# petabi/petal-neighbors

Measured on AMD Instinct MI355X. Metric: exact k-NN queries/sec (1M x 128 fp32, k=10), higher is better.
Workload: dtype f32; 1 GPU; c2: 1000000 points x 128 dims f32, 10000 queries, k=10, uniform[0,1); n_points=1000000, dim=128, n_queries=10000, k=10, engine=bf16, exchange=none (one shard), rccl_world_size=1

## Files before the change

bindings/rust/src/ffi.rs:

```rust
#![allow(non_camel_case_types)]
use std::os::raw::{c_char, c_int, c_uint, c_void};

pub const PN_RADIUS_SORTED: c_uint = 1;
pub const PN_SELF_INCLUDE: c_uint = 2;
pub const PN_MS_SEED_ROWS: c_uint = 4;
pub const PN_MS_ORPHANS: c_uint = 8;
pub const PN_KDE_GAUSSIAN: c_int = 0;
pub const PN_KDE_TOPHAT: c_int = 1;
pub const PN_KDE_EPANECHNIKOV: c_int = 2;
pub const PN_KDE_EXPONENTIAL: c_int = 3;
pub const PN_KDE_LINEAR: c_int = 4;

#[repr(C)]
pub struct pn_index {
    _private: [u8; 0],
}
#[repr(C)]
pub struct pn_sharded {
    _private: [u8; 0],
}

pub const PN_OK: c_int = 0;
pub const PN_ERR_EMPTY: c_int = 1;
pub const PN_ERR_NOT_CONTIGUOUS: c_int = 2;
pub const PN_ERR_COMM: c_int = 8;

extern "C" {
    pub fn pn_last_error() -> *const c_char;
    pub fn pn_index_destroy(index: *mut pn_index);
    pub fn pn_free(p: *mut c_void);

    pub fn pn_index_create_f32(points: *const f32, n_rows: usize, n_cols: usize, row_stride: isize, col_stride: isize,
                               device: c_int, out: *mut *mut pn_index) -> c_int;
    pub fn pn_index_create_f64(points: *const f64, n_rows: usize, n_cols: usize, row_stride: isize, col_stride: isize,
                               device: c_int, out: *mut *mut pn_index) -> c_int;
    pub fn pn_index_create_cosine_f32(points: *const f32, n_rows: usize, n_cols: usize, row_stride: isize,
                                      col_stride: isize, device: c_int, out: *mut *mut pn_index) -> c_int;
    pub fn pn_index_create_cosine_f64(points: *const f64, n_rows: usize, n_cols: usize, row_stride: isize,
                                      col_stride: isize, device: c_int, out: *mut *mut pn_index) -> c_int;

    pub fn pn_query_f32(index: *const pn_index, queries: *const f32, nq: usize, q_cols: usize, q_row_stride: isize,
                        k: usize, idx_out: *mut u64, dist_out: *mut f32) -> c_int;
    pub fn pn_query_f64(index: *const pn_index, queries: *const f64, nq: usize, q_cols: usize, q_row_stride: isize,
                        k: usize, idx_out: *mut u64, dist_out: *mut f64) -> c_int;
    pub fn pn_query_radius_f32(index: *const pn_index, queries: *const f32, nq: usize, q_cols: usize,
                               q_row_stride: isize, radius: f32, offsets: *mut u64, idx_out: *mut *mut u64) -> c_int;
    pub fn pn_query_radius_f64(index: *const pn_index, queries: *const f64, nq: usize, q_cols: usize,
                               q_row_stride: isize, radius: f64, offsets: *mut u64, idx_out: *mut *mut u64) -> c_int;
    pub fn pn_query_radius_with_distance_f32(index: *const pn_index, queries: *const f32, nq: usize, q_cols: usize,
                                             q_row_stride: isize, radius: f32, flags: c_uint, offsets: *mut u64,
                                             idx_out: *mut *mut u64, dist_out: *mut *mut f32) -> c_int;
    pub fn pn_query_radius_with_distance_f64(index: *const pn_index, queries: *const f64, nq: usize, q_cols: usize,
                                             q_row_stride: isize, radius: f64, flags: c_uint, offsets: *mut u64,
                                             idx_out: *mut *mut u64, dist_out: *mut *mut f64) -> c_int;
    pub fn pn_query_radius_with_distance_device_f32(index: *const pn_index, d_queries: *const f32, nq: usize,
                                                    q_cols: usize, q_row_stride: usize, radius: f32, flags: c_uint,
                                                    d_offsets: *mut u64, d_idx: *mut u64, d_dist: *mut f32,
                                                    capacity: usize, d_total: *mut u64, stream: *mut c_void) -> c_int;
    pub fn pn_query_radius_with_distance_device_f64(index: *const pn_index, d_queries: *const f64, nq: usize,
                                                    q_cols: usize, q_row_stride: usize, radius: f64, flags: c_uint,
                                                    d_offsets: *mut u64, d_idx: *mut u64, d_dist: *mut f64,
                                                    capacity: usize, d_total: *mut u64, stream: *mut c_void) -> c_int;
    pub fn pn_sharded_query_radius_with_distance_f32(sharded: *const pn_sharded, queries: *const f32, nq: usize,
                                                     q_cols: usize, q_row_stride: isize, radius: f32, flags: c_uint,
// ... 284 lines not shown
```

include/petal_mi355x.h:

```cpp
#ifndef PETAL_MI355X_H
#define PETAL_MI355X_H

#include <stddef.h>
#include <stdint.h>

#ifdef __cplusplus
extern "C" {
#endif

#define PN_ABI_VERSION 3

enum {
    PN_OK = 0,
    PN_ERR_EMPTY = 1,
    PN_ERR_NOT_CONTIGUOUS = 2,
    PN_ERR_INVALID = 3,
    PN_ERR_DEVICE = 4,
    PN_ERR_NOMEM = 5,
    PN_ERR_UNSUPPORTED = 6,
    PN_ERR_EMPTY_MATRIX = 7,
    PN_ERR_COMM = 8
};

enum {
    PN_ENGINE_AUTO = 0,
    PN_ENGINE_EXACT = 1,
    PN_ENGINE_MFMA = 2,
    PN_ENGINE_BF16 = 3
};

enum {
    PN_OPT_ENGINE = 1,
    PN_OPT_SEGMENTS = 2,
    PN_OPT_INDEX_BASE = 3,
    PN_OPT_PROFILE = 4,
    PN_OPT_FILTER_SLOTS = 5,
    PN_OPT_MFMA_STRUCTURE = 6,
    PN_OPT_EXCHANGE_ALWAYS = 7,
    PN_OPT_SHARED_THRESHOLDS = 8,
    PN_OPT_BF16_WAVES = 9,
    PN_OPT_SEED_MODEL = 10,
    PN_OPT_DBSCAN_PIECE = 11,
    PN_OPT_MST_BATCH = 12,
    PN_OPT_OPTICS_PIECE = 13,
    PN_OPT_KDE_PIECE = 14,
    PN_OPT_MS_PIECE = 15,
    PN_OPT_KMEANS_FILTER = 16
};

enum {
    PN_KDE_GAUSSIAN = 0,
    PN_KDE_TOPHAT = 1,
    PN_KDE_EPANECHNIKOV = 2,
    PN_KDE_EXPONENTIAL = 3,
    PN_KDE_LINEAR = 4
};

typedef struct pn_index pn_index;

typedef struct pn_info {
    uint64_t n_points;
    uint64_t dim;
    uint64_t row_stride_device;
    int32_t elem_bytes;
    int32_t device;
    int32_t mfma_eligible;
    int32_t bf16_eligible;
    int32_t bf16_layout;
    int32_t seed_model;
} pn_info;

typedef struct pn_stats {
    uint64_t queries;
    uint64_t fallback_queries;
    uint64_t candidates;
    uint64_t hot_launches;
    double hot_ms;
    double last_call_ms;
    uint64_t radius_results;
    uint64_t evaluations;
    double shard_ms;
    double exchange_ms;
    uint64_t reserved[1];
} pn_stats;

const char *pn_last_error(void);
const char *pn_strerror(int code);
int pn_abi_version(void);
int pn_device_count(int *count);

int pn_index_create_f32(const float *points, size_t n_rows, size_t n_cols, ptrdiff_t row_stride,
                        ptrdiff_t col_stride, int device, pn_index **out);
int pn_index_create_f64(const double *points, size_t n_rows, size_t n_cols, ptrdiff_t row_stride,
                        ptrdiff_t col_stride, int device, pn_index **out);
int pn_index_create_cosine_f32(const float *points, size_t n_rows, size_t n_cols, ptrdiff_t row_stride,
                               ptrdiff_t col_stride, int device, pn_index **out);
int pn_index_create_cosine_f64(const double *points, size_t n_rows, size_t n_cols, ptrdiff_t row_stride,
                               ptrdiff_t col_stride, int device, pn_index **out);
int pn_index_create_device_f32(const float *d_points, size_t n_rows, size_t n_cols, size_t row_stride,
                               int device, void *stream, pn_index **out);
// ... 378 lines not shown
```

petal-neighbors_amd/_lib.py:

```python
from __future__ import annotations

import ctypes as C
import os

_HERE = os.path.dirname(os.path.abspath(__file__))
LIB_PATH = os.environ.get("PN_LIBRARY_PATH") or os.path.join(_HERE, "libpetal_mi355x.so")

PN_OK, PN_ERR_EMPTY, PN_ERR_NOT_CONTIGUOUS, PN_ERR_INVALID, PN_ERR_DEVICE, PN_ERR_NOMEM, \
    PN_ERR_UNSUPPORTED, PN_ERR_EMPTY_MATRIX, PN_ERR_COMM = range(9)
PN_COMM_ID_BYTES = 128
PN_ENGINE_AUTO, PN_ENGINE_EXACT, PN_ENGINE_MFMA, PN_ENGINE_BF16 = 0, 1, 2, 3
PN_OPT_ENGINE, PN_OPT_SEGMENTS, PN_OPT_INDEX_BASE, PN_OPT_PROFILE, PN_OPT_FILTER_SLOTS = 1, 2, 3, 4, 5
PN_OPT_MFMA_STRUCTURE = 6
PN_OPT_EXCHANGE_ALWAYS = 7
PN_OPT_SHARED_THRESHOLDS = 8
PN_OPT_BF16_WAVES = 9
PN_OPT_SEED_MODEL = 10
PN_OPT_DBSCAN_PIECE = 11
PN_OPT_MST_BATCH = 12
PN_OPT_OPTICS_PIECE = 13
PN_OPT_KDE_PIECE = 14
PN_OPT_MS_PIECE = 15
PN_OPT_KMEANS_FILTER = 16
PN_KDE_GAUSSIAN, PN_KDE_TOPHAT, PN_KDE_EPANECHNIKOV, PN_KDE_EXPONENTIAL, PN_KDE_LINEAR = 0, 1, 2, 3, 4
PN_RADIUS_SORTED = 1
PN_SELF_INCLUDE = 2
PN_MS_SEED_ROWS = 4
PN_MS_ORPHANS = 8


class PnInfo(C.Structure):
    _fields_ = [("n_points", C.c_uint64), ("dim", C.c_uint64), ("row_stride_device", C.c_uint64),
                ("elem_bytes", C.c_int32), ("device", C.c_int32), ("mfma_eligible", C.c_int32),
                ("bf16_eligible", C.c_int32), ("bf16_layout", C.c_int32), ("seed_model", C.c_int32)]


class PnStats(C.Structure):
    _fields_ = [("queries", C.c_uint64), ("fallback_queries", C.c_uint64), ("candidates", C.c_uint64),
                ("hot_launches", C.c_uint64), ("hot_ms", C.c_double), ("last_call_ms", C.c_double),
                ("radius_results", C.c_uint64), ("evaluations", C.c_uint64),
                ("shard_ms", C.c_double), ("exchange_ms", C.c_double), ("reserved", C.c_uint64 * 1)]


class PnShardedInfo(C.Structure):
    _fields_ = [("n_points", C.c_uint64), ("dim", C.c_uint64), ("local_first_row", C.c_uint64),
                ("local_rows", C.c_uint64), ("n_shards", C.c_int32), ("world", C.c_int32),
                ("local_shards", C.c_int32), ("rank", C.c_int32), ("mfma_eligible", C.c_int32),
                ("bf16_eligible", C.c_int32)]


_sz, _ssz, _i, _vp, _u64, _cu, _d = C.c_size_t, C.c_ssize_t, C.c_int, C.c_void_p, C.c_uint64, C.c_uint, C.c_double
_u64p, _ip, _vpp = C.POINTER(C.c_uint64), C.POINTER(C.c_int), C.POINTER(C.c_void_p)
_R, _RP = "real", "real*"

_QH, _QD = [_vp, _vp, _sz, _sz, _ssz], [_vp, _vp, _sz, _sz, _sz]
_CSR_H, _CSR_D = [_vp, _vpp, _vpp], [_vp, _vp, _vp, _sz, _vp, _vp]
_CREATE = [_vp, _sz, _sz, _ssz, _ssz, _i, _vpp]
_SH_CREATE = [_vp, _sz, _sz, _ssz, _ssz, _ip, _i, _vpp]
_PAIRWISE = [_vp, _sz, _sz, _ssz, _i, _vp]

PAIRED = {
    "pn_index_create": (_i, _CREATE),
    "pn_index_create_cosine": (_i, _CREATE),
    "pn_pairwise_device": (_i, [_vp, _sz, _sz, _sz, _i, _vp, _vp]),
    "pn_index_create_device": (_i, [_vp, _sz, _sz, _sz, _i, _vp, _vpp]),
    "pn_query": (_i, _QH + [_sz, _vp, _vp]),
    "pn_query_device": (_i, _QD + [_sz, _vp, _vp, _vp]),
    "pn_query_nearest": (_i, _QH + [_vp, _vp]),
    "pn_query_radius": (_i, _QH + [_R, _vp, _vpp]),
    "pn_query_radius_device": (_i, _QD + [_R, _vp, _vp, _sz, _vp, _vp]),
    "pn_query_radius_with_distance": (_i, _QH + [_R, _cu] + _CSR_H),
    "pn_query_radius_with_distance_device": (_i, _QD + [_R, _cu] + _CSR_D),
    "pn_query_self": (_i, [_vp, _sz, _cu, _vp, _vp]),
    "pn_query_self_device": (_i, [_vp, _sz, _cu, _vp, _vp, _vp]),
    "pn_query_radius_self": (_i, [_vp, _R, _cu] + _CSR_H),
    "pn_query_radius_self_device": (_i, [_vp, _R, _cu] + _CSR_D),
# ... 128 lines not shown
```

petal-neighbors_amd/csrc/bf16_filter.hip:

```cpp
#include "pn_internal.h"
#include "topk_buffer.h"

#include <cstdio>
#include <cstdlib>

namespace pn {

typedef __bf16 bf16x8 __attribute__((ext_vector_type(8)));
typedef float f32x16 __attribute__((ext_vector_type(16)));
typedef uint32_t u32x4 __attribute__((ext_vector_type(4)));
typedef __attribute__((address_space(3))) void lds_void_b;
typedef const __attribute__((address_space(1))) void glb_void_b;

#ifdef PN_DIAG_BF_COUNT
__device__ unsigned long long g_bfdbg[16];
#define BF_COUNT(i, v) (dbg_[i] += (unsigned long long)(v))
#define BF_DBG_DECL unsigned long long dbg_[12] = {0, 0, 0, 0, 0, 0, 0, 0, 0, 0, 0, 0}
#define BF_DBG_ARG , unsigned long long (&dbg_)[12]
#define BF_DBG_PASS , dbg_
#define BF_DBG_FLUSH(lane)                                                        \
    do {                                                                          \
        if ((lane) == 0)                                                          \
            for (int i_ = 0; i_ < 12; ++i_) {                                     \
                atomicAdd(&g_bfdbg[i_], dbg_[i_]);                                \
                dbg_[i_] = 0;                                                     \
            }                                                                     \
    } while (0)
__device__ __forceinline__ unsigned long long bf_stamp() {
    unsigned long long t;
    asm volatile("s_memtime %0\n\ts_waitcnt lgkmcnt(0)" : "=s"(t)::"memory");
    return t;
}
__device__ __forceinline__ unsigned long long bf_stamp_nw() {
    unsigned long long t;
    asm volatile("s_memtime %0" : "=s"(t));
    return t;
}
__device__ __forceinline__ void bf_settle(unsigned long long &t) { asm volatile("s_waitcnt lgkmcnt(0)" : "+s"(t)::"memory"); }
#else
#define BF_COUNT(i, v) ((void)0)
#define BF_DBG_DECL ((void)0)
#define BF_DBG_ARG
#define BF_DBG_PASS
#define BF_DBG_FLUSH(lane) ((void)0)
#endif

constexpr int kBQ = 256;
constexpr int kBP = 64;
constexpr double kG = 1.0 / 8192.0;
constexpr double kUp = 1.0 + 1.0 / 1099511627776.0;
__host__ __device__ inline int bf16_extra_col(int dim) {
    const int room = (dim + 15) / 16 * 16 - dim;
    return room >= 5 && dim > 16 ? dim : (dim + 15) / 16 * 16;
}
__host__ __device__ inline int bf16_steps(int dim) { return (bf16_extra_col(dim) + 5 + 15) / 16; }
__host__ __device__ inline bool bf16_ci_dim(int dim) { return dim >= 17 && dim <= 128 && bf16_steps(dim) > (dim + 15) / 16; }
__host__ __device__ inline int bf16_steps_for(int dim, bool ci) { return ci ? (dim + 15) / 16 : bf16_steps(dim); }

__device__ __forceinline__ uint16_t bf_rne(float x) {
    const uint32_t u = __float_as_uint(x);
    return (uint16_t)((u + 0x7FFFu + ((u >> 16) & 1u)) >> 16);
}
__device__ __forceinline__ float bf_f(uint16_t b) { return __uint_as_float((uint32_t)b << 16); }
__device__ __forceinline__ float f_down(double x) {
    float f = (float)x;
    if ((double)f > x) f = __uint_as_float(__float_as_uint(f) - 1u);
    return f;
}
__device__ __forceinline__ float f_up(double x) {
    float f = (float)x;
    if ((double)f < x) f = __uint_as_float(__float_as_uint(f) + 1u);
    return f;
}
__device__ __forceinline__ float f_up_signed(double x) {
    float f = (float)x;
    if ((double)f < x) f = (f >= 0.0f) ? __uint_as_float(__float_as_uint(f) + 1u) : __uint_as_float(__float_as_uint(f) - 1u);
    return f;
}
__device__ __forceinline__ uint16_t bf_trunc(float x) { return (uint16_t)(__float_as_uint(x) >> 16); }
__device__ __forceinline__ uint16_t bf_up(float x) {
    const uint32_t u = __float_as_uint(x);
    return (uint16_t)((u >> 16) + ((u & 0xFFFFu) ? 1u : 0u));
}

constexpr int kWR = 256;
constexpr int kWPitch = 128;
constexpr int kWPiece = kWR * kWPitch;
constexpr int kWStage = 2 * kWPiece;
constexpr int kWDma = kWStage / 1024 / 8;
__host__ __device__ inline int bf16_wide_nkc(int dim) { return (dim + 63) / 64; }
__host__ __device__ inline bool bf16_wide_has_x(int dim) { return bf16_extra_col(dim) + 5 > 64 * bf16_wide_nkc(dim); }
constexpr int kWXPiece = kWR * 32;
__host__ __device__ inline size_t bf16_wide_tile_bytes(int dim) {
    return (size_t)bf16_wide_nkc(dim) * kWPiece + (bf16_wide_has_x(dim) ? kWXPiece : 0);
}
__host__ __device__ inline unsigned bf_wide_swz(size_t r) { return (unsigned)((r >> 1) & 7); }
__host__ __device__ inline unsigned bf_wide_xswz(size_t r) { return (unsigned)((r >> 3) & 1); }
__device__ __forceinline__ size_t bf_wide_at(size_t r, int k, int dim) {
    const int nkc = bf16_wide_nkc(dim);
    const size_t tile = (r / kWR) * (bf16_wide_tile_bytes(dim) / 2), rr = r % kWR;
    if ((k >> 6) >= nkc) {
        const unsigned slot = (unsigned)(((k - 64 * nkc) >> 3) & 1) ^ bf_wide_xswz(rr);
        return tile + (size_t)nkc * (kWPiece / 2) + rr * 16 + (size_t)slot * 8 + (size_t)(k & 7);
    }
    const unsigned slot = (unsigned)((k & 63) >> 3) ^ bf_wide_swz(rr);
    return tile + ((size_t)(k >> 6) * kWR + rr) * (size_t)(kWPitch / 2) + (size_t)slot * 8 + (size_t)(k & 7);
}

template <typename T>
__device__ __forceinline__ bool bf_row_part8(const T *__restrict__ src, const float *__restrict__ mu, int dim, size_t ld,
                                             int c0, int CH, bool in_rows, uint16_t (&hb)[18], double &pn, double &en,
                                             double &hn) {
    T xf[18];
#pragma unroll
    for (int i = 0; i < 18; ++i) xf[i] = (T)0;
    constexpr int VE = 16 / (int)sizeof(T);
    const bool vec = (CH % 4) == 0 && c0 + CH <= (int)ld;
    if (in_rows) {
        if (vec) {
#pragma unroll
            for (int i = 0; i < 18; i += VE)
                if (i + VE <= CH) {
                    typedef T tv_ __attribute__((ext_vector_type(VE)));
                    const tv_ t4 = *reinterpret_cast<const tv_ *>(src + c0 + i);
#pragma unroll
                    for (int j = 0; j < VE; ++j) xf[i + j] = t4[j];
                }
        } else {
#pragma unroll
// ... 97 lines not shown
template <typename T>
__global__ __launch_bounds__(256) void bf16_row_stats8_kernel(const T *__restrict__ P, const float *__restrict__ mu,
                                                              size_t n, int dim, size_t ld, int KS, size_t rows,
                                                              double *__restrict__ out) {
    const int sub = (int)(threadIdx.x & 7);
    const int CH = 2 * KS;
    double bm = 0.0, dm = 0.0, bs = 0.0, ds = 0.0;
    const size_t stride = (size_t)gridDim.x * blockDim.x;
    for (size_t t = (size_t)blockIdx.x * blockDim.x + threadIdx.x; t < rows * 8; t += stride) {
        const size_t r = t >> 3;
        uint16_t v[18];
        double pn, en, hn;
        const bool in_rows = r < n;
        const bool finite = bf_row_part8<T>(P + (in_rows ? r : 0) * ld, mu, dim, ld, sub * CH, CH, in_rows, v, pn, en, hn);
        if (in_rows && sub == 0 && finite && pn < 1.2676506002282294e30) {
            const double bp = (2.0 * sqrt(en) * kUp + 2.0 * kG * sqrt(hn) * kUp) * (1.0 + 2.0 * kG) * kUp;
            const double dp = 2.0 * sqrt(pn) * kUp * (1.0 + 2.0 * kG) * kUp;
            bm = fmax(bm, bp);
            dm = fmax(dm, dp);
            bs += bp;
            ds += dp;
        }
    }
    for (int d = 32; d > 0; d >>= 1) {
        bm = fmax(bm, __shfl_xor(bm, d));
        dm = fmax(dm, __shfl_xor(dm, d));
        bs += __shfl_xor(bs, d);
        ds += __shfl_xor(ds, d);
    }
    __shared__ double red[4][4];
    const int wave = (int)(threadIdx.x >> 6);
    if ((threadIdx.x & 63) == 0) {
        red[wave][0] = bm;
        red[wave][1] = dm;
        red[wave][2] = bs;
        red[wave][3] = ds;
    }
    __syncthreads();
    if (threadIdx.x == 0) {
        for (int w = 1; w < 4; ++w) {
            bm = fmax(bm, red[w][0]);
            dm = fmax(dm, red[w][1]);
            bs += red[w][2];
            ds += red[w][3];
        }
        atomicMax(reinterpret_cast<unsigned long long *>(out), (unsigned long long)__double_as_longlong(bm));
        atomicMax(reinterpret_cast<unsigned long long *>(out + 1), (unsigned long long)__double_as_longlong(dm));
        atomicAdd(out + 2, bs);
        atomicAdd(out + 3, ds);
    }
}

template <typename T>
__global__ void bf16_row_stats_kernel(const T *__restrict__ P, const float *__restrict__ mu, size_t n, int dim,
                                      size_t ld, double *__restrict__ out) {
    const size_t r = (size_t)blockIdx.x * blockDim.x + threadIdx.x;
    double bp = 0.0, dp = 0.0;
    if (r < n) {
        double pn = 0.0, en = 0.0, hn = 0.0;
        bool finite = true;
        const T *src = P + r * ld;
        for (int k = 0; k < dim; ++k) {
            const double x = (double)src[k];
            finite = finite && (fabs(x) < 1.0e30);
            const double c = x - (double)mu[k];
            const float cf = (float)c;
            const uint16_t hb = (fabsf(cf) < 8.67361737988403547e-19f) ? (uint16_t)0 : bf_rne(cf);
            const double xh = (double)bf_f(hb);
            pn += c * c;
            en += (c - xh) * (c - xh);
            hn += xh * xh;
        }
        if (finite && pn < 1.2676506002282294e30) {
            bp = (2.0 * sqrt(en) * kUp + 2.0 * kG * sqrt(hn) * kUp) * (1.0 + 2.0 * kG) * kUp;
            dp = 2.0 * sqrt(pn) * kUp * (1.0 + 2.0 * kG) * kUp;
        }
    }
    double bm = bp, dm = dp, bs = bp, ds = dp;
    for (int d = 32; d > 0; d >>= 1) {
        bm = fmax(bm, __shfl_xor(bm, d));
        dm = fmax(dm, __shfl_xor(dm, d));
        bs += __shfl_xor(bs, d);
        ds += __shfl_xor(ds, d);
    }
    if ((threadIdx.x & 63) == 0) {
        atomicMax(reinterpret_cast<unsigned long long *>(out), (unsigned long long)__double_as_longlong(bm));
        atomicMax(reinterpret_cast<unsigned long long *>(out + 1), (unsigned long long)__double_as_longlong(dm));
        atomicAdd(out + 2, bs);
        atomicAdd(out + 3, ds);
    }
}

template <typename T, bool QRY>
__global__ void bf16_pack_wide8_kernel(const T *__restrict__ X, const float *__restrict__ mu, size_t n_valid,
                                       size_t n_rows_img, int dim, size_t ld, uint16_t *__restrict__ img,
                                       double *__restrict__ qn, uint32_t *__restrict__ qbad, uint32_t *__restrict__ bad,
                                       Bf16SeedModel sm) {
    const size_t t = (size_t)blockIdx.x * blockDim.x + threadIdx.x;
    const size_t r = t >> 3;
    const int sub = (int)(t & 7);
    if (r >= n_rows_img) return;
    double sm_mean = 0.0, sm_var = 0.0;
    const int n_slots = 8 * bf16_wide_nkc(dim) + (bf16_wide_has_x(dim) ? 2 : 0);
    const int E = bf16_extra_col(dim);
    const int gx0 = E >> 3, gx1 = (E + 4) >> 3;
    const bool in_rows = r < n_valid;
// ... 79 lines not shown
        rem -= (double)bf_f(x[1]);
        x[2] = bf_trunc(f_down(rem));
        const double e_n = sqrt(en) * kUp, h_n = sqrt(hn) * kUp, p_n = sqrt(s) * kUp;
        x[3] = bf_up(f_up((2.0 * e_n + 2.0 * kG * h_n) * (1.0 + 2.0 * kG)));
        x[4] = bf_up(f_up(2.0 * p_n * (1.0 + 2.0 * kG)));
    }
    const bool zero_data = QRY && !ok;
    if (zero_data)
        for (int g = sub; g < n_slots; g += 8)
            if (g != gx0 && g != gx1) *reinterpret_cast<u4_ *>(img + bf_wide_at(r, 8 * g, dim)) = u4_{0u, 0u, 0u, 0u};
#pragma unroll
    for (int w = 0; w < 2; ++w) {
        const int g = w == 0 ? gx0 : gx1;
        if ((w == 1 && gx1 == gx0) || (g & 7) != sub || g >= n_slots) continue;
#pragma unroll
        for (int j = 0; j < 8; ++j) {
            const int k = 8 * g + j;
            if (zero_data) vx[w][j] = 0;
            if (k >= E && k < E + 5) vx[w][j] = x[k - E];
        }
        *reinterpret_cast<u4_ *>(img + bf_wide_at(r, 8 * g, dim)) = pack8(vx[w]);
    }
    if (QRY && sm.seed_out) {
#pragma unroll
        for (int d = 1; d < 8; d <<= 1) {
            sm_mean += __shfl_xor(sm_mean, d);
            sm_var += __shfl_xor(sm_var, d);
        }
    }
    if (sub == 0) {
        if (QRY) {
            qn[r] = ok ? s / kUp : 0.0;
            qbad[r] = ok ? 0u : 1u;
            if (sm.seed_out) {
                float sd = __uint_as_float(0xFF800000u);
                if (in_rows && ok) {
                    const double var = sm.v0 + sm_var;
                    sd = f_up_signed(sm.c0 - 2.0 * sm_mean - sm.z * sqrt(var > 0.0 ? var : 0.0));
                }
                const uint32_t key = f2s(sd);
                sm.seed_out[r] = (sd == sd && key != 0xFFFFFFFFu && in_rows && ok) ? key + 1u : f2s(__uint_as_float(0xFF800000u));
            }
        } else if (in_rows && !ok) {
            atomicOr(bad, 1u);
        }
    }
}

template <typename T>
__global__ void bf16_pack_queries8_kernel(const T *__restrict__ Q, const float *__restrict__ mu, size_t nq,
                                          size_t nq_pad, int dim, size_t ld, int KS, uint16_t *__restrict__ B,
                                          double *__restrict__ qn, uint32_t *__restrict__ qbad, int ci, double bmax,
                                          double dmax, T *__restrict__ Qp, size_t ldq,
                                          uint32_t *__restrict__ misc, Bf16SeedModel sm) {
    const size_t t = (size_t)blockIdx.x * blockDim.x + threadIdx.x;
    const size_t q = t >> 3;
    const int sub = (int)(t & 7);
    if (misc && t < 16) misc[t] = 0u;
    if (q >= nq_pad) return;
    const int K = 16 * KS, CH = 2 * KS, E = bf16_extra_col(dim);
    const int c0 = sub * CH;
    uint16_t v[18];
    double s = 0.0, en = 0.0, hn = 0.0, sm_mean = 0.0, sm_var = 0.0;
    bool finite = true;
    const T *src = Q + q * ld;
    if (Qp) {
        for (int k = K + sub; k < (int)ldq; k += 8) Qp[q * ldq + k] = (T)0;
    }
    T xf[18];
    const bool in_rows = q < nq;
    constexpr int VE = 16 / (int)sizeof(T);
    const bool vec = (CH % 4) == 0 && ((reinterpret_cast<uintptr_t>(Q) | (ld * sizeof(T))) & 15u) == 0 &&
                     c0 + CH <= dim;
#pragma unroll
    for (int i = 0; i < 18; ++i) xf[i] = (T)0;
    if (in_rows) {
        if (vec) {
#pragma unroll
            for (int i = 0; i < 18; i += VE)
                if (i + VE <= CH) {
                    typedef T tv_ __attribute__((ext_vector_type(VE)));
                    const tv_ t4 = *reinterpret_cast<const tv_ *>(src + c0 + i);
#pragma unroll
                    for (int j = 0; j < VE; ++j) xf[i + j] = t4[j];
                }
        } else {
#pragma unroll
            for (int i = 0; i < 18; ++i)
                if (i < CH && c0 + i < dim) xf[i] = src[c0 + i];
        }
    }
    if (Qp) {
        T *qd = Qp + q * ldq + c0;
#pragma unroll
        for (int i = 0; i < 18; i += 2)
            if (i + 2 <= CH && c0 + i + 2 <= (int)ldq) {
                typedef T tp_ __attribute__((ext_vector_type(2)));
                tp_ pr;
                pr[0] = xf[i];
                pr[1] = xf[i + 1];
                *reinterpret_cast<tp_ *>(qd + i) = pr;
            }
    }
    float muv[18], m1v[18], av[18], bv[18];
    const bool vecm = (CH % 4) == 0 && c0 + CH <= dim;
#pragma unroll
    for (int i = 0; i < 18; i += 4) {
// ... 35 lines not shown
            const double x = (double)xf[i];
            finite = finite && (fabs(x) < 1.0e30);
            const double c = x - (double)muv[i];
            const float cf = (float)c;
            const uint16_t hb = (fabsf(cf) < 8.67361737988403547e-19f) ? (uint16_t)0 : bf_rne(cf);
            const float xh = bf_f(hb);
            v[i] = bf_rne(-2.0f * xh);
            s += c * c;
            const double e = c - (double)xh;
            en += e * e;
            hn += (double)xh * (double)xh;
            if (sm.seed_out) {
                sm_mean += c * (double)m1v[i];
                sm_var += c * (c * (double)av[i] - (double)bv[i]);
            }
        }
    }
    uint32_t fin = finite ? 1u : 0u;
#pragma unroll
    for (int d = 1; d < 8; d <<= 1) {
        s += __shfl_xor(s, d);
        en += __shfl_xor(en, d);
        hn += __shfl_xor(hn, d);
        fin &= (uint32_t)__shfl_xor((int)fin, d);
    }
    if (sm.seed_out) {
#pragma unroll
        for (int d = 1; d < 8; d <<= 1) {
            sm_mean += __shfl_xor(sm_mean, d);
            sm_var += __shfl_xor(sm_var, d);
        }
    }
    const bool ok = fin != 0u && (s < 1.2676506002282294e30);
    if (!ok) {
#pragma unroll
        for (int i = 0; i < 18; ++i)
            if (c0 + i < dim) v[i] = 0;
    }
    if (!ci) {
#pragma unroll
        for (int i = 0; i < 18; ++i) {
            const int k = c0 + i;
            if (i < CH) {
                if (k == E + 0 || k == E + 1 || k == E + 2) v[i] = 0x3F80u;
                if (ok && k == E + 3) v[i] = (uint16_t)(bf_up(f_up(sqrt(hn) * kUp)) | 0x8000u);
                if (ok && k == E + 4) v[i] = (uint16_t)(bf_up(f_up(sqrt(en) * kUp)) | 0x8000u);
            }
        }
    }
    uint16_t *dst = B + q * (size_t)K + c0;
#pragma unroll
    for (int i = 0; i < 18; ++i)
        if (i < CH) dst[i] = v[i];
    if (sub == 0) {
        if (ci) {
            const double eq = (sqrt(hn) * kUp * bmax + sqrt(en) * kUp * dmax) * kUp;
            qn[q] = ok ? s / kUp - eq : 0.0;
        } else {
            qn[q] = ok ? s / kUp : 0.0;
        }
        qbad[q] = ok ? 0u : 1u;
        if (sm.seed_out) {
            float sd = __uint_as_float(0xFF800000u);
            if (q < nq && ok) {
                const double var = sm.v0 + sm_var;
                const double S = sm.c0 - 2.0 * sm_mean - sm.z * sqrt(var > 0.0 ? var : 0.0);
                sd = f_up_signed(S);
            }
            const uint32_t key = f2s(sd);
            sm.seed_out[q] = (sd == sd && key != 0xFFFFFFFFu && q < nq && ok) ? key + 1u : f2s(__uint_as_float(0xFF800000u));
        }
    }
}

template <typename T>
__global__ __launch_bounds__(256) void cos_normalize_rows_kernel(const T *__restrict__ X, size_t n_valid, size_t n_out,
                                                                 int dim, size_t ld_in, double *__restrict__ out,
                                                                 size_t ld_out, uint32_t *__restrict__ bad, int nan_rows) {
    const size_t t = (size_t)blockIdx.x * blockDim.x + threadIdx.x;
    const size_t r = t >> 3;
    const int sub = (int)(t & 7);
    if (r >= n_out) return;
    const int CH = (int)(ld_out / 8), c0 = sub * CH;
    double *o = out + r * ld_out + c0;
    if (r >= n_valid) {
        for (int i = 0; i < CH; ++i) o[i] = 0.0;
        return;
    }
    const T *x = X + r * ld_in;
    double ss = 0.0;
    for (int i = 0; i < CH; ++i)
        if (c0 + i < dim) {
            const double v = (double)x[c0 + i];
            ss += v * v;
        }
#pragma unroll
    for (int d = 1; d < 8; d <<= 1) ss += __shfl_xor(ss, d);
    const bool ok = ss >= 7.888609052210118e-31 && ss <= 1.2676506002282294e30;
    if (!ok) {
        if (nan_rows) {
            for (int i = 0; i < CH; ++i) o[i] = (c0 + i < dim) ? __longlong_as_double(0x7FF8000000000000ll) : 0.0;
        } else {
            if (sub == 0) atomicOr(bad, 1u);
            for (int i = 0; i < CH; ++i) o[i] = 0.0;
        }
        return;
    }
    const double inv = 1.0 / sqrt(ss);
    for (int i = 0; i < CH; ++i) o[i] = (c0 + i < dim) ? (double)x[c0 + i] * inv : 0.0;
}
template <typename T>
hipError_t launch_cos_normalize_rows(const T *X, size_t n_valid, size_t n_out, int dim, size_t ld_in, double *out,
                                     size_t ld_out, uint32_t *bad, bool nan_rows, hipStream_t s) {
    if (ld_out % 8 != 0 || (size_t)dim > ld_out || (size_t)dim > ld_in) return hipErrorInvalidValue;
// ... 83 lines not shown
}

constexpr int kLA = 3;
constexpr int kBfFinalKeep = 32;
constexpr int kScoutList = 12;
__device__ __forceinline__ void bf_min2(const f32x16 &v, float &mn, float &sec) {
    const float big = 3.4e38f;
    auto lo3 = [](float a, float b, float c) { return fminf(fminf(a, b), c); };
    auto md3 = [](float a, float b, float c) { return __builtin_amdgcn_fmed3f(a, b, c); };
    const float l0 = lo3(v[0], v[1], v[2]), d0 = md3(v[0], v[1], v[2]);
    const float l1 = lo3(v[3], v[4], v[5]), d1 = md3(v[3], v[4], v[5]);
    const float l2 = lo3(v[6], v[7], v[8]), d2 = md3(v[6], v[7], v[8]);
    const float l3 = lo3(v[9], v[10], v[11]), d3 = md3(v[9], v[10], v[11]);
    const float l4 = lo3(v[12], v[13], v[14]), d4 = md3(v[12], v[13], v[14]);
    const float l5 = v[15];
    const float a = lo3(l0, l1, l2), am = md3(l0, l1, l2);
    const float b = lo3(l3, l4, l5), bm = md3(l3, l4, l5);
    mn = fminf(a, b);
    const float sec_lo = lo3(fmaxf(a, b), am, bm);
    const float dmin = fminf(lo3(d0, d1, d2), fminf(d3, d4));
    sec = fminf(sec_lo, dmin);
    (void)big;
}

template <int KS, bool CI>
__device__ __forceinline__ void bf_chain(const char *arow, const bf16x8 (&pre)[kLA], const bf16x8 (&b0)[KS],
                                         const bf16x8 (&b1)[KS], const f32x16 &c0, f32x16 &w0, f32x16 &w1, f32x16 &r0,
                                         f32x16 &r1, float &m0, float &m1) {
    bf16x8 f[KS];
#pragma unroll
    for (int i = 0; i < kLA && i < KS; ++i) f[i] = pre[i];
    f32x16 z;
#pragma unroll
    for (int i = 0; i < 16; ++i) z[i] = 0.0f;
#pragma unroll
    for (int ks = 0; ks < KS; ++ks) {
        if (ks + kLA < KS) f[ks + kLA] = *reinterpret_cast<const bf16x8 *>(arow + 32 * (ks + kLA));
        if (CI) {
            w0 = __builtin_amdgcn_mfma_f32_32x32x16_bf16(f[ks], b0[ks], ks ? w0 : c0, 0, 0, 0);
            w1 = __builtin_amdgcn_mfma_f32_32x32x16_bf16(f[ks], b1[ks], ks ? w1 : c0, 0, 0, 0);
        } else {
            w0 = __builtin_amdgcn_mfma_f32_32x32x16_bf16(f[ks], b0[ks], ks ? w0 : z, 0, 0, 0);
            w1 = __builtin_amdgcn_mfma_f32_32x32x16_bf16(f[ks], b1[ks], ks ? w1 : z, 0, 0, 0);
        }
#pragma unroll
        for (int i = 16 * ks / KS; i < 16 * (ks + 1) / KS; ++i) {
            m0 = i ? fminf(m0, r0[i]) : r0[0];
            m1 = i ? fminf(m1, r1[i]) : r1[0];
        }
        __builtin_amdgcn_sched_barrier(0);
    }
}

template <int CP>
__device__ __forceinline__ f32x16 bf_cinit(const char *tb, int blk, int h) {
    typedef float f32x4_ __attribute__((ext_vector_type(4)));
    f32x16 c;
#pragma unroll
    for (int g = 0; g < 4; ++g) {
        const f32x4_ v = *reinterpret_cast<const f32x4_ *>(tb + ((blk * 8 + 2 * g + h) * CP + (CP - 1)) * 16);
        c[4 * g + 0] = v[0];
        c[4 * g + 1] = v[1];
        c[4 * g + 2] = v[2];
        c[4 * g + 3] = v[3];
    }
    return c;
}

struct BfNoMid {
    static constexpr int at(int) { return -1; }
    __device__ __forceinline__ void operator()() const {}
};
template <int KS, bool CI, int CP, typename MID = BfNoMid>
__device__ __forceinline__ void bf_chain_p(const char *arow, bf16x8 (&pre)[kLA], const bf16x8 (&b0)[KS],
                                           const bf16x8 (&b1)[KS], f32x16 &c, f32x16 &w0, f32x16 &w1, f32x16 &r0,
                                           f32x16 &r1, float &m0, float &m1, const char *narow, const char *ntb,
                                           int nblk, int h, MID mid = MID()) {
    typedef float f32x4_ __attribute__((ext_vector_type(4)));
    bf16x8 f[KS];
#pragma unroll
    for (int i = 0; i < kLA && i < KS; ++i) f[i] = pre[i];
    f32x16 z, nc = c;
#pragma unroll
    for (int i = 0; i < 16; ++i) z[i] = 0.0f;
#pragma unroll
    for (int ks = 0; ks < KS; ++ks) {
        if (ks == MID::at(KS)) mid();
        if (ks + kLA < KS) f[ks + kLA] = *reinterpret_cast<const bf16x8 *>(arow + 32 * (ks + kLA));
#pragma unroll
        for (int i = 0; i < kLA; ++i)
            if (ks == (KS - kLA + i > 0 ? KS - kLA + i : 0))
                pre[i] = *reinterpret_cast<const bf16x8 *>(narow + 32 * (i < KS ? i : 0));
        if (CI) {
#pragma unroll
            for (int g = 0; g < 4; ++g)
                if (ks == (KS - 4 + g > 0 ? KS - 4 + g : 0)) {
                    const f32x4_ v =
                        *reinterpret_cast<const f32x4_ *>(ntb + ((nblk * 8 + 2 * g + h) * CP + (CP - 1)) * 16);
                    nc[4 * g + 0] = v[0];
                    nc[4 * g + 1] = v[1];
                    nc[4 * g + 2] = v[2];
                    nc[4 * g + 3] = v[3];
                }
            w0 = __builtin_amdgcn_mfma_f32_32x32x16_bf16(f[ks], b0[ks], ks ? w0 : c, 0, 0, 0);
            w1 = __builtin_amdgcn_mfma_f32_32x32x16_bf16(f[ks], b1[ks], ks ? w1 : c, 0, 0, 0);
            if (ks == 0) asm volatile("" ::"v"(c));
        } else {
            w0 = __builtin_amdgcn_mfma_f32_32x32x16_bf16(f[ks], b0[ks], ks ? w0 : z, 0, 0, 0);
            w1 = __builtin_amdgcn_mfma_f32_32x32x16_bf16(f[ks], b1[ks], ks ? w1 : z, 0, 0, 0);
        }
#pragma unroll
        for (int i = 16 * ks / KS; i < 16 * (ks + 1) / KS; ++i) {
            m0 = i ? fminf(m0, r0[i]) : r0[0];
            m1 = i ? fminf(m1, r1[i]) : r1[0];
        }
        __builtin_amdgcn_sched_barrier(0);
    }
    c = nc;
}

constexpr uint32_t kShPeriod = 32;
constexpr uint32_t kShMaxPass = 1u << 14;
__device__ __forceinline__ uint32_t sh_load(const uint32_t *p) {
    return __hip_atomic_load(p, __ATOMIC_RELAXED, __HIP_MEMORY_SCOPE_AGENT);
}
__device__ __forceinline__ void sh_store(uint32_t *p, uint32_t v) {
    __hip_atomic_store(p, v, __ATOMIC_RELAXED, __HIP_MEMORY_SCOPE_AGENT);
}
__device__ __forceinline__ void sh_store_entry(uint2 *p, uint32_t key, uint32_t row) {
    __hip_atomic_store(reinterpret_cast<unsigned long long *>(p), ((unsigned long long)row << 32) | key, __ATOMIC_RELAXED,
                       __HIP_MEMORY_SCOPE_AGENT);
}
__device__ __forceinline__ uint32_t sh_tag(uint32_t epoch, uint32_t ncomp) { return (epoch << 20) | ((ncomp & 0xFFu) << 12); }

template <int M>
__device__ __forceinline__ void bf_refresher(const uint2 *__restrict__ cand, const uint32_t *pcnt, uint32_t *gtau,
                                          const uint32_t *done, uint32_t n_main, size_t nq_pad, uint32_t nseg,
                                          uint32_t epoch, uint32_t rank, uint32_t wv, uint32_t n_wv, int lane) {
    constexpr uint32_t CAP = 64u * M;
    constexpr int NK = 8;
    auto words_of = [&](size_t q) -> uint32_t {
        uint32_t x = 0;
        if (lane < (int)nseg) x = sh_load(pcnt + (size_t)lane * nq_pad + q);
        else if (lane == 63) x = sh_load(done);
        return x;
    };
    for (uint32_t pass = 0; pass < kShMaxPass; ++pass) {
        uint32_t x_next = words_of(wv < nq_pad ? wv : 0);
        for (size_t q = wv; q < nq_pad; q += n_wv) {
            const uint32_t x = x_next;
            x_next = words_of(q + n_wv < nq_pad ? q + n_wv : q);
            if ((uint32_t)__builtin_amdgcn_readlane((int)x, 63) >= n_main) return;
#ifdef PN_DIAG_BF_COUNT
            if (lane == 0) atomicAdd(&g_bfdbg[12], 1ull);
#endif
            uint32_t c = (lane < (int)nseg && (x >> 20) == epoch) ? (x & 0xFFFu) : 0u;
            if (c > CAP) c = 0;
            uint32_t inc = c;
#pragma unroll
            for (int d = 1; d < 64; d <<= 1) {
                const uint32_t t = (uint32_t)__shfl_up((int)inc, d);
                if (lane >= d) inc += t;
            }
            uint32_t U = (uint32_t)__builtin_amdgcn_readlane((int)inc, 63);
            if (U < rank) continue;
            if (U > 64u * NK) U = 64u * NK;
            const uint32_t excl = inc - c;
            uint32_t key[NK];
#pragma unroll
            for (int i = 0; i < NK; ++i) key[i] = 0xFFFFFFFFu;
            const int nk = (int)((U + 63u) / 64u);
// ... 861 lines not shown
        }
        asm volatile("s_waitcnt vmcnt(0)" ::: "memory");
        const uint32_t kfin = keep_arg > kp ? keep_arg : kp;
        unsigned long long need = __ballot(h == 0 && cnt > kfin);
        constexpr int NB = M == 1 ? 4 : 1;
        while (need) {
            int jj[NB];
            uint32_t cj[NB], key[NB][M], ixs[NB][M];
#pragma unroll
            for (int bb = 0; bb < NB; ++bb) {
                jj[bb] = need ? __builtin_ctzll(need) : -1;
                if (need) need &= need - 1;
                cj[bb] = jj[bb] >= 0 ? (uint32_t)__builtin_amdgcn_readlane((int)cnt, jj[bb] >= 0 ? jj[bb] : 0) : 0u;
                if (jj[bb] >= 0) bf_compact_load<M>(ce_blk + (size_t)jj[bb] * CAP, cj[bb], lane, key[bb], ixs[bb]);
            }
#pragma unroll
            for (int bb = 0; bb < NB; ++bb) {
                if (jj[bb] >= 0) {
                    uint32_t T, nn;
                    bf_compact_finish<M>(ce_blk + (size_t)jj[bb] * CAP, key[bb], ixs[bb], cj[bb], kp, lane, T, nn);
                    if (jq == jj[bb]) { tau = fminf(tau, s2f(T)); cnt = nn; }
                }
            }
        }
        if (h == 0) {
            ccnt[cell0 + jq] = cnt;
            ctau[cell0 + jq] = f2s(tau);
        }
        BF_DBG_FLUSH(lane);
    }
    if (SH) {
        __syncthreads();
        if (tid == 0) (void)__hip_atomic_fetch_add(sh.done, 1u, __ATOMIC_RELAXED, __HIP_MEMORY_SCOPE_AGENT);
    }
}

#ifndef PN_DIAG_PAIR_STAGGER
#define PN_DIAG_PAIR_STAGGER 1
#endif
constexpr int kPairStagger = PN_DIAG_PAIR_STAGGER;
#ifndef PN_DIAG_PAIR_MID4
#define PN_DIAG_PAIR_MID4 2
#endif
struct BfPairMeet {
    uint32_t ns;
    static constexpr int at(int ks) { return ks * PN_DIAG_PAIR_MID4 / 4 > 1 ? ks * PN_DIAG_PAIR_MID4 / 4 : 1; }
    __device__ __forceinline__ void operator()() const {
        bf_wait_dma(ns);
        __builtin_amdgcn_s_barrier();
        asm volatile("" ::: "memory");
    }
};

template <int KS, bool CI, int STAG>
__device__ __forceinline__ void bf_pair_run(const char *__restrict__ img, char *tiles, uint32_t kp, uint32_t kfin, uint2 *__restrict__ cand,
                                            uint32_t *__restrict__ ccnt, uint32_t *__restrict__ ctau,
                                            const bf16x8 (&b0)[KS], const bf16x8 (&b1)[KS], float tau0, float tau1,
                                            uint32_t rt0, uint32_t rt1, size_t cell0, bool active, int wave, int lane) {
    constexpr int C = 2 * KS, CP = C + 1;
    constexpr uint32_t CAP = 64u;
    constexpr int TB = kBP * CP * 16;
    constexpr int NBUF = 3, NW = 8;
    const int jq = lane & 31, h = lane >> 5;
    BF_DBG_DECL;
    constexpr int P = (CP + NW - 1) / NW;
    static_assert(P <= 3, "piece schedule written out for up to three pieces per wave");
    const int n_mine = CP - wave * P < P ? (CP - wave * P > 0 ? CP - wave * P : 0) : P;
    const uint32_t lane_off = (uint32_t)lane * 16u;
    auto dma_tile = [&](uint32_t rt, int buf) {
        const char *wbase = img + ((size_t)rt * (size_t)TB + (size_t)(wave * (P * 1024)));
        const char *ws = wbase + lane_off;
        char *wd = tiles + buf * TB + wave * (P * 1024);
        if (0 < n_mine) __builtin_amdgcn_global_load_lds((glb_void_b *)ws, (lds_void_b *)wd, 16, 0, 0);
        if (P > 1 && 1 < n_mine) __builtin_amdgcn_global_load_lds((glb_void_b *)ws, (lds_void_b *)wd, 16, 1024, 0);
        if (P > 2 && 2 < n_mine) __builtin_amdgcn_global_load_lds((glb_void_b *)ws, (lds_void_b *)wd, 16, 2048, 0);
    };

    uint32_t cnt0 = 0, cnt1 = 0;
    uint2 *ce_blk0 = cand + cell0 * CAP;
    uint2 *ce_blk1 = ce_blk0 + (size_t)32 * CAP;
    uint2 *ceq0 = ce_blk0 + (size_t)jq * CAP, *ceq1 = ce_blk1 + (size_t)jq * CAP;
    uint32_t ns = 0;

    f32x16 a00, a01, a10, a11;
#pragma unroll
    for (int r = 0; r < 16; ++r) {
        a00[r] = 3.0e38f;
        a01[r] = 3.0e38f;
        a10[r] = 3.0e38f;
        a11[r] = 3.0e38f;
    }
    bf16x8 pre[kLA];
    f32x16 cc = a00;
    {
        const char *ar = tiles + (jq * CP + h) * 16;
#pragma unroll
        for (int i = 0; i < kLA; ++i) pre[i] = *reinterpret_cast<const bf16x8 *>(ar + 32 * (i < KS ? i : 0));
        if (CI) cc = bf_cinit<CP>(tiles, 0, h);
    }
    int cur = 0;
    for (uint32_t rt = rt0; rt < rt1; ++rt) {
        const int nxt = cur == NBUF - 1 ? 0 : cur + 1, prv = cur == 0 ? NBUF - 1 : cur - 1;
        const char *tb = tiles + cur * TB;
        const char *arow0 = tb + (jq * CP + h) * 16;
        const char *arow1 = arow0 + 32 * CP * 16;
        float m0, m1, p0, p1;
        if (STAG == 2) BfPairMeet{ns}();
        if (STAG == 1)
            bf_chain_p<KS, CI, CP>(arow0, pre, b0, b1, cc, a00, a01, a10, a11, m0, m1, arow1, tb, 1, h, BfPairMeet{ns});
        else
            bf_chain_p<KS, CI, CP>(arow0, pre, b0, b1, cc, a00, a01, a10, a11, m0, m1, arow1, tb, 1, h);
        if (rt == rt0) { m0 = __uint_as_float(0x7F800000u); m1 = m0; }
        if (__any(m0 < tau0 || m1 < tau1)) {
            const uint32_t row0 = (rt - 1) * kBP + 32;
            if (__any(m0 < tau0)) bf_slow<1, false>(a10, m0, tau0, cnt0, row0, h, jq, lane, kp, ceq0, ce_blk0, ns BF_DBG_PASS);
            if (__any(m1 < tau1)) bf_slow<1, false>(a11, m1, tau1, cnt1, row0, h, jq, lane, kp, ceq1, ce_blk1, ns BF_DBG_PASS);
        }
        if (STAG == 0) {
            bf_wait_dma(ns);
#ifndef PN_DIAG_PAIR_NOLGKM
            asm volatile("s_waitcnt lgkmcnt(0)" ::: "memory");
#endif
            __builtin_amdgcn_s_barrier();
            asm volatile("" ::: "memory");
        }
        if (rt + 2 < rt1) {
            dma_tile(rt + 2, prv);
            ns = 0;
        }
        const bool last = rt + 1 >= rt1;
        const char *ntb = last ? tb : tiles + nxt * TB;
        bf_chain_p<KS, CI, CP>(arow1, pre, b0, b1, cc, a10, a11, a00, a01, p0, p1, ntb + (jq * CP + h) * 16, ntb, 0, h);
        if (__any(p0 < tau0 || p1 < tau1)) {
            const uint32_t row0 = rt * kBP;
            if (__any(p0 < tau0)) bf_slow<1, false>(a00, p0, tau0, cnt0, row0, h, jq, lane, kp, ceq0, ce_blk0, ns BF_DBG_PASS);
            if (__any(p1 < tau1)) bf_slow<1, false>(a01, p1, tau1, cnt1, row0, h, jq, lane, kp, ceq1, ce_blk1, ns BF_DBG_PASS);
        }
        cur = nxt;
    }
    {
        float m0 = a10[0], m1 = a11[0];
#pragma unroll
        for (int i = 1; i < 16; ++i) {
            m0 = fminf(m0, a10[i]);
            m1 = fminf(m1, a11[i]);
        }
        const uint32_t row0 = (rt1 - 1) * kBP + 32;
        if (__any(m0 < tau0)) bf_slow<1, false>(a10, m0, tau0, cnt0, row0, h, jq, lane, kp, ceq0, ce_blk0, ns BF_DBG_PASS);
        if (__any(m1 < tau1)) bf_slow<1, false>(a11, m1, tau1, cnt1, row0, h, jq, lane, kp, ceq1, ce_blk1, ns BF_DBG_PASS);
    }
    asm volatile("s_waitcnt vmcnt(0)" ::: "memory");
    auto final_compact = [&](uint2 *ce_blk, float &tau, uint32_t &cnt) {
        constexpr int NB = 4;
        unsigned long long need = __ballot(h == 0 && cnt > kfin);
        while (need) {
            int jj[NB];
            uint32_t cj[NB], key[NB][1], ixs[NB][1];
#pragma unroll
            for (int b = 0; b < NB; ++b) {
                jj[b] = need ? __builtin_ctzll(need) : -1;
                if (need) need &= need - 1;
                cj[b] = jj[b] >= 0 ? (uint32_t)__builtin_amdgcn_readlane((int)cnt, jj[b] >= 0 ? jj[b] : 0) : 0u;
                if (jj[b] >= 0) bf_compact_load<1>(ce_blk + (size_t)jj[b] * CAP, cj[b], lane, key[b], ixs[b]);
            }
#pragma unroll
            for (int b = 0; b < NB; ++b) {
                if (jj[b] >= 0) {
                    uint32_t T, nn;
                    bf_compact_finish<1>(ce_blk + (size_t)jj[b] * CAP, key[b], ixs[b], cj[b], kp, lane, T, nn);
                    if (jq == jj[b]) { tau = fminf(tau, s2f(T)); cnt = nn; }
                }
            }
        }
    };
    final_compact(ce_blk0, tau0, cnt0);
    final_compact(ce_blk1, tau1, cnt1);
    if (active && h == 0) {
        ccnt[cell0 + jq] = cnt0;
        ctau[cell0 + jq] = f2s(tau0);
        ccnt[cell0 + 32 + jq] = cnt1;
        ctau[cell0 + 32 + jq] = f2s(tau1);
    }
    BF_DBG_FLUSH(lane);
}

template <int KS, bool CI>
__global__ __launch_bounds__(512, 2) void bf16_filter_kernel_pair(const char *__restrict__ img, uint32_t n_tiles,
                                                                  const u32x4 *__restrict__ Bq, uint32_t q_tiles,
                                                                  uint32_t kp_keep, uint2 *__restrict__ cand,
                                                                  uint32_t *__restrict__ ccnt,
                                                                  uint32_t *__restrict__ ctau, size_t nq_pad,
                                                                  const uint32_t *tau_init, BfShared sh) {
    const uint32_t kp = kp_keep & 0xFFFFu, keep_arg = kp_keep >> 16;
    const uint32_t kfin = keep_arg > kp ? keep_arg : kp;
    constexpr int CP = 2 * KS + 1;
    constexpr int TB = kBP * CP * 16;
    extern __shared__ __attribute__((aligned(16))) unsigned char smem_raw[];
    char *tiles = reinterpret_cast<char *>(smem_raw);
    const int tid = threadIdx.x, lane = tid & 63;
    const int wave = __builtin_amdgcn_readfirstlane(tid >> 6);
    const int jq = lane & 31, h = lane >> 5;
    constexpr int C = 2 * KS;
    const uint32_t W = gridDim.x, n_pairs = (q_tiles + 1u) >> 1, c_per = W / n_pairs;
    uint32_t w;
    {
        const uint32_t b = blockIdx.x, x = b & 7u, base = W >> 3, rem = W & 7u;
        const uint32_t L = x * base + (x < rem ? x : rem) + (b >> 3);
        w = (L % n_pairs) * c_per + L / n_pairs;
    }
    const uint32_t pt = w / c_per, seg = w % c_per;
    const uint32_t rt0 = (uint32_t)((unsigned long long)seg * n_tiles / c_per);
    const uint32_t rt1 = (uint32_t)((unsigned long long)(seg + 1) * n_tiles / c_per);
    if (rt0 >= rt1) return;
    const uint32_t qt = 2u * pt + (uint32_t)(wave >> 2);
    const bool active = qt < q_tiles;
    const size_t q0 = active ? (size_t)qt * kBQ + (size_t)(wave & 3) * 64 : 0;
    const size_t cell0 = (size_t)seg * nq_pad + q0;

    bf16x8 b0[KS], b1[KS];
    float tau0 = __uint_as_float(0xFF800000u), tau1 = tau0;
    if (active) {
        const u32x4 *br0 = Bq + (q0 + jq) * (size_t)C + h;
        const u32x4 *br1 = br0 + (size_t)32 * C;
#pragma unroll
        for (int ks = 0; ks < KS; ++ks) {
            const u32x4 v0 = br0[2 * ks], v1 = br1[2 * ks];
            b0[ks] = __builtin_bit_cast(bf16x8, v0);
            b1[ks] = __builtin_bit_cast(bf16x8, v1);
        }
        if (sh.seed_lists) {
            const size_t ql = q0 + (size_t)lane;
            float sd = __uint_as_float(0xFF800000u);
            if (ql < (size_t)sh.seed_nq) {
                const uint32_t key = f2s(bf_seed_lane(sh.seed_lists, nq_pad, sh.nseg, sh.seed_rank, ql));
                sd = s2f(key == 0xFFFFFFFFu ? key : key + 1u);
            }
            tau0 = __shfl(sd, jq);
            tau1 = __shfl(sd, 32 + jq);
        } else {
            tau0 = s2f(tau_init[q0 + jq]);
            tau1 = s2f(tau_init[q0 + 32 + jq]);
        }
    } else {
        const u32x4 zero = {0u, 0u, 0u, 0u};
#pragma unroll
        for (int ks = 0; ks < KS; ++ks) {
            b0[ks] = __builtin_bit_cast(bf16x8, zero);
            b1[ks] = b0[ks];
        }
    }
    {
        constexpr int P = (CP + 7) / 8;
        const int n_mine = CP - wave * P < P ? (CP - wave * P > 0 ? CP - wave * P : 0) : P;
        for (uint32_t t = 0; t < 2u && rt0 + t < rt1; ++t) {
            const char *ws = img + ((size_t)(rt0 + t) * (size_t)TB + (size_t)(wave * (P * 1024))) + (uint32_t)lane * 16u;
            char *wd = tiles + t * TB + wave * (P * 1024);
            if (0 < n_mine) __builtin_amdgcn_global_load_lds((glb_void_b *)ws, (lds_void_b *)wd, 16, 0, 0);
            if (P > 1 && 1 < n_mine) __builtin_amdgcn_global_load_lds((glb_void_b *)ws, (lds_void_b *)wd, 16, 1024, 0);
            if (P > 2 && 2 < n_mine) __builtin_amdgcn_global_load_lds((glb_void_b *)ws, (lds_void_b *)wd, 16, 2048, 0);
        }
    }
    __syncthreads();
    if (wave >= 4)
        bf_pair_run<KS, CI, kPairStagger>(img, tiles, kp, kfin, cand, ccnt, ctau, b0, b1, tau0, tau1, rt0, rt1, cell0,
                                          active, wave, lane);
    else
        bf_pair_run<KS, CI, 0>(img, tiles, kp, kfin, cand, ccnt, ctau, b0, b1, tau0, tau1, rt0, rt1, cell0, active, wave,
                               lane);
}

template <int M, bool RAD>
__global__ __launch_bounds__(512, 1) void bf16_wide_kernel(const char *__restrict__ img, uint32_t n_tiles,
                                                           const char *__restrict__ Bimg, uint32_t nkc,
                                                           uint32_t tile_bytes, uint32_t has_x, uint32_t kp,
                                                           uint2 *__restrict__ cand, uint32_t *__restrict__ ccnt,
                                                           uint32_t *__restrict__ ctau, size_t nq_pad,
                                                           uint32_t scout_max,
                                                           const uint32_t *__restrict__ tau_init,
                                                           float *__restrict__ scout_out) {
    constexpr uint32_t CAP = 64u * M;
    extern __shared__ __attribute__((aligned(16))) unsigned char smem_raw[];
    char *lds = reinterpret_cast<char *>(smem_raw);

    const int tid = threadIdx.x, lane = tid & 63;
    const int wave = __builtin_amdgcn_readfirstlane(tid >> 6);
    const int jq = lane & 31, h = lane >> 5;
    const int qg = wave & 3, rh = wave >> 2;
    BF_DBG_DECL;

    uint32_t w = blockIdx.x;
    const uint32_t W = gridDim.x;
    {
        const uint32_t x = blockIdx.x & 7u, base = W >> 3, rem = W & 7u;
        w = x * base + (x < rem ? x : rem) + (blockIdx.x >> 3);
    }
    const unsigned long long U = (unsigned long long)(nq_pad / kWR) * n_tiles, Wn = W;
    unsigned long long u0 = (unsigned long long)w * U / Wn;
    const unsigned long long u1 = (unsigned long long)(w + 1) * U / Wn;
    const float inf = __uint_as_float(0x7F800000u);

    int slot_off[4];
#pragma unroll
    for (int s = 0; s < 4; ++s) slot_off[s] = (int)(((unsigned)(2 * s + h) ^ bf_wide_swz((size_t)jq)) * 16u);
    int st = 0;
    uint32_t ns = 0;
    f32x16 acc[4][2];

    while (u0 < u1) {
    const uint32_t qt = (uint32_t)(u0 / n_tiles);
    const unsigned long long v_begin = (unsigned long long)qt * n_tiles, v_end = v_begin + n_tiles;
    const unsigned long long run_end = u1 < v_end ? u1 : v_end;
    const uint32_t rt0 = (uint32_t)(u0 - v_begin), rt1 = (uint32_t)(run_end - v_begin);
    unsigned long long wf = v_begin * Wn / U;
    while ((wf + 1) * U / Wn <= v_begin) ++wf;
    while (wf > 0 && wf * U / Wn > v_begin) --wf;
    const uint32_t sg = (uint32_t)(w - wf);
    const size_t q0 = (size_t)qt * kWR + (size_t)qg * 64;
    const size_t cell0 = (size_t)(sg * 2 + rh) * nq_pad + q0;
    float tau0 = inf, tau1 = inf;
    uint32_t cnt0 = 0, cnt1 = 0;

// ... 356 lines not shown
    double mu2 = 0.0;
    for (int k = 0; k < dim; ++k) {
        const double m = sums[k] / (double)n;
        const float f = (m == m && fabs(m) < 1e30) ? (float)m : 0.0f;
        mu[k] = f;
        mu2 += (double)f * (double)f;
    }
    const double s2 = sums[dim], s2c = s2 - (double)n * mu2;
    const bool centered = !never && s2 > 0.0 && s2c < s2 / factor;
    if (!centered)
        for (int k = 0; k < dim; ++k) mu[k] = 0.0f;
    words[0] = centered ? 1u : 0u;
}
hipError_t launch_bf16_decide_mu(const double *sums, size_t n, int dim, bool never, float *mu, uint32_t *words, hipStream_t s) {
    hipLaunchKernelGGL(bf16_decide_mu_kernel, dim3(1), dim3(64), 0, s, sums, n, dim, bf16_is_wide(dim) ? 2.0 : 16.0,
                       never ? 1 : 0, mu, words);
    return hipGetLastError();
}

template <typename T>
hipError_t launch_bf16_row_stats(const T *P, const float *mu, size_t n, int dim, size_t ld, double *out4,
                                 hipStream_t s) {
    if (!bf16_is_wide(dim)) {
        const size_t rows = (n + 31) / 32 * 32;
        const size_t blocks = rows * 8 / 256;
        hipLaunchKernelGGL(bf16_row_stats8_kernel<T>, dim3((unsigned)(blocks < 2048 ? blocks : 2048)), dim3(256), 0, s, P, mu,
                           n, dim, ld, bf16_ks_for(dim, false), rows, out4);
        return hipGetLastError();
    }
    hipLaunchKernelGGL(bf16_row_stats_kernel<T>, dim3((unsigned)((n + 127) / 128)), dim3(128), 0, s, P, mu, n, dim, ld, out4);
    return hipGetLastError();
}
template hipError_t launch_bf16_row_stats<float>(const float *, const float *, size_t, int, size_t, double *, hipStream_t);
template hipError_t launch_bf16_row_stats<double>(const double *, const float *, size_t, int, size_t, double *, hipStream_t);

template <typename T>
hipError_t launch_bf16_pack_corpus(const T *P, const float *mu, size_t n, int dim, size_t ld, void *img,
                                   uint32_t *bad, bool ci, hipStream_t s) {
    const bool wide = bf16_is_wide(dim);
    if (wide && ci) return hipErrorInvalidValue;
    const size_t rows = wide ? (n + kWR - 1) / kWR * kWR : (n + kBP - 1) / kBP * kBP;
    if (wide) {
        hipLaunchKernelGGL((bf16_pack_wide8_kernel<T, false>), dim3((unsigned)(rows * 8 / 256)), dim3(256), 0, s, P, mu, n, rows,
                           dim, ld, static_cast<uint16_t *>(img), (double *)nullptr, (uint32_t *)nullptr, bad, Bf16SeedModel{});
        return hipGetLastError();
    }
    hipLaunchKernelGGL(bf16_pack_corpus8_kernel<T>, dim3((unsigned)(rows * 8 / 256)), dim3(256), 0, s, P, mu, n, dim, ld,
                       bf16_ks_for(dim, ci), static_cast<uint16_t *>(img), rows, bad, ci ? 1 : 0);
    return hipGetLastError();
}
template hipError_t launch_bf16_pack_corpus<float>(const float *, const float *, size_t, int, size_t, void *, uint32_t *, bool, hipStream_t);
template hipError_t launch_bf16_pack_corpus<double>(const double *, const float *, size_t, int, size_t, void *, uint32_t *, bool, hipStream_t);

bool bf16_pack_fused_supported(int dim) { return !bf16_is_wide(dim); }
template <typename T>
hipError_t launch_bf16_pack_queries(const T *Q, const float *mu, size_t nq, size_t nq_pad, int dim, size_t ld,
                                    void *B, double *qn, uint32_t *qbad, bool ci, double bmax, double dmax,
                                    hipStream_t s, T *Qp, size_t ldq, uint32_t *misc, const Bf16SeedModel *smp) {
    if ((Qp || misc) && !bf16_pack_fused_supported(dim)) return hipErrorInvalidValue;
    Bf16SeedModel sm{};
    if (smp) sm = *smp;
    if (sm.seed_out && (!sm.m1 || !sm.a || !sm.b)) return hipErrorInvalidValue;
    if (!bf16_is_wide(dim)) {
        hipLaunchKernelGGL(bf16_pack_queries8_kernel<T>, dim3((unsigned)(nq_pad * 8 / 256)), dim3(256), 0, s, Q, mu, nq,
                           nq_pad, dim, ld, bf16_ks_for(dim, ci), static_cast<uint16_t *>(B), qn, qbad, ci ? 1 : 0,
                           bmax, dmax, Qp, ldq, misc, sm);
        return hipGetLastError();
    }
    if (ci || nq_pad % 32 != 0) return hipErrorInvalidValue;
    hipLaunchKernelGGL((bf16_pack_wide8_kernel<T, true>), dim3((unsigned)(nq_pad * 8 / 256)), dim3(256), 0, s, Q, mu, nq, nq_pad,
                       dim, ld, static_cast<uint16_t *>(B), qn, qbad, (uint32_t *)nullptr, sm);
    return hipGetLastError();
}
template <typename T>
__global__ void bf16_column_moments_kernel(const T *__restrict__ P, const float *__restrict__ mu, size_t n, int dim, size_t ld,
                                           double *__restrict__ out) {
    const size_t r0 = (size_t)blockIdx.x * 1024;
    const size_t r1 = r0 + 1024 < n ? r0 + 1024 : n;
    for (int k = threadIdx.x; k < dim; k += blockDim.x) {
        const double m = (double)mu[k];
        double s1 = 0.0, s2 = 0.0, s3 = 0.0, s4 = 0.0;
        for (size_t r = r0; r < r1; ++r) {
            const double x = (double)P[r * ld + k];
            const double u = (fabs(x) < 1.0e30) ? x - m : 0.0;
            const double u2 = u * u;
            s1 += u;
            s2 += u2;
            s3 += u2 * u;
            s4 += u2 * u2;
        }
        atomicAdd(&out[k], s1);
        atomicAdd(&out[dim + k], s2);
        atomicAdd(&out[2 * dim + k], s3);
        atomicAdd(&out[3 * dim + k], s4);
    }
}
template <typename T>
hipError_t launch_bf16_column_moments(const T *P, const float *mu, size_t n, int dim, size_t ld, double *out, hipStream_t s) {
    hipLaunchKernelGGL(bf16_column_moments_kernel<T>, dim3((unsigned)((n + 1023) / 1024)), dim3(128), 0, s, P, mu, n, dim, ld, out);
    return hipGetLastError();
}
template hipError_t launch_bf16_column_moments<float>(const float *, const float *, size_t, int, size_t, double *, hipStream_t);
template hipError_t launch_bf16_column_moments<double>(const double *, const float *, size_t, int, size_t, double *, hipStream_t);

template hipError_t launch_bf16_pack_queries<float>(const float *, const float *, size_t, size_t, int, size_t, void *, double *,
                                                    uint32_t *, bool, double, double, hipStream_t, float *, size_t, uint32_t *,
                                                    const Bf16SeedModel *);
template hipError_t launch_bf16_pack_queries<double>(const double *, const float *, size_t, size_t, int, size_t, void *, double *,
                                                     uint32_t *, bool, double, double, hipStream_t, double *, size_t, uint32_t *,
                                                     const Bf16SeedModel *);

static_assert(kBQ == (int)kBf16QueryTile && kBP == (int)kBf16RowTile && kWR == (int)kBf16WideTile, "bf16_launch.h");
static void bf_debug_kernel(const char *which, unsigned grid, unsigned block) {
    if (debug_plan()) std::fprintf(stderr, "bf16 main pass: kernel %s grid %u x %u\n", which, grid, block);
}
template <auto Kern, typename... A>
static hipError_t bf_go(unsigned grid, unsigned block, size_t sh, hipStream_t s, A... args) {
    static LdsAttrOnce lds_attr;
    const hipError_t e = lds_attr.ensure(reinterpret_cast<const void *>(Kern), sh);
    if (e != hipSuccess) return e;
    hipLaunchKernelGGL(Kern, dim3(grid), dim3(block), sh, s, args...);
    return hipGetLastError();
}
static bool bf_launch_valid(const Bf16Launch &l, bool wide) {
    const CandBuf &cb = l.cb;
    const Bf16Grid &g = l.grid, w = bf16_grid(l.n, cb.nq_pad, g.n_wg, g.split, wide);
    if (!bf16_supported(l.dim) || bf16_is_wide(l.dim) != wide || cb.nq_pad % kBQ || l.kp < 1 || l.kp + 32 > cb.cap ||
        (cb.cap != 64 && cb.cap != 128 && cb.cap != 256) || cb.idx_stride != 2 ||
        cb.idx != static_cast<uint32_t *>(cb.keys) + 1 || g.n_wg < 1 || g.split < 1 || l.scout_tiles < 0)
        return false;
    if (g.q_tiles < 1 || g.q_tiles != w.q_tiles || g.n_tiles != w.n_tiles || g.aligned != w.aligned || g.nseg != w.nseg ||
        g.run_tiles != w.run_tiles || cb.nseg < g.nseg || (wide ? g.split != 1 : (uint32_t)g.split > g.n_tiles))
        return false;
    const bool thresholds = l.pass == Bf16Pass::Seeded || l.pass == Bf16Pass::Radius;
    if (thresholds != (l.tau != nullptr) || (l.pass == Bf16Pass::ScoutOnly) != (l.scout_out != nullptr)) return false;
    return l.pass != Bf16Pass::Radius || (cb.cap == 256 && !l.refresh);
}
template <int KS, int M, bool RAD, bool CI>
static hipError_t launch_bf16_t(const Bf16Launch &l, hipStream_t s) {
    const CandBuf &cb = l.cb;
    const Bf16Grid &g = l.grid;
    const size_t sh = (size_t)3 * kBP * (2 * KS + 1) * 16 + 16;
    const uint32_t kp = (uint32_t)l.kp, split = (uint32_t)g.split, scout = (uint32_t)l.scout_tiles;
    const uint32_t kp_keep = kp | ((uint32_t)(M <= 2 && !RAD && cb.final_keep > (int)kp ? cb.final_keep : 0) << 16);
    const uint32_t spp = (uint32_t)bf16_touching((size_t)g.q_tiles * split, g.n_wg);
    const unsigned n_wg = (unsigned)g.n_wg, n_all = n_wg + (unsigned)(l.refresh ? l.refresh->n_refresh : 0);
    BfShared a{};
    a.nseg = (uint32_t)cb.nseg;
    if (l.seed) {
        a.seed_lists = l.seed->lists;
        a.seed_rank = l.seed->rank;
        a.seed_nq = l.seed->nq;
        a.seed_words = l.seed->words;
    }
    if (l.refresh) {
        a.pcnt = l.refresh->pcnt;
        a.done = l.refresh->done;
        a.n_main = n_wg;
        a.epoch = l.refresh->epoch;
        a.rank = l.refresh->rank;
    }
    const char *img = static_cast<const char *>(l.img);
    const u32x4 *B = static_cast<const u32x4 *>(l.B);
    uint2 *keys = static_cast<uint2 *>(cb.keys);
    uint32_t *tau = static_cast<uint32_t *>(cb.tau);
    if constexpr (!RAD) {
        if constexpr (M == 1)
            if (l.kernel == Bf16Kernel::Pair) {
                const unsigned grid = (unsigned)(((g.q_tiles + 1u) / 2u) * (n_wg / g.q_tiles));
                bf_debug_kernel("pair", grid, 512);
                return bf_go<bf16_filter_kernel_pair<KS, CI>>(grid, 512, sh, s, img, g.n_tiles, B, g.q_tiles, kp_keep, keys,
                                                              cb.cnt, tau, cb.nq_pad, l.tau, a);
            }
        if (l.kernel == Bf16Kernel::Eight) {
            bf_debug_kernel("8", n_all, 512);
            return l.refresh ? bf_go<bf16_filter8_kernel<KS, CI, true, M>>(n_all, 512, sh, s, img, g.n_tiles, B, g.q_tiles, kp_keep,
                                                                          keys, cb.cnt, tau, cb.nq_pad, l.tau, a)
                             : bf_go<bf16_filter8_kernel<KS, CI, false, M>>(n_all, 512, sh, s, img, g.n_tiles, B, g.q_tiles, kp_keep,
                                                                           keys, cb.cnt, tau, cb.nq_pad, l.tau, a);
        }
        if constexpr (M <= 2)
            if (l.refresh) {
                bf_debug_kernel("4", n_all, 256);
                return bf_go<bf16_filter_kernel<KS, M, false, CI, 2, true>>(n_all, 256, sh, s, img, g.n_tiles, B, g.q_tiles, kp_keep,
                                                                           keys, cb.cnt, tau, cb.nq_pad, split, spp, scout, l.tau,
                                                                           l.scout_out, a);
            }
    }
#define PN_BF_LAUNCH_MODE(MD)                                                                                            \
    bf_go<bf16_filter_kernel<KS, M, RAD, CI, MD>>(n_wg, 256, sh, s, img, g.n_tiles, B, g.q_tiles, kp_keep, keys, cb.cnt, tau, \
                                                  cb.nq_pad, split, spp, scout, l.tau, l.scout_out, a)
    if (l.pass == Bf16Pass::ScoutOnly) return PN_BF_LAUNCH_MODE(1);
    if (l.pass != Bf16Pass::SelfScout) {
        if (!RAD) bf_debug_kernel("4", n_wg, 256);
        return PN_BF_LAUNCH_MODE(2);
    }
    return PN_BF_LAUNCH_MODE(0);
#undef PN_BF_LAUNCH_MODE
}

template <int KS, bool CI>
static hipError_t launch_bf16_m(const Bf16Launch &l, hipStream_t s) {
    if (l.pass == Bf16Pass::Radius) return launch_bf16_t<KS, 4, true, CI>(l, s);
    switch (l.cb.cap) {
        case 64: return launch_bf16_t<KS, 1, false, CI>(l, s);
        case 128: return launch_bf16_t<KS, 2, false, CI>(l, s);
        default: return launch_bf16_t<KS, 4, false, CI>(l, s);
    }
}

bool bf16_shared_supported(int cap) {
    return cap == 64 || cap == 128;
}
hipError_t launch_bf16_filter(const Bf16Launch &l, hipStream_t s) {
    const CandBuf &cb = l.cb;
    if (!bf_launch_valid(l, false) || (l.ci && !bf16_ci_dim(l.dim)) ||
        !bf16_kernel_applies(l.kernel, l.grid, cb.cap, l.pass, l.refresh.has_value()))
        return hipErrorInvalidValue;
    if (l.refresh) {
        const Bf16Refresh &r = *l.refresh;
        if (l.pass != Bf16Pass::Seeded || !l.grid.aligned || !bf16_shared_supported(cb.cap) || r.n_refresh < 1 ||
            r.epoch < 1 || r.epoch > 4095 || r.rank < 1 || !r.pcnt || !r.done)
            return hipErrorInvalidValue;
    }
    if (l.seed && (!l.seed->lists || l.seed->rank < 1 || l.seed->rank > (uint32_t)kScoutList || !bf16_seed_in_kernel(cb.nseg)))
        return hipErrorInvalidValue;
#define PN_BF_CASE(K, C) \
    case K: return launch_bf16_m<K, C>(l, s);
#ifdef PN_DEV_KS8_ONLY
    if (l.ci) {
        switch (bf16_ks_for(l.dim, true)) {
            PN_BF_CASE(8, true)
            default: return hipErrorInvalidValue;
        }
    }
    return hipErrorInvalidValue;
#else
    if (l.ci) {
        switch (bf16_ks_for(l.dim, true)) {
            PN_BF_CASE(2, true) PN_BF_CASE(3, true) PN_BF_CASE(4, true) PN_BF_CASE(5, true) PN_BF_CASE(6, true)
            PN_BF_CASE(7, true) PN_BF_CASE(8, true)
            default: return hipErrorInvalidValue;
        }
    }
    switch (bf16_ks_for(l.dim, false)) {
        PN_BF_CASE(2, false) PN_BF_CASE(3, false) PN_BF_CASE(4, false) PN_BF_CASE(5, false) PN_BF_CASE(6, false)
        PN_BF_CASE(7, false) PN_BF_CASE(8, false) PN_BF_CASE(9, false)
        default: return hipErrorInvalidValue;
    }
#endif
#undef PN_BF_CASE
}

__global__ __launch_bounds__(64) void bf16_seed_kernel(const float *__restrict__ lists, size_t nq_pad, int nseg,
                                                       uint32_t rank, uint32_t *__restrict__ out, size_t nq) {
    extern __shared__ __attribute__((aligned(16))) unsigned char smem_raw[];
    uint32_t *sk = reinterpret_cast<uint32_t *>(smem_raw);
    const int lane = threadIdx.x;
    const size_t q = blockIdx.x;
    if (q >= nq) {
        if (lane == 0) out[q] = f2s(__uint_as_float(0xFF800000u));
        return;
    }
    const uint32_t per = 2 * kScoutList, n = (uint32_t)nseg * per;
    uint32_t T = 0;
    if (n <= 512u) {
        uint32_t v[8];
#pragma unroll
        for (int i = 0; i < 8; ++i) {
            const uint32_t e = (uint32_t)lane + 64u * (uint32_t)i;
            v[i] = e < n ? f2s(lists[((size_t)(e / per) * nq_pad + q) * per + e % per]) : 0xFFFFFFFFu;
        }
        for (int bit = 31; bit >= 0; --bit) {
            const uint32_t cnd = T | (1u << bit);
            uint32_t c = 0;
#pragma unroll
            for (int i = 0; i < 8; ++i) c += (uint32_t)__popcll(__ballot(v[i] < cnd));
            if (c < rank) T = cnd;
        }
// ... 195 lines not shown
```

petal-neighbors_amd/csrc/bf16_launch.h:

```cpp
#pragma once

#include <cstddef>
#include <cstdint>

namespace pn {

enum class Bf16Pass { ScoutOnly, SelfScout, Seeded, Radius };
enum class Bf16Kernel { Four, Eight, Pair, Wide };

constexpr uint32_t kBf16QueryTile = 256;
constexpr uint32_t kBf16RowTile = 64;
constexpr uint32_t kBf16WideTile = 256;

inline int bf16_touching(size_t q_tiles, int n_wg) { return (int)(((size_t)n_wg + q_tiles - 1) / q_tiles) + 1; }
inline int bf16_segments(size_t q_tiles, int n_wg, int split) {
    return split * bf16_touching(q_tiles * (size_t)split, n_wg);
}

struct Bf16Grid {
    uint32_t q_tiles, n_tiles;
    int n_wg, split;
    bool aligned;
    int nseg;
    uint32_t run_tiles;
};
inline Bf16Grid bf16_grid(size_t n, size_t nq_pad, int n_wg, int split, bool wide = false) {
    Bf16Grid g{};
    const uint32_t rows = wide ? kBf16WideTile : kBf16RowTile;
    g.q_tiles = (uint32_t)(nq_pad / kBf16QueryTile);
    g.n_tiles = (uint32_t)((n + rows - 1) / rows);
    g.n_wg = n_wg;
    g.split = split;
    g.aligned = split == 1 && g.q_tiles > 0 && n_wg >= (int)g.q_tiles && (uint32_t)n_wg % g.q_tiles == 0;
    const int per_query = g.aligned ? n_wg / (int)g.q_tiles : g.q_tiles ? bf16_segments(g.q_tiles, n_wg, split) : 0;
    g.nseg = wide ? 2 * per_query : per_query;
    g.run_tiles = g.aligned && !wide ? g.n_tiles / (uint32_t)per_query : 0u;
    return g;
}

constexpr uint32_t kBf8MaxRun = 200;
constexpr size_t kBf8MaxImage = (size_t)768 << 20;
#ifndef PN_DIAG_PAIR_MIN_RUN
#define PN_DIAG_PAIR_MIN_RUN 200
#endif
constexpr uint32_t kPairMinRun = PN_DIAG_PAIR_MIN_RUN;

inline bool bf16_kernel_applies(Bf16Kernel k, const Bf16Grid &g, int cap, Bf16Pass pass, bool refreshers) {
    if (k == Bf16Kernel::Four) return true;
    if (k == Bf16Kernel::Wide || pass != Bf16Pass::Seeded || !g.aligned) return false;
    return k == Bf16Kernel::Eight || (cap == 64 && !refreshers && g.q_tiles >= 2);
}
inline Bf16Kernel bf16_main_kernel(const Bf16Grid &g, int cap, Bf16Pass pass, bool refreshers, size_t image_bytes,
                                   int wg_slots, int forced) {
    if (!bf16_kernel_applies(Bf16Kernel::Eight, g, cap, pass, refreshers)) return Bf16Kernel::Four;
    if (bf16_kernel_applies(Bf16Kernel::Pair, g, cap, pass, refreshers)) {
        const bool fills = wg_slots > 0 && g.n_wg >= wg_slots;
        if (forced == 16 || (forced == 0 && fills && g.run_tiles >= kPairMinRun && image_bytes <= kBf8MaxImage))
            return Bf16Kernel::Pair;
    }
    const bool want8 = forced == 8 || (forced == 0 && image_bytes <= kBf8MaxImage && (cap >= 128 || g.run_tiles < kBf8MaxRun));
    return want8 ? Bf16Kernel::Eight : Bf16Kernel::Four;
}

}
```

petal-neighbors_amd/csrc/index.hip:

```cpp
#include <algorithm>
#include <cmath>
#include <cstdarg>
#include <cstddef>
#include <cstdio>
#include <cstdlib>
#include <cstring>
#include <atomic>
#include <chrono>
#include <mutex>
#include <new>
#include <string>
#include <thread>
#include <vector>

#include "../../include/petal_mi355x.h"
#include "pn_internal.h"
#include "csr_pieces.h"

using namespace pn;

static thread_local std::string g_err;

static int fail(int code, const char *fmt, ...) {
    char buf[512];
// ... 43 lines not shown
        case PN_ERR_UNSUPPORTED: return "unsupported";
        case PN_ERR_EMPTY_MATRIX: return "empty matrix";
        case PN_ERR_COMM: return "collective communication (RCCL) error";
        default: return "unknown error";
    }
}
extern "C" int pn_device_count(int *count) {
    if (!count) return fail(PN_ERR_INVALID, "count is NULL");
    int c = 0;
    hipError_t e = hipGetDeviceCount(&c);
    if (e != hipSuccess) {
        *count = 0;
        return fail(PN_ERR_DEVICE, "hipGetDeviceCount: %s", hipGetErrorString(e));
    }
    *count = c;
    return PN_OK;
}

struct DevBuf {
    void *p = nullptr;
    size_t bytes = 0;
    std::vector<void *> *retired = nullptr;
    int ensure(size_t need) {
        if (need <= bytes && p) return PN_OK;
        if (p) {
            bool kept = false;
            if (retired) {
                try {
                    retired->push_back(p);
                    kept = true;
                } catch (const std::bad_alloc &) {
                }
            }
            if (!kept) (void)hipFree(p);
        }
        p = nullptr;
        bytes = 0;
        size_t want = need + need / 8 + 256;
        hipError_t e = hipMalloc(&p, want);
        if (e != hipSuccess) return fail(PN_ERR_NOMEM, "hipMalloc(%zu): %s", want, hipGetErrorString(e));
        bytes = want;
        return PN_OK;
    }
    void release() {
        if (p) (void)hipFree(p);
        p = nullptr;
        bytes = 0;
    }
};

struct WorkspaceBufs {
    DevBuf w_q, w_qnorm, w_qnrm, w_keys, w_idx, w_cnt, w_tau, w_flags, w_sel, w_misc, w2_keys, w2_idx, w2_cnt, w2_tau, w_lo;
    DevBuf w_bq, w_qn, w_qbad, w_gq, w_gqn, w_gsel, w_seed, w_lists;
    DevBuf w_hq, w_hidx, w_hdist;
    DevBuf w_hrad;
    DevBuf w_fparts;
    DevBuf w_rpos, w_rfin, w_rcx, w_rox, w_rscan;
    DevBuf w_rkd;
    DevBuf w_cs_nch, w_cs_off, w_cs_scan, w_cs_idx, w_cs_dist, w_cs_hoff;
    DevBuf w_sf_idx, w_sf_dist, w_sf_off, w_sf_coff, w_sf_flag, w_sf_cnt, w_sf_scan, w_sf_hoff;
    DevBuf w_db, w_db_side, w_db_out;
    DevBuf w_mst, w_mst_io;
    DevBuf w_hdb, w_hdb_io;
    DevBuf w_lof, w_lof_io;
    DevBuf w_opt, w_opt_graph, w_opt_io;
    DevBuf w_kde, w_kde_io;
    DevBuf w_ms, w_ms_io;
    DevBuf w_km_rows, w_km_cent, w_km, w_km_upd, w_km_io;
    DevBuf w_pcnt;
};
static_assert(std::is_standard_layout<WorkspaceBufs>::value && sizeof(WorkspaceBufs) % sizeof(DevBuf) == 0,
              "WorkspaceBufs holds DevBuf members only");
struct Workspace : WorkspaceBufs {
    void *pin_in = nullptr, *pin_out = nullptr;
    size_t pin_in_bytes = 0, pin_out_bytes = 0;
    int pin_ensure(void **p, size_t *have, size_t need) {
        if (need <= *have && *p) return PN_OK;
        if (*p) {
            (void)hipStreamSynchronize(stream);
            (void)hipHostFree(*p);
        }
        *p = nullptr;
        *have = 0;
        const size_t want = need + need / 2 + 4096;
        if (hipHostMalloc(p, want, hipHostMallocMapped) != hipSuccess) return fail(PN_ERR_NOMEM, "hipHostMalloc(%zu) failed", want);
        *have = want;
        return PN_OK;
    }
    uint32_t sh_epoch = 0;
    size_t sh_nseg = 0, sh_nq_pad = 0;
    hipStream_t stream = nullptr;
    hipEvent_t ev_r[2] = {nullptr, nullptr};
    hipEvent_t done = nullptr;
    hipStream_t last_stream = nullptr;
    bool in_flight = false;
    std::vector<void *> retired;
    DevBuf *begin() { return reinterpret_cast<DevBuf *>(static_cast<WorkspaceBufs *>(this)); }
    DevBuf *end() { return begin() + sizeof(WorkspaceBufs) / sizeof(DevBuf); }
    Workspace() {
        for (DevBuf &b : *this) b.retired = &retired;
    }
    Workspace(const Workspace &) = delete;
    Workspace &operator=(const Workspace &) = delete;
    void free_retired() {
        for (void *q : retired) (void)hipFree(q);
        retired.clear();
    }
};

struct CallRec {
    hipEvent_t ev[6] = {nullptr, nullptr, nullptr, nullptr, nullptr, nullptr};
    hipEvent_t done = nullptr;
    uint32_t *h_nflag = nullptr;
    size_t nq = 0;
    uint64_t call_id = 0;
    bool pending = false, busy = false, two_launches = false, has_flag = false, bf16_tier = false, hot = false;
    bool model_seed = false;
    int prof = 0;
};
constexpr int kCallRecs = 16;

constexpr int kSeedModelRetry = 64, kSeedModelMaxRetries = 3;
constexpr int kSeedModelGrid = 7;
enum PieceFamily { kPieceDbscan, kPieceOptics, kPieceKde, kPieceMs, kPieceFamilies };
struct pn_index {
    int device = 0;
    int elem_bytes = 4;
    size_t n = 0, dim = 0, ld = 0, n_pad = 0;
    void *d_pts = nullptr;
    float *d_norm = nullptr;
    bool mfma_ok = false;
    void *d_img = nullptr;
    float *d_mu = nullptr;
    bool centered = false;
    bool bf16_ok = false;
    int metric = 0;
    void *d_cnorm = nullptr;
    bool bf16_ci = false;
    double bf16_bmax = 0.0, bf16_dmax = 0.0;
    int n_cu = 256;
    hipStream_t stream = nullptr;
    unsigned long long *d_stats = nullptr;
    int engine = PN_ENGINE_AUTO;
    int opt_segments = 0;
    uint64_t index_base = 0;
    int profile = 0;
    int filter_slots = 0;
    int mfma_structure = 0;
    int shared_tau = 1;
    int bf16_waves = 0;
    float *d_smodel = nullptr;
    double sm_c0 = 0.0, sm_v0 = 0.0;
    double sm_zgrid[kSeedModelGrid] = {};
    double sm_sigma = 0.0;
    bool sm_ok = false;
    int seed_model = 1;
    uint64_t piece[kPieceFamilies] = {};
    uint64_t mst_batch = 0;
    int kmeans_filter = 0;
    struct Shared {
        std::mutex mu;
        std::vector<Workspace *> free_ws, all_ws;
        CallRec recs[kCallRecs];
        unsigned next_rec = 0;
        uint64_t next_call = 1, stats_call = 0;
        int bf16_level = 0;
        std::atomic<int> seed_model_widen{0};
        std::atomic<bool> seed_model_off{false};
        int seed_model_off_calls = 0;
        int seed_model_retries = 0;
        pn_stats stats{};
        std::atomic<HostTree *> tree{nullptr};
        std::mutex tree_mu;
    };
    mutable Shared sh;
};

struct DeviceGuard {
    int prev = -1;
    bool ok = true;
    explicit DeviceGuard(int dev) {
        if (hipGetDevice(&prev) != hipSuccess) prev = -1;
        if (prev != dev) ok = hipSetDevice(dev) == hipSuccess;
    }
    ~DeviceGuard() {
        if (prev >= 0) (void)hipSetDevice(prev);
    }
};

static int check_device(int device) {
    int c = 0;
    hipError_t e = hipGetDeviceCount(&c);
    if (e != hipSuccess || c <= 0)
        return fail(PN_ERR_DEVICE, "no usable GPU (hipGetDeviceCount: %s); this library has no CPU path",
                    hipGetErrorString(e));
    if (device < 0 || device >= c) return fail(PN_ERR_INVALID, "device %d out of range [0,%d)", device, c);
    return PN_OK;
}

namespace {
struct StreamPool {
    std::mutex mu;
    std::vector<std::pair<int, hipStream_t>> idle;
};
StreamPool &stream_pool() {
    static StreamPool *p = new StreamPool();
    return *p;
}
constexpr size_t kStreamPoolMax = 32;
// ... 53 lines not shown
PinnedPool &pinned_pool() {
    static PinnedPool *p = new PinnedPool();
    return *p;
}
constexpr size_t kPinnedBlock = 256;
struct PinnedBlock {
    void *h = nullptr;
    ~PinnedBlock() {
        if (!h) return;
        PinnedPool &pp = pinned_pool();
        std::lock_guard<std::mutex> lk(pp.mu);
        if (pp.idle.size() < 16) pp.idle.push_back(h);
        else (void)hipHostFree(h);
    }
    hipError_t acquire() {
        {
            PinnedPool &pp = pinned_pool();
            std::lock_guard<std::mutex> lk(pp.mu);
            if (!pp.idle.empty()) {
                h = pp.idle.back();
                pp.idle.pop_back();
                return hipSuccess;
            }
        }
        return hipHostMalloc(&h, kPinnedBlock, hipHostMallocDefault);
    }
};
}

struct BuildWords {
    double st[4];
    uint32_t w[4];
    float selftest;
    uint32_t pad;
};
constexpr int kMaxDevices = 64;
static std::atomic<int> g_bf16_hw[kMaxDevices];
static std::atomic<bool> g_bf16_hw_init{false};
static std::mutex g_bf16_hw_mu;
static std::atomic<int> &bf16_hw_state(int device) {
    if (!g_bf16_hw_init.load(std::memory_order_acquire)) {
        std::lock_guard<std::mutex> lk(g_bf16_hw_mu);
        if (!g_bf16_hw_init.load(std::memory_order_relaxed)) {
            for (auto &a : g_bf16_hw) a.store(-1, std::memory_order_relaxed);
            g_bf16_hw_init.store(true, std::memory_order_release);
        }
    }
    return g_bf16_hw[device >= 0 && device < kMaxDevices ? device : 0];
}
constexpr float kBf16SelftestLimit = 0.02f;

template <typename RT>
static int seed_model_build(pn_index *ix, const RT *rows, hipStream_t s);
template <typename T>
static int finish_index(pn_index *ix, const T *d_src, size_t row_stride, hipStream_t s) {
    {
        hipDeviceProp_t prop;
        if (hipGetDeviceProperties(&prop, ix->device) == hipSuccess && prop.multiProcessorCount > 0)
            ix->n_cu = prop.multiProcessorCount;
    }
    HIPCHK(hipMalloc((void **)&ix->d_stats, kPnStatWords * sizeof(unsigned long long)));
    HIPCHK(hipMemsetAsync(ix->d_stats, 0, kPnStatWords * sizeof(unsigned long long), s));
    const size_t bytes = ix->n_pad * ix->ld * sizeof(T);
    HIPCHK(hipMalloc(&ix->d_pts, bytes ? bytes : 256));
    HIPCHK(launch_pack_rows<T>(d_src, ix->n, ix->dim, row_stride, (T *)ix->d_pts, ix->n_pad, ix->ld, s));
    ix->mfma_ok = false;
    ix->bf16_ok = false;
    ix->bf16_ci = false;
    const bool cosine = ix->metric == 1;
    if (cosine) {
        HIPCHK(hipMalloc(&ix->d_cnorm, ix->n_pad * sizeof(T)));
        HIPCHK(hipMemsetAsync(ix->d_cnorm, 0, ix->n_pad * sizeof(T), s));
        HIPCHK(launch_cosine_norms<T>((const T *)ix->d_pts, ix->n, (int)ix->dim, ix->ld, (T *)ix->d_cnorm, s));
    }
    DevTmp scr, nrm;
    PinnedBlock hw;
    const size_t sums_bytes = (ix->dim + 1) * sizeof(double);
    HIPCHK(scr.alloc(sums_bytes + sizeof(BuildWords)));
    HIPCHK(hipMemsetAsync(scr.p, 0, sums_bytes + sizeof(BuildWords), s));
    HIPCHK(hw.acquire());
    static_assert(sizeof(BuildWords) <= kPinnedBlock, "host words fit one pinned block");
    double *d_sums = (double *)scr.p;
    BuildWords *d_bw = (BuildWords *)((char *)scr.p + sums_bytes);
    BuildWords *h_bw = (BuildWords *)hw.h;
    uint32_t *d_w = (uint32_t *)((char *)d_bw + offsetof(BuildWords, w));
    double *d_st = (double *)((char *)d_bw + offsetof(BuildWords, st));
    auto read_words = [&]() -> int {
        HIPCHK(hipMemcpyAsync(h_bw, d_bw, sizeof(BuildWords), hipMemcpyDeviceToHost, s));
        HIPCHK(hipStreamSynchronize(s));
        return PN_OK;
    };
    if constexpr (sizeof(T) == 4) {
        if (!cosine) {
            HIPCHK(hipMalloc((void **)&ix->d_norm, ix->n_pad * sizeof(float)));
            HIPCHK(launch_row_norms_f32((const float *)ix->d_pts, ix->n_pad, ix->n, (int)ix->dim, ix->ld,
                                        mfma_alpha(ix->dim), ix->d_norm, d_w + 0, s));
        }
    }
    const bool try_bf16 = bf16_supported((int)ix->dim) && ix->n < 0xFFFFFFF0ull && ix->n >= 64;
    if (try_bf16) {
        const void *rows = ix->d_pts;
        if (cosine) {
            HIPCHK(nrm.alloc(ix->n_pad * ix->ld * sizeof(double)));
            HIPCHK(launch_cos_normalize_rows<T>((const T *)ix->d_pts, ix->n, ix->n_pad, (int)ix->dim, ix->ld, (double *)nrm.p,
                                                ix->ld, d_w + 1, false, s));
            rows = nrm.p;
        }
        auto col_sums = [&]() {
            return cosine ? launch_bf16_column_sums<double>((const double *)rows, ix->n, (int)ix->dim, ix->ld, d_sums, s)
                          : launch_bf16_column_sums<T>((const T *)rows, ix->n, (int)ix->dim, ix->ld, d_sums, s);
        };
        auto row_stats = [&]() {
            return cosine ? launch_bf16_row_stats<double>((const double *)rows, ix->d_mu, ix->n, (int)ix->dim, ix->ld, d_st, s)
                          : launch_bf16_row_stats<T>((const T *)rows, ix->d_mu, ix->n, (int)ix->dim, ix->ld, d_st, s);
        };
        auto pack = [&]() {
            return cosine ? launch_bf16_pack_corpus<double>((const double *)rows, ix->d_mu, ix->n, (int)ix->dim, ix->ld,
                                                            ix->d_img, d_w + 1, ix->bf16_ci, s)
                          : launch_bf16_pack_corpus<T>((const T *)rows, ix->d_mu, ix->n, (int)ix->dim, ix->ld, ix->d_img,
                                                       d_w + 1, ix->bf16_ci, s);
        };
        HIPCHK(hipMalloc((void **)&ix->d_mu, ix->dim * sizeof(float)));
        HIPCHK(col_sums());
        HIPCHK(launch_bf16_decide_mu(d_sums, ix->n, (int)ix->dim, false, ix->d_mu, d_w + 2, s));
        if (bf16_ci_candidate((int)ix->dim)) {
            HIPCHK(row_stats());
            PNCHK(read_words());
            const double *h_st = h_bw->st;
            const double bmean = h_st[2] / (double)ix->n, dmean = h_st[3] / (double)ix->n;
            ix->bf16_ci = h_st[0] > 0.0 && h_st[1] > 0.0 && h_st[0] <= 1.3 * bmean && h_st[1] <= 1.3 * dmean &&
                          h_st[0] < 1e30 && h_st[1] < 1e30;
            ix->bf16_bmax = h_st[0];
            ix->bf16_dmax = h_st[1];
        }
        HIPCHK(hipMalloc(&ix->d_img, bf16_image_bytes(ix->n, (int)ix->dim, ix->bf16_ci)));
        HIPCHK(pack());
        if (bf16_hw_state(ix->device).load() < 0)
            HIPCHK(launch_bf16_selftest((float *)((char *)d_bw + offsetof(BuildWords, selftest)), s));
    }
    PNCHK(read_words());
    if constexpr (sizeof(T) == 4)
        ix->mfma_ok = !cosine && (h_bw->w[0] == 0) && mfma_supported((int)ix->dim, ix->ld) && ix->n < 0xFFFFFFF0ull;
    if (try_bf16) {
        std::atomic<int> &hw = bf16_hw_state(ix->device);
        if (hw.load() < 0) hw.store(h_bw->selftest < kBf16SelftestLimit ? 1 : 0);
        ix->centered = h_bw->w[2] != 0;
        ix->bf16_ok = h_bw->w[1] == 0;
        if (hw.load() == 0) {
            ix->bf16_ok = false;
            (void)fail(PN_OK, "bf16 tier refused on device %d: the matrix core's accumulation error is %.4f of the 2^-13 "
                              "allowance the bound makes (limit %.2f)", ix->device, (double)h_bw->selftest,
                       (double)kBf16SelftestLimit);
        }
        if (!ix->bf16_ok) {
            (void)hipFree(ix->d_img);
            ix->d_img = nullptr;
            ix->bf16_ci = false;
        }
    }
    if (cosine) {
        if (nrm.p) PNCHK(seed_model_build<double>(ix, (const double *)nrm.p, s));
    } else {
        PNCHK(seed_model_build<T>(ix, (const T *)ix->d_pts, s));
    }
    return PN_OK;
}

static int validate_create(const void *points, size_t n_rows, size_t n_cols, ptrdiff_t row_stride,
                           ptrdiff_t col_stride, pn_index **out) {
    if (!out) return fail(PN_ERR_INVALID, "out is NULL");
    *out = nullptr;
    if (n_rows == 0) return fail(PN_ERR_EMPTY, "array is empty");
    if (n_cols > 1 && col_stride != 1) return fail(PN_ERR_NOT_CONTIGUOUS, "array is not contiguous in memory");
    if (n_cols == 0 && n_rows >= 2) return fail(PN_ERR_EMPTY_MATRIX, "empty matrix");
    if (!points && n_cols) return fail(PN_ERR_INVALID, "points is NULL");
    if (row_stride < 0) return fail(PN_ERR_UNSUPPORTED, "negative row stride");
    if (n_rows > 1 && (size_t)row_stride < n_cols && n_cols > 0 && row_stride != 0)
        return fail(PN_ERR_UNSUPPORTED, "overlapping rows (row_stride < n_cols)");
    if (n_rows >= 0xFFFFFFF0ull) return fail(PN_ERR_UNSUPPORTED, "more than 2^32-16 rows per index: shard the corpus");
    return PN_OK;
}

template <typename T>
static int create_from_host(const T *points, size_t n_rows, size_t n_cols, ptrdiff_t row_stride,
                            ptrdiff_t col_stride, int device, pn_index **out, int metric = 0) {
    PNCHK(validate_create(points, n_rows, n_cols, row_stride, col_stride, out));
    PNCHK(check_device(device));
    DeviceGuard g(device);
    if (!g.ok) return fail(PN_ERR_DEVICE, "hipSetDevice(%d) failed", device);
    pn_index *ix = new (std::nothrow) pn_index();
    if (!ix) return fail(PN_ERR_NOMEM, "host allocation failed");
    ix->device = device;
    ix->elem_bytes = (int)sizeof(T);
    ix->metric = metric;
    ix->n = n_rows;
    ix->dim = n_cols;
    ix->ld = pick_ld(n_cols);
    ix->n_pad = round_up(n_rows, kRowPad);
    int rc = PN_OK;
    T *d_tmp = nullptr;
    do {
        if (!(ix->stream = pooled_stream_acquire(device))) {
            rc = fail(PN_ERR_DEVICE, "hipStreamCreate failed");
            break;
        }
        const size_t tmp_elems = n_rows * (n_cols ? n_cols : 1);
        hipError_t e = hipMalloc((void **)&d_tmp, tmp_elems * sizeof(T));
        if (e != hipSuccess) { rc = fail(PN_ERR_NOMEM, "hipMalloc staging: %s", hipGetErrorString(e)); break; }
        if (n_cols) {
            if (n_rows == 1 || (size_t)row_stride == n_cols)
                e = hipMemcpy(d_tmp, points, tmp_elems * sizeof(T), hipMemcpyHostToDevice);
            else if (row_stride == 0) {
                for (size_t r = 0; r < n_rows && e == hipSuccess; ++r)
                    e = hipMemcpy(d_tmp + r * n_cols, points, n_cols * sizeof(T), hipMemcpyHostToDevice);
            } else
                e = hipMemcpy2D(d_tmp, n_cols * sizeof(T), points, (size_t)row_stride * sizeof(T),
// ... 61 lines not shown
    }
    if (rc != PN_OK) {
        pn_index_destroy(ix);
        return rc;
    }
    *out = ix;
    return PN_OK;
}
extern "C" int pn_index_create_device_f32(const float *d_points, size_t n_rows, size_t n_cols, size_t row_stride,
                                          int device, void *stream, pn_index **out) {
    return create_from_device<float>(d_points, n_rows, n_cols, row_stride, device, stream, out);
}
extern "C" int pn_index_create_device_f64(const double *d_points, size_t n_rows, size_t n_cols, size_t row_stride,
                                          int device, void *stream, pn_index **out) {
    return create_from_device<double>(d_points, n_rows, n_cols, row_stride, device, stream, out);
}

static void handle_wait(const pn_index *ix, bool all) {
    std::vector<hipEvent_t> evs;
    {
        std::lock_guard<std::mutex> lk(ix->sh.mu);
        for (Workspace *ws : (all ? ix->sh.all_ws : ix->sh.free_ws))
            if (ws->in_flight && ws->done) evs.push_back(ws->done);
    }
    for (hipEvent_t e : evs) (void)hipEventSynchronize(e);
}

extern "C" void pn_index_destroy(pn_index *ix) {
    if (!ix) return;
    DeviceGuard g(ix->device);
    handle_wait(ix, true);
    if (ix->stream) (void)hipStreamSynchronize(ix->stream);
    for (Workspace *ws : ix->sh.all_ws) {
        for (DevBuf &b : *ws) b.release();
        ws->free_retired();
        for (hipEvent_t e : ws->ev_r)
            if (e) (void)hipEventDestroy(e);
        if (ws->pin_in) (void)hipHostFree(ws->pin_in);
        if (ws->pin_out) (void)hipHostFree(ws->pin_out);
        if (ws->done) (void)hipEventDestroy(ws->done);
        pooled_stream_release(ix->device, ws->stream);
        delete ws;
    }
    for (CallRec &r : ix->sh.recs) {
        for (hipEvent_t e : r.ev)
            if (e) (void)hipEventDestroy(e);
        if (r.done) (void)hipEventDestroy(r.done);
        if (r.h_nflag) (void)hipHostFree(r.h_nflag);
    }
    if (ix->d_pts) (void)hipFree(ix->d_pts);
    if (ix->d_img) (void)hipFree(ix->d_img);
    if (ix->d_mu) (void)hipFree(ix->d_mu);
    if (ix->d_smodel) (void)hipFree(ix->d_smodel);
    if (ix->d_norm) (void)hipFree(ix->d_norm);
    if (ix->d_cnorm) (void)hipFree(ix->d_cnorm);
    if (ix->d_stats) (void)hipFree(ix->d_stats);
    pooled_stream_release(ix->device, ix->stream);
    if (HostTree *t = ix->sh.tree.load()) host_tree_free(t);
    delete ix;
}

static int ws_acquire(const pn_index *ix, hipStream_t *s, bool own_stream, Workspace **out) {
    Workspace *ws = nullptr;
    {
        std::lock_guard<std::mutex> lk(ix->sh.mu);
        if (!ix->sh.free_ws.empty()) {
            ws = ix->sh.free_ws.back();
            ix->sh.free_ws.pop_back();
        }
    }
    if (!ws) {
        ws = new (std::nothrow) Workspace();
        if (!ws) return fail(PN_ERR_NOMEM, "host allocation failed");
        if (hipEventCreateWithFlags(&ws->done, hipEventDisableTiming) != hipSuccess) {
            delete ws;
            return fail(PN_ERR_DEVICE, "workspace creation failed: %s", hipGetErrorString(hipGetLastError()));
        }
        std::lock_guard<std::mutex> lk(ix->sh.mu);
        ix->sh.all_ws.push_back(ws);
    }
    if (own_stream) {
        if (!ws->stream && !(ws->stream = pooled_stream_acquire(ix->device))) {
            std::lock_guard<std::mutex> lk(ix->sh.mu);
            ix->sh.free_ws.push_back(ws);
            return fail(PN_ERR_DEVICE, "workspace stream creation failed: %s", hipGetErrorString(hipGetLastError()));
        }
        *s = ws->stream;
    }
    if (!ws->retired.empty() && (!ws->in_flight || hipEventQuery(ws->done) == hipSuccess)) ws->free_retired();
    if (ws->in_flight && ws->last_stream != *s) {
        if (hipStreamWaitEvent(*s, ws->done, 0) != hipSuccess) {
            std::lock_guard<std::mutex> lk(ix->sh.mu);
            ix->sh.free_ws.push_back(ws);
            return fail(PN_ERR_DEVICE, "hipStreamWaitEvent failed");
        }
    }
    *out = ws;
    return PN_OK;
}
static void ws_release(const pn_index *ix, Workspace *ws, hipStream_t s) {
    ws->in_flight = hipEventRecord(ws->done, s) == hipSuccess;
    if (!ws->in_flight) (void)hipStreamSynchronize(s);
    ws->last_stream = s;
    std::lock_guard<std::mutex> lk(ix->sh.mu);
    ix->sh.free_ws.push_back(ws);
}
// ... 146 lines not shown
    out->bf16_eligible = ix->bf16_ok ? 1 : 0;
    out->bf16_layout = !ix->bf16_ok ? 0 : ix->bf16_ci ? 2 : 1;
    out->seed_model = ix->sm_ok ? 1 : 0;
    return PN_OK;
}

static int set_piece(pn_index *ix, PieceFamily family, int64_t value, const char *bad) {
    if (value < 0) return fail(PN_ERR_INVALID, "%s", bad);
    ix->piece[family] = (uint64_t)value;
    return PN_OK;
}
extern "C" int pn_index_set_option(pn_index *ix, int option, int64_t value) {
    if (!ix) return fail(PN_ERR_INVALID, "index is NULL");
    std::lock_guard<std::mutex> lk(ix->sh.mu);
    switch (option) {
        case PN_OPT_ENGINE:
            if (value < PN_ENGINE_AUTO || value > PN_ENGINE_BF16) return fail(PN_ERR_INVALID, "bad engine %lld", (long long)value);
            if (ix->metric == 1 && value == PN_ENGINE_MFMA)
                return fail(PN_ERR_UNSUPPORTED, "a Cosine index is served by the bf16 filter or the exact scan");
            if (value == PN_ENGINE_BF16 && !ix->bf16_ok)
                return fail(PN_ERR_UNSUPPORTED, "the bf16 filter cannot serve this index (D > 4096, fewer than 64 rows or out-of-range values)");
            if (value == PN_ENGINE_MFMA && !ix->mfma_ok)
                return fail(PN_ERR_UNSUPPORTED, "the MFMA filter cannot serve this index (f64, non-finite norms or unsupported shape)");
            ix->engine = (int)value;
            ix->sh.bf16_level = 0;
            return PN_OK;
        case PN_OPT_SEGMENTS:
            if (value < 0 || value > 4096) return fail(PN_ERR_INVALID, "bad segment count");
            ix->opt_segments = (int)value;
            return PN_OK;
        case PN_OPT_INDEX_BASE: ix->index_base = (uint64_t)value; return PN_OK;
        case PN_OPT_PROFILE: ix->profile = value < 0 ? 0 : value > 2 ? 2 : (int)value; return PN_OK;
        case PN_OPT_FILTER_SLOTS:
            if (value < 0 || value > 960) return fail(PN_ERR_INVALID, "bad filter slot count");
            ix->filter_slots = (int)value;
            return PN_OK;
        case PN_OPT_MFMA_STRUCTURE:
            if (value == 1) return fail(PN_ERR_INVALID, "structure 1 (the (query tile x segment) grid) was retired in round 4");
            if (value < 0 || value > 3) return fail(PN_ERR_INVALID, "bad structure");
            ix->mfma_structure = (int)value;
            return PN_OK;
        case PN_OPT_SHARED_THRESHOLDS:
            if (value < 0 || value > 4096) return fail(PN_ERR_INVALID, "bad shared-threshold rank");
            ix->shared_tau = (int)value;
            return PN_OK;
        case PN_OPT_BF16_WAVES:
            if (value != 0 && value != 4 && value != 8 && value != 16) return fail(PN_ERR_INVALID, "bad wave count (0, 4, 8 or 16)");
            ix->bf16_waves = (int)value;
            return PN_OK;
        case PN_OPT_SEED_MODEL:
            if (value != 0 && value != 1) return fail(PN_ERR_INVALID, "bad seed-model switch (0 or 1)");
            ix->seed_model = (int)value;
            return PN_OK;
        case PN_OPT_DBSCAN_PIECE: return set_piece(ix, kPieceDbscan, value, "bad DBSCAN piece size");
        case PN_OPT_MST_BATCH:
            if (value < 0) return fail(PN_ERR_INVALID, "bad MST batch size");
            ix->mst_batch = (uint64_t)value;
            return PN_OK;
        case PN_OPT_OPTICS_PIECE: return set_piece(ix, kPieceOptics, value, "bad OPTICS piece size");
        case PN_OPT_KDE_PIECE: return set_piece(ix, kPieceKde, value, "bad KDE piece size");
        case PN_OPT_MS_PIECE: return set_piece(ix, kPieceMs, value, "bad mean shift piece size");
        case PN_OPT_KMEANS_FILTER:
            if (value < 0 || value > 2) return fail(PN_ERR_INVALID, "bad k-means filter choice %lld", (long long)value);
            ix->kmeans_filter = (int)value;
            return PN_OK;
        default: return fail(PN_ERR_INVALID, "unknown option %d", option);
    }
}

extern "C" int pn_index_get_stats(const pn_index *ix, pn_stats *out, int reset) {
    if (!ix || !out) return fail(PN_ERR_INVALID, "NULL argument");
    DeviceGuard g(ix->device);
    if (!g.ok) return fail(PN_ERR_DEVICE, "hipSetDevice(%d) failed", ix->device);
    handle_wait(ix, false);
    std::lock_guard<std::mutex> lk(ix->sh.mu);
    recs_collect(ix, true);
    unsigned long long h[kPnStatWords] = {0};
    if (ix->d_stats) HIPCHK(hipMemcpy(h, ix->d_stats, sizeof h, hipMemcpyDeviceToHost));
    *out = ix->sh.stats;
    out->fallback_queries += h[0];
    for (int i = 0; i < kPnStatSlots; ++i) {
        out->candidates += h[4 + 2 * i];
        out->evaluations += h[5 + 2 * i];
    }
    if (reset) {
        ix->sh.stats = pn_stats{};
        if (ix->d_stats) HIPCHK(hipMemset(ix->d_stats, 0, sizeof h));
    }
    return PN_OK;
}

static int pick_cap(size_t kp) {
    const int caps[] = {128, 256, 512, 1024};
    for (int c : caps)
        if ((size_t)c >= kp + 64) return c;
    return 0;
}

struct ScanPlan {
    int nseg;
    size_t seg_len;
};

static ScanPlan plan_segments(size_t n, size_t q_tiles, int cap, int forced, size_t min_seg_rows, size_t max_entries,
                              size_t target_wgs = 2048, bool round_down = false) {
    size_t max_seg = max_entries / (size_t)cap;
// ... 259 lines not shown
        for (int j = kSeedModelGrid - 1; j >= 0; --j) {
            const size_t rho = (size_t)16 << j;
            std::nth_element(a, a + (ptrdiff_t)rho, a + (ptrdiff_t)hi);
            gridv[q * kSeedModelGrid + (size_t)j] = a[rho];
            ok = ok && std::isfinite(a[rho]);
            hi = rho;
        }
        if (!ok) return;
        qmean[q] = c0 - 2.0 * mean;
        qsd[q] = std::sqrt(var);
    };
    {
        constexpr size_t NT = 8;
        std::vector<std::thread> pool;
        bool threaded = true;
        try {
            for (size_t t = 0; t < NT; ++t)
                pool.emplace_back([&, t] {
                    for (size_t q = t; q < NQ; q += NT) one_query(q);
                });
        } catch (...) {
            threaded = false;
        }
        const size_t started = pool.size();
        for (std::thread &th : pool) th.join();
        if (!threaded)
            for (size_t t = started; t < NT; ++t)
                for (size_t q = t; q < NQ; q += NT) one_query(q);
    }
    for (size_t q = 0; q < NQ; ++q) used += qsd[q] > 0.0 ? 1u : 0u;
    if (used < NQ * 3 / 4) return PN_OK;
    for (int j = 0; j < kSeedModelGrid; ++j) {
        double zs = 0.0;
        for (size_t q = 0; q < NQ; ++q)
            if (qsd[q] > 0.0) zs += (qmean[q] - (double)gridv[q * kSeedModelGrid + (size_t)j]) / qsd[q];
        ix->sm_zgrid[j] = zs / (double)used;
    }
    const double z64 = ix->sm_zgrid[2];
    double ls = 0.0, lss = 0.0;
    for (size_t q = 0; q < NQ; ++q) {
        if (!(qsd[q] > 0.0)) continue;
        const float S = (float)(qmean[q] - z64 * qsd[q]);
        const float *a = &all[q * (size_t)NSEG * per];
        size_t cnt_below = 0;
        for (size_t e = 0; e <= top_rank; ++e) cnt_below += a[e] < S ? 1u : 0u;
        if (cnt_below > 0) cnt_below -= 1;
        const double l = std::log(((double)cnt_below + 0.5) / 64.0);
        ls += l;
        lss += l * l;
    }
    const double lm = ls / (double)used, lv = lss / (double)used - lm * lm;
    ix->sm_c0 = c0;
    ix->sm_v0 = v0;
    ix->sm_sigma = std::sqrt(lv > 0.0 ? lv : 0.0);
    bool mono = true;
    for (int j = 1; j < kSeedModelGrid; ++j) mono = mono && ix->sm_zgrid[j] < ix->sm_zgrid[j - 1];
    if (plan_knobs().debug)
        std::fprintf(stderr, "[pn seed model] build: device part %.2f ms, host part %.2f ms\n", t_dev, ms_since(t_begin) - t_dev);
    if (plan_knobs().debug)
        std::fprintf(stderr, "[pn seed model] n %zu dim %d: z at ranks 16..1024 = %.3f %.3f %.3f %.3f %.3f %.3f %.3f, log-rank "
                             "error at rank 64: mean %.3f sigma %.3f; c0 %.6g v0 %.6g\n",
                     ix->n, dim, ix->sm_zgrid[0], ix->sm_zgrid[1], ix->sm_zgrid[2], ix->sm_zgrid[3], ix->sm_zgrid[4],
                     ix->sm_zgrid[5], ix->sm_zgrid[6], lm, ix->sm_sigma, c0, v0);
    if (!mono || !(ix->sm_zgrid[kSeedModelGrid - 1] > 0.5) || !(ix->sm_sigma <= kSeedModelSigma)) return PN_OK;
    HIPCHK(hipMalloc((void **)&ix->d_smodel, h_model.size() * sizeof(float)));
    HIPCHK(hipMemcpyAsync(ix->d_smodel, h_model.data(), h_model.size() * sizeof(float), hipMemcpyHostToDevice, s));
    HIPCHK(hipStreamSynchronize(s));
    ix->sm_ok = true;
    return PN_OK;
}

struct Bf16Plan {
    Bf16Grid grid;
    Bf16Pass main_pass;
    Bf16Kernel main_kernel;
    int kp, cap, scout_max;
    bool ok;
    bool shared_scout;
    int scout_tiles, seed_rank;
    bool wide;
    int per_tile;
    int n_refresh, sh_rank;
    int first_eval;
    bool model_seed;
    double model_z;
};
static void plan_seed_model(const pn_index *ix, Bf16Plan &p, double R, size_t kout, bool eligible) {
    p.model_seed = false;
    p.model_z = 0.0;
    if (!eligible || !ix->sm_ok || ix->seed_model == 0 || ix->sh.seed_model_off.load(std::memory_order_relaxed) ||
        kout > (plan_knobs().model_kmax ? plan_knobs().model_kmax : (size_t)128) || ix->n < 100000)
        return;
    const double sig = ix->sm_sigma > 0.05 ? ix->sm_sigma : 0.05;
    double rho_t = (R + 5.5 * std::sqrt(R)) * std::exp(4.0 * sig) * std::pow(1.5, (double)ix->sh.seed_model_widen.load(std::memory_order_relaxed));
    if (plan_knobs().model_rank > 0.0) rho_t = plan_knobs().model_rank;
    if (rho_t < 16.0) rho_t = 16.0;
    const double top_rank = (double)(16u << (kSeedModelGrid - 1));
    if (rho_t > top_rank || rho_t * 50.0 > (double)ix->n) return;
    const double x = std::log2(rho_t / 16.0);
    int j = (int)x;
    if (j > kSeedModelGrid - 2) j = kSeedModelGrid - 2;
    const double f = x - (double)j;
    p.model_z = ix->sm_zgrid[j] * (1.0 - f) + ix->sm_zgrid[j + 1] * f + plan_knobs().model_dz;
    p.model_seed = p.model_z > 0.5 && p.model_z < 12.0;
}
static Bf16Plan bf16_plan_wide(const pn_index *ix, size_t nq_pad, size_t kout, int level) {
    Bf16Plan p{};
    p.wide = true;
    p.main_kernel = Bf16Kernel::Wide;
    const size_t q_tiles = nq_pad / 256, r_tiles = (ix->n + 255) / 256;
    const size_t n_cu = (size_t)ix->n_cu;
    auto eff_of = [&](size_t c) {
        const double rounds = (double)(q_tiles * c) / (double)n_cu;
        return rounds <= 1.0 ? rounds : rounds / std::ceil(rounds);
    };
    size_t c_max = 1;
    double best_eff = eff_of(1);
    for (size_t c = 2; c <= 32; ++c) {
        if (r_tiles / c < 8) break;
        if (ix->opt_segments > 0 && 2 * c > (size_t)ix->opt_segments) break;
        c_max = c;
// ... 151 lines not shown
    if (level == 0 && ix->filter_slots == 0 && kp > 16.0 && kp < 32.0) {
        const double per2 = 2.0 * R / (double)(per_tile > (size_t)split ? per_tile : (size_t)split);
        const double v = per2 + n_sigma * std::sqrt(per2) + 3.0;
        kp = v < 32.0 ? (v > kp ? v : kp) : 32.0;
    }
    p.kp = (int)std::ceil(kp);
    p.ok = level < 2 && p.kp + 32 <= 256;
    p.cap = p.ok ? bf16_cap_for(p.kp) : 0;
    p.grid = bf16_grid(ix->n, nq_pad, (int)n_wg, split);
    const double sm = (double)r_tiles / (10.0 * R);
    p.scout_max = sm > 64.0 ? 64 : (int)sm;
    p.shared_scout = false;
    if (p.ok && level == 0 && ix->filter_slots == 0 && p.grid.aligned && per_tile >= 2) {
        const size_t run_len = r_tiles / per_tile;
        double lam_target = R / 27.0 > 1.2 ? R / 27.0 : 1.2;
        if (plan_knobs().scout_lambda > 0.0) lam_target = plan_knobs().scout_lambda;
        double t = lam_target * (double)r_tiles / (R * (double)per_tile);
        if (t > (double)run_len / 19.0) t = (double)run_len / 19.0;
        p.scout_tiles = (int)t;
        if (p.scout_tiles < 1 && run_len >= 8) p.scout_tiles = 1;
        while (p.scout_tiles >= 4 || (p.scout_tiles >= 1 && run_len < 64)) {
            const double lam = R * (double)p.scout_tiles * (double)per_tile / (double)r_tiles;
            double term = std::exp(-lam), cdf = term;
            int rank = 1;
            while (1.0 - cdf > 1e-7 && rank < 96) {
                term *= lam / (double)rank;
                cdf += term;
                ++rank;
            }
            p.seed_rank = rank < 5 ? 5 : rank;
            p.shared_scout = p.seed_rank < 96 && p.seed_rank <= 6 * p.grid.nseg;
            if (p.shared_scout || p.scout_tiles < 8) break;
            p.scout_tiles = p.scout_tiles * 3 / 4;
        }
    }
    p.first_eval = (int)std::ceil(R);
    plan_seed_model(ix, p, R, kout, p.shared_scout || (!plan_knobs().model_shared_only && p.ok && level == 0 && ix->filter_slots == 0));
    p.n_refresh = 0;
    p.sh_rank = 0;
    if (p.shared_scout && p.grid.aligned && ix->shared_tau != 0 && !(p.model_seed && ix->shared_tau == 1) &&
        bf16_shared_supported(p.cap)) {
        const int slots = 2 * ix->n_cu - p.grid.n_wg;
        const int rank = ix->shared_tau >= 2 ? ix->shared_tau : (int)std::ceil(R + 5.5 * std::sqrt(R));
        size_t sh_min_run = 320;
        if (plan_knobs().sh_min_run) sh_min_run = plan_knobs().sh_min_run;
        if (slots >= 4 && rank <= 256 && rank < p.grid.nseg * p.cap && r_tiles / per_tile >= sh_min_run) {
            p.n_refresh = slots > 64 ? 64 : slots;
            p.sh_rank = rank;
        }
    }
    p.main_pass = p.shared_scout || (p.model_seed && ix->d_smodel) ? Bf16Pass::Seeded : Bf16Pass::SelfScout;
    p.main_kernel = bf16_main_kernel(p.grid, p.cap, p.main_pass, p.n_refresh > 0,
                                     bf16_image_bytes(ix->n, (int)ix->dim, ix->bf16_ci), 2 * ix->n_cu, ix->bf16_waves);
    if (plan_knobs().debug)
        fprintf(stderr, "bf16_plan: n %zu q_tiles %zu k %zu R %.0f: n_wg %d per_tile %zu split %d nseg %d kp %d cap %d aligned %d "
                        "shared_scout %d scout_tiles %d seed_rank %d scout_max %d n_refresh %d sh_rank %d model_seed %d z %.3f\n",
                ix->n, q_tiles, kout, R, p.grid.n_wg, per_tile, split, p.grid.nseg, p.kp, p.cap, (int)p.grid.aligned, (int)p.shared_scout,
                p.scout_tiles, p.seed_rank, p.scout_max, p.n_refresh, p.sh_rank, (int)p.model_seed, p.model_z);
    return p;
}
struct MfmaPlan {
    bool ok = false;
    int kp = 0;
    int cap = 0;
    int n_wg = 0, nseg = 0;
    bool two_per_cu = false;
};
static MfmaPlan mfma_plan(const pn_index *ix, size_t kout, size_t nq_pad) {
    MfmaPlan p;
    const size_t kp = mfma_slots(ix, kout, nq_pad);
    if (kp + 64 > 256) return p;
    const bool hbm_ok = (ix->mfma_structure == 0 || ix->mfma_structure == 3);
    if (kp > 30 && !(hbm_ok && ix->ld <= 128)) return p;
    p.kp = (int)kp;
    p.cap = (int)round_up(kp, 32);
    p.two_per_cu = hbm_ok;
    const size_t q_tiles = nq_pad / 128, r_tiles = (ix->n + 63) / 64;
    size_t n_wg = (size_t)(p.two_per_cu ? 2 * ix->n_cu : ix->n_cu);
    size_t cap_wg = q_tiles * 32;
    const size_t by_work = (q_tiles * r_tiles + 31) / 32;
    if (by_work < cap_wg) cap_wg = by_work;
    if (cap_wg < 1) cap_wg = 1;
    if (n_wg > cap_wg) n_wg = cap_wg;
    int nseg = mfma_v2_max_segments(q_tiles, (int)n_wg);
    while (nseg > 2 && select_rerank_lds_bytes(nseg, p.cap, p.kp, ix->dim, sizeof(float)) > kSelectRerankLdsMax) --nseg;
    if (select_rerank_lds_bytes(nseg, p.cap, p.kp, ix->dim, sizeof(float)) > kSelectRerankLdsMax) return p;
    if (nseg < mfma_v2_max_segments(q_tiles, (int)n_wg)) n_wg = (size_t)(nseg - 1) * q_tiles;
    p.n_wg = (int)n_wg;
    p.nseg = mfma_v2_max_segments(q_tiles, p.n_wg);
    p.ok = true;
    return p;
}

static int run_mfma(const pn_index *ix, Workspace &ws, const MfmaPlan &plan, const float *Qp, size_t nq, size_t nq_pad,
                    size_t kout, uint64_t *d_idx, float *d_dist, size_t out_stride, hipStream_t s, CallRec *rec) {
    if (!plan.ok) return fail(PN_ERR_UNSUPPORTED, "MFMA tier cannot serve k = %zu", kout);
    const size_t kp = (size_t)plan.kp;
    const int cap = plan.cap, n_wg = plan.n_wg;
    const bool two_per_cu = plan.two_per_cu;
    PNCHK(ws.w_qnorm.ensure(nq_pad * sizeof(float)));
    uint32_t *d_misc = (uint32_t *)ws.w_misc.p;
    HIPCHK(launch_row_norms_f32(Qp, nq_pad, nq, (int)ix->dim, ix->ld, mfma_alpha(ix->dim), (float *)ws.w_qnorm.p,
                                d_misc + 1, s));
    const size_t cells = (size_t)plan.nseg * nq_pad;
    const size_t slots = cells * (size_t)cap;
    PNCHK(ws.w_keys.ensure(slots * sizeof(uint32_t)));
// ... 6 lines not shown
    HIPCHK(hipMemsetAsync(ws.w_cnt.p, 0, cells * sizeof(uint32_t), s));
    HIPCHK(hipMemsetD32Async((hipDeviceptr_t)ws.w_tau.p, (int)0xFF800000u, cells, s));
    const bool prof = rec && rec->prof;
    if (prof) {
        HIPCHK(hipEventRecord(rec->ev[0], s));
        rec->hot = true;
    }
    uint32_t *gcand = nullptr;
    if (two_per_cu) {
        PNCHK(ws.w_sel.ensure(mfma_v2_gcand_bytes(n_wg, (int)kp)));
        gcand = (uint32_t *)ws.w_sel.p;
    }
    HIPCHK(launch_mfma_filter_v2_f32((const float *)ix->d_pts, ix->d_norm, ix->n, ix->ld, Qp, (const float *)ws.w_qnorm.p,
                                     ix->ld, (int)kp, cb, n_wg, gcand, s));
    if (prof) HIPCHK(hipEventRecord(rec->ev[1], s));
    HIPCHK(launch_select_rerank<float>(cb, (const float *)ix->d_pts, ix->n, (int)ix->dim, ix->ld, Qp, (int)nq, ix->ld,
                                       (int)kout, ix->index_base, d_idx, d_dist, out_stride, (uint32_t *)ws.w_flags.p, d_misc,
                                       nullptr, nullptr, (uint32_t *)ws.w_gsel.p, ix->d_stats, s, 0, plan.kp));
    return PN_OK;
}

template <typename T>
static int run_bf16(const pn_index *ix, Workspace &ws, const Bf16Plan &plan, const T *Qp, size_t nq, size_t nq_pad,
                    size_t kout, uint64_t *d_idx, T *d_dist, size_t out_stride, hipStream_t s, CallRec *rec,
                    const T *d_q_raw = nullptr, size_t q_stride = 0, const T *qnorm = nullptr) {
    if (!plan.ok) return fail(PN_ERR_UNSUPPORTED, "bf16 tier cannot serve k = %zu", kout);
    const bool cosine = ix->metric == 1;
    if (cosine && (!qnorm || d_q_raw)) return fail(PN_ERR_INVALID, "Cosine tier: query norms missing");
    const int cap = plan.cap, nseg = plan.grid.nseg;
    const size_t kp = (size_t)plan.kp;
    const size_t cells = (size_t)nseg * nq_pad, slots = cells * (size_t)cap;
    PNCHK(ws.w_bq.ensure(bf16_query_bytes(nq_pad, (int)ix->dim, ix->bf16_ci)));
    PNCHK(ws.w_qn.ensure(nq_pad * sizeof(double)));
    PNCHK(ws.w_qbad.ensure(nq_pad * sizeof(uint32_t)));
    PNCHK(ws.w_keys.ensure(slots * 2 * sizeof(uint32_t)));
    PNCHK(ws.w_cnt.ensure(cells * sizeof(uint32_t)));
    PNCHK(ws.w_tau.ensure(cells * sizeof(uint32_t)));
    PNCHK(ws.w_flags.ensure(nq_pad * sizeof(uint32_t)));
    PNCHK(ws.w_gsel.ensure(nq_pad * sizeof(uint32_t)));
    uint32_t *d_misc = (uint32_t *)ws.w_misc.p;
    const bool model = plan.model_seed && ix->d_smodel;
    Bf16SeedModel smd{};
    if (model) {
        PNCHK(ws.w_seed.ensure(nq_pad * sizeof(uint32_t)));
        smd.m1 = ix->d_smodel;
        smd.a = ix->d_smodel + ix->ld;
        smd.b = ix->d_smodel + 2 * ix->ld;
        smd.c0 = ix->sm_c0;
        smd.v0 = ix->sm_v0;
        smd.z = plan.model_z;
        smd.seed_out = (uint32_t *)ws.w_seed.p;
        if (rec) rec->model_seed = true;
    }
    if (cosine) {
        PNCHK(ws.w_qnrm.ensure(nq_pad * ix->ld * sizeof(double)));
        HIPCHK(launch_cos_normalize_rows<T>(Qp, nq, nq_pad, (int)ix->dim, ix->ld, (double *)ws.w_qnrm.p, ix->ld, nullptr,
                                            true, s));
        HIPCHK(launch_bf16_pack_queries<double>((const double *)ws.w_qnrm.p, ix->d_mu, nq, nq_pad, (int)ix->dim, ix->ld,
                                                ws.w_bq.p, (double *)ws.w_qn.p, (uint32_t *)ws.w_qbad.p, ix->bf16_ci,
                                                ix->bf16_bmax, ix->bf16_dmax, s, (double *)nullptr, 0, nullptr,
                                                model ? &smd : nullptr));
    } else if (d_q_raw)
        HIPCHK(launch_bf16_pack_queries(d_q_raw, ix->d_mu, nq, nq_pad, (int)ix->dim, q_stride, ws.w_bq.p,
                                        (double *)ws.w_qn.p, (uint32_t *)ws.w_qbad.p, ix->bf16_ci, ix->bf16_bmax,
                                        ix->bf16_dmax, s, const_cast<T *>(Qp), ix->ld, d_misc, model ? &smd : nullptr));
    else
        HIPCHK(launch_bf16_pack_queries(Qp, ix->d_mu, nq, nq_pad, (int)ix->dim, ix->ld, ws.w_bq.p, (double *)ws.w_qn.p,
                                        (uint32_t *)ws.w_qbad.p, ix->bf16_ci, ix->bf16_bmax, ix->bf16_dmax, s,
                                        (T *)nullptr, 0, nullptr, model ? &smd : nullptr));
    CandBuf cb{ws.w_keys.p, (uint32_t *)ws.w_keys.p + 1, (uint32_t *)ws.w_cnt.p, ws.w_tau.p, nq_pad, nseg, cap, 2};
    cb.final_keep = bf16_cell_max((int)kp, cap, nseg, bf16_is_wide((int)ix->dim));
    if (!plan.grid.aligned) {
        HIPCHK(hipMemsetAsync(ws.w_cnt.p, 0, cells * sizeof(uint32_t), s));
        HIPCHK(hipMemsetD32Async((hipDeviceptr_t)ws.w_tau.p, (int)0xFF800000u, cells, s));
    }
    const bool prof = rec && rec->prof;
    if (prof) {
        HIPCHK(hipEventRecord(rec->ev[0], s));
        rec->hot = true;
        rec->two_launches = plan.shared_scout && !model;
    }
    Bf16Launch main{ix->d_img, ix->n, (int)ix->dim, ix->bf16_ci, ws.w_bq.p, (int)kp, cb, plan.grid, plan.main_pass, plan.main_kernel};
    auto launch = [&](const Bf16Launch &l) { return plan.wide ? launch_bf16_wide_filter(l, s) : launch_bf16_filter(l, s); };
    if (plan.shared_scout) {
        const size_t words = cells * 2 * (size_t)bf16_scout_list();
        PNCHK(ws.w_lists.ensure(words * sizeof(float)));
        PNCHK(ws.w_seed.ensure(nq_pad * sizeof(uint32_t)));
        if (!plan.grid.aligned)
            HIPCHK(hipMemsetD32Async((hipDeviceptr_t)ws.w_lists.p, (int)0x7F800000u, words, s));
        if (!model) {
            if (!plan.wide && bf16_seed_in_kernel(nseg) && plan.seed_rank <= bf16_scout_list())
                main.seed = Bf16SeedLists{(const float *)ws.w_lists.p, (uint32_t)plan.seed_rank, (uint32_t)nq, (uint32_t *)ws.w_seed.p};
            Bf16Launch scout = main;
            scout.pass = Bf16Pass::ScoutOnly;
            scout.kernel = plan.wide ? Bf16Kernel::Wide : Bf16Kernel::Four;
            scout.scout_tiles = plan.scout_tiles;
            scout.scout_out = (float *)ws.w_lists.p;
            if (plan.n_refresh == 0) scout.seed.reset();
            HIPCHK(launch(scout));
            if (!main.seed)
                HIPCHK(launch_bf16_seed((const float *)ws.w_lists.p, nq_pad, nseg, plan.seed_rank, (uint32_t *)ws.w_seed.p, s, nq));
        }
        if (plan.n_refresh > 0) {
            const void *pc_before = ws.w_pcnt.p;
            PNCHK(ws.w_pcnt.ensure(cells * sizeof(uint32_t)));
            if (ws.w_pcnt.p != pc_before) ws.sh_nseg = 0;
            if (ws.sh_nseg != (size_t)nseg || ws.sh_nq_pad != nq_pad) {
                HIPCHK(hipMemsetAsync(ws.w_pcnt.p, 0, cells * sizeof(uint32_t), s));
                ws.sh_nseg = (size_t)nseg;
                ws.sh_nq_pad = nq_pad;
            }
            ws.sh_epoch = ws.sh_epoch % 4095u + 1u;
            main.refresh = Bf16Refresh{(uint32_t *)ws.w_pcnt.p, d_misc + 8, ws.sh_epoch, (uint32_t)plan.sh_rank, plan.n_refresh};
        }
    }
    if (plan.main_pass == Bf16Pass::Seeded)
        main.tau = (const uint32_t *)ws.w_seed.p;
    else
        main.scout_tiles = plan.scout_max;
    HIPCHK(launch(main));
    if (prof) HIPCHK(hipEventRecord(rec->ev[1], s));
    if (cosine) {
        HIPCHK(launch_select_rerank<T>(cb, (const T *)ix->d_pts, ix->n, (int)ix->dim, ix->ld, Qp, (int)nq, ix->ld, (int)kout,
                                       ix->index_base, d_idx, d_dist, out_stride, (uint32_t *)ws.w_flags.p, d_misc,
                                       (const double *)ws.w_qn.p, (const uint32_t *)ws.w_qbad.p, (uint32_t *)ws.w_gsel.p,
                                       ix->d_stats, s, plan.first_eval, cb.final_keep, (const T *)ix->d_cnorm, qnorm));
        return PN_OK;
    }
    HIPCHK(launch_select_rerank<T>(cb, (const T *)ix->d_pts, ix->n, (int)ix->dim, ix->ld, Qp, (int)nq, ix->ld, (int)kout,
                                   ix->index_base, d_idx, d_dist, out_stride, (uint32_t *)ws.w_flags.p, d_misc,
                                   (const double *)ws.w_qn.p, (const uint32_t *)ws.w_qbad.p, (uint32_t *)ws.w_gsel.p,
                                   ix->d_stats, s, plan.first_eval, cb.final_keep));
    return PN_OK;
}

template <typename T>
static int query_enqueue(const pn_index *ix, Workspace &ws, const T *d_q, size_t nq, size_t q_cols, size_t q_stride,
                         size_t kout, uint64_t *d_idx, T *d_dist, size_t out_stride, hipStream_t s) {
    const size_t dim_eff = q_cols < ix->dim ? q_cols : ix->dim;
    int level;
    uint64_t call_id;
    {
        std::lock_guard<std::mutex> lk(ix->sh.mu);
        recs_collect(ix, false);
        level = ix->sh.bf16_level;
        call_id = ix->sh.next_call++;
// ... 3168 lines not shown
```

petal-neighbors_amd/csrc/pn_internal.h:

```cpp
#pragma once
#include <hip/hip_runtime.h>

#include <atomic>
#include <cstddef>
#include <cstdint>
#include <cstdlib>
#include <optional>
#include <type_traits>

#include "bf16_launch.h"

namespace pn {

inline bool debug_plan() {
    static const bool on = getenv("PN_DEBUG_PLAN") != nullptr;
    return on;
}

struct LdsAttrOnce {
    std::atomic<uint64_t> done{0};
    hipError_t ensure(const void *kern, size_t bytes) {
        int dev = 0;
        hipError_t e = hipGetDevice(&dev);
        if (e != hipSuccess) return e;
// ... 324 lines not shown
hipError_t launch_pack_rows(const T *src, size_t n, size_t cols, size_t row_stride, T *dst, size_t n_pad, size_t ld,
                            hipStream_t s);
hipError_t launch_fill_uniform_f32(float *out, uint64_t count, uint64_t seed, uint64_t first, hipStream_t s);
hipError_t launch_row_norms_f32(const float *X, size_t n_pad, size_t n, int dim, size_t ld, float alpha,
                                float *norm_out, uint32_t *nonfinite_flag, hipStream_t s);

bool mfma_supported(int dim, size_t ld);
int mfma_v2_max_segments(size_t q_tiles, int n_wg);
size_t mfma_v2_gcand_bytes(int n_wg, int kp);
int mfma_v2_cap_for(int kp);
hipError_t launch_mfma_filter_v2_f32(const float *P, const float *pnorm, size_t n, size_t ldp, const float *Q,
                                     const float *qnorm, size_t ldq, int kp, const CandBuf &cb, int n_wg,
                                     uint32_t *gcand, hipStream_t s);

hipError_t launch_mfma_radius_f32(const float *P, const float *pnorm, size_t n, size_t ldp, const float *Q,
                                  const float *qnorm, size_t nq_pad, float tau_excl, uint32_t cap, uint32_t *rcnt,
                                  uint32_t *ridx, int n_wg, hipStream_t s);
hipError_t launch_radius_check_f32(const uint32_t *rcnt, const uint32_t *ridx, size_t nq_pad, int nseg, uint32_t cap,
                                   const float *P, size_t ldp, const float *Q, int nq, int dim, float r,
                                   uint32_t *kept, uint32_t *nkept, uint32_t *overflow, int ridx_stride,
                                   uint32_t *over_q , hipStream_t s,
                                   float *kept_dist = nullptr);
hipError_t launch_radius_gather(const uint32_t *kept, const uint32_t *nkept, const uint64_t *offsets, int nq,
                                size_t kept_stride, uint64_t index_base, uint64_t *out, hipStream_t s,
                                const void *kept_dist = nullptr, void *out_dist = nullptr, int dist_bytes = 0);

bool bf16_supported(int dim);
bool bf16_is_wide(int dim);
int bf16_ks_for(int dim, bool ci);
bool bf16_ci_candidate(int dim);
size_t bf16_image_bytes(size_t n, int dim, bool ci);
size_t bf16_query_bytes(size_t nq_pad, int dim, bool ci);
int bf16_cap_for(int kp);
int bf16_query_tile();
template <typename T>
hipError_t launch_bf16_column_sums(const T *P, size_t n, int dim, size_t ld, double *sums, hipStream_t s);
hipError_t launch_bf16_selftest(float *out, hipStream_t s);
hipError_t launch_bf16_decide_mu(const double *sums, size_t n, int dim, bool never, float *mu, uint32_t *words, hipStream_t s);
template <typename T>
hipError_t launch_bf16_row_stats(const T *P, const float *mu, size_t n, int dim, size_t ld, double *out4,
                                 hipStream_t s);
template <typename T>
hipError_t launch_cos_normalize_rows(const T *X, size_t n_valid, size_t n_out, int dim, size_t ld_in, double *out,
                                     size_t ld_out, uint32_t *bad, bool nan_rows, hipStream_t s);
template <typename T>
hipError_t launch_bf16_pack_corpus(const T *P, const float *mu, size_t n, int dim, size_t ld, void *img,
                                   uint32_t *bad, bool ci, hipStream_t s);
bool bf16_pack_fused_supported(int dim);
struct Bf16SeedModel {
    const float *m1 = nullptr, *a = nullptr, *b = nullptr;
    double c0 = 0.0, v0 = 0.0, z = 0.0;
    uint32_t *seed_out = nullptr;
};
template <typename T>
hipError_t launch_bf16_pack_queries(const T *Q, const float *mu, size_t nq, size_t nq_pad, int dim, size_t ld,
                                    void *B, double *qn, uint32_t *qbad, bool ci, double bmax, double dmax,
                                    hipStream_t s, T *Qp = nullptr, size_t ldq = 0, uint32_t *misc = nullptr,
                                    const Bf16SeedModel *sm = nullptr);
template <typename T>
hipError_t launch_bf16_column_moments(const T *P, const float *mu, size_t n, int dim, size_t ld, double *out, hipStream_t s);
struct Bf16SeedLists {
    const float *lists;
    uint32_t rank, nq;
    uint32_t *words;
};
struct Bf16Refresh {
    uint32_t *pcnt, *done;
    uint32_t epoch, rank;
    int n_refresh;
};
struct Bf16Launch {
    const void *img;
    size_t n;
    int dim;
    bool ci;
    const void *B;
    int kp;
    CandBuf cb;
    Bf16Grid grid;
    Bf16Pass pass;
    Bf16Kernel kernel;
    int scout_tiles = 0;
    const uint32_t *tau = nullptr;
    float *scout_out = nullptr;
    std::optional<Bf16SeedLists> seed;
    std::optional<Bf16Refresh> refresh;
};
bool bf16_seed_in_kernel(int nseg);
bool bf16_shared_supported(int cap);
hipError_t launch_bf16_filter(const Bf16Launch &l, hipStream_t s);
hipError_t launch_bf16_wide_filter(const Bf16Launch &l, hipStream_t s);
int bf16_scout_list();
int bf16_cell_max(int kp, int cap, int nseg, bool wide);
hipError_t launch_bf16_seed(const float *lists, size_t nq_pad, int nseg, int rank, uint32_t *out, hipStream_t s,
                            size_t nq = 0);
hipError_t launch_bf16_radius_tau(const double *qn, size_t nq_pad, double tau_r, uint32_t *out, hipStream_t s);

template <typename T>
hipError_t launch_bf16_radii_tau(const double *qn, const T *radii, size_t nq, size_t nq_pad, int dim, bool cosine,
                                 uint32_t *out, uint32_t *qbad, hipStream_t s);
hipError_t launch_radii_add_listed(const uint32_t *nsel, unsigned long long *stats, hipStream_t s);
hipError_t launch_bf16_bound(const void *img, const void *B, size_t n_rows, size_t nq, int dim, float *out, bool ci,
                             hipStream_t s);

}

#include "host_tree.h"

struct pn_index;
namespace pn {
int set_error(int code, const char *fmt, ...);
int query_device_strided_f32(const pn_index *ix, const float *d_q, size_t nq, size_t q_cols, size_t q_stride, size_t k,
                             uint64_t *d_idx, float *d_dist, size_t out_stride, hipStream_t s);
int query_device_strided_f64(const pn_index *ix, const double *d_q, size_t nq, size_t q_cols, size_t q_stride, size_t k,
                             uint64_t *d_idx, double *d_dist, size_t out_stride, hipStream_t s);
const void *index_rows(const pn_index *ix, size_t *ld);
int merge_topk_device_keys_f32(const uint64_t *pi, const float *pd, size_t np, size_t is, size_t ds, size_t nq, size_t kp,
                               size_t ko, uint64_t *oi, float *od, int device, void *stream, bool signed_keys);
int merge_topk_device_keys_f64(const uint64_t *pi, const double *pd, size_t np, size_t is, size_t ds, size_t nq, size_t kp,
                               size_t ko, uint64_t *oi, double *od, int device, void *stream, bool signed_keys);
}
```

Baseline: 5.213 million queries/s.

## Add int8 MFMA candidate filter with rigorous bounds for bf16 k-NN engine

Measured after the change: 7.700 million queries/s, median of 6. 47.7% higher.

```diff
diff --git a/bindings/rust/src/ffi.rs b/bindings/rust/src/ffi.rs
--- a/bindings/rust/src/ffi.rs
+++ b/bindings/rust/src/ffi.rs
@@ -10,6 +10,7 @@
 pub const PN_KDE_EPANECHNIKOV: c_int = 2;
 pub const PN_KDE_EXPONENTIAL: c_int = 3;
 pub const PN_KDE_LINEAR: c_int = 4;
+pub const PN_OPT_I8_FILTER: c_int = 17;
 
 #[repr(C)]
 pub struct pn_index {
diff --git a/include/petal_mi355x.h b/include/petal_mi355x.h
--- a/include/petal_mi355x.h
+++ b/include/petal_mi355x.h
@@ -45,7 +45,8 @@
     PN_OPT_OPTICS_PIECE = 13,
     PN_OPT_KDE_PIECE = 14,
     PN_OPT_MS_PIECE = 15,
-    PN_OPT_KMEANS_FILTER = 16
+    PN_OPT_KMEANS_FILTER = 16,
+    PN_OPT_I8_FILTER = 17
 };
 
 enum {
diff --git a/petal-neighbors_amd/_lib.py b/petal-neighbors_amd/_lib.py
--- a/petal-neighbors_amd/_lib.py
+++ b/petal-neighbors_amd/_lib.py
@@ -22,6 +22,7 @@
 PN_OPT_KDE_PIECE = 14
 PN_OPT_MS_PIECE = 15
 PN_OPT_KMEANS_FILTER = 16
+PN_OPT_I8_FILTER = 17
 PN_KDE_GAUSSIAN, PN_KDE_TOPHAT, PN_KDE_EPANECHNIKOV, PN_KDE_EXPONENTIAL, PN_KDE_LINEAR = 0, 1, 2, 3, 4
 PN_RADIUS_SORTED = 1
 PN_SELF_INCLUDE = 2
diff --git a/petal-neighbors_amd/csrc/bf16_filter.hip b/petal-neighbors_amd/csrc/bf16_filter.hip
--- a/petal-neighbors_amd/csrc/bf16_filter.hip
+++ b/petal-neighbors_amd/csrc/bf16_filter.hip
@@ -56,6 +56,7 @@
 __host__ __device__ inline int bf16_steps(int dim) { return (bf16_extra_col(dim) + 5 + 15) / 16; }
 __host__ __device__ inline bool bf16_ci_dim(int dim) { return dim >= 17 && dim <= 128 && bf16_steps(dim) > (dim + 15) / 16; }
 __host__ __device__ inline int bf16_steps_for(int dim, bool ci) { return ci ? (dim + 15) / 16 : bf16_steps(dim); }
+__host__ __device__ inline int i8_steps(int dim) { return dim <= 64 ? 2 : (dim + 31) / 32; }
 
 __device__ __forceinline__ uint16_t bf_rne(float x) {
     const uint32_t u = __float_as_uint(x);
@@ -75,6 +76,13 @@
 __device__ __forceinline__ float f_up_signed(double x) {
     float f = (float)x;
     if ((double)f < x) f = (f >= 0.0f) ? __uint_as_float(__float_as_uint(f) + 1u) : __uint_as_float(__float_as_uint(f) - 1u);
+    return f;
+}
+__device__ __forceinline__ float f_down_signed(double x) {
+    float f = (float)x;
+    if ((double)f > x)
+        f = (__float_as_uint(f) & 0x80000000u) ? __uint_as_float(__float_as_uint(f) + 1u)
+                                               : (f == 0.0f ? -1.4e-45f : __uint_as_float(__float_as_uint(f) - 1u));
     return f;
 }
 __device__ __forceinline__ uint16_t bf_trunc(float x) { return (uint16_t)(__float_as_uint(x) >> 16); }
@@ -278,6 +286,106 @@
 }
 
 template <typename T>
+__global__ __launch_bounds__(256) void i8_absmax_kernel(const T *__restrict__ P, const float *__restrict__ m, size_t n, int dim,
+                                                        size_t ld, double *__restrict__ out) {
+    const int sub = (int)(threadIdx.x & 7);
+    double a = 0.0;
+    const size_t stride = (size_t)gridDim.x * blockDim.x;
+    for (size_t t = (size_t)blockIdx.x * blockDim.x + threadIdx.x; t < n * 8; t += stride) {
+        const T *src = P + (t >> 3) * ld;
+        for (int k = sub; k < dim; k += 8) a = fmax(a, fabs((double)src[k] - (double)m[k]));
+    }
+    for (int d = 32; d > 0; d >>= 1) a = fmax(a, __shfl_xor(a, d));
+    __shared__ double red[4];
+    if ((threadIdx.x & 63) == 0) red[threadIdx.x >> 6] = a;
+    __syncthreads();
+    if (threadIdx.x == 0) {
+        a = fmax(fmax(red[0], red[1]), fmax(red[2], red[3]));
+        atomicMax(reinterpret_cast<unsigned long long *>(out), (unsigned long long)__double_as_longlong(a));
+    }
+}
+template <typename T>
+__global__ __launch_bounds__(256) void i8_pack_corpus_kernel(const T *__restrict__ P, const float *__restrict__ m, size_t n,
+                                                             int dim, size_t ld, int KS8, double step, char *__restrict__ img,
+                                                             size_t n_rows_img, double *__restrict__ st) {
+    const size_t t = (size_t)blockIdx.x * blockDim.x + threadIdx.x;
+    const size_t r = t >> 3;
+    const int sub = (int)(t & 7);
+    const int CP = 2 * KS8 + 1, CH = 4 * KS8, c0 = sub * CH;
+    const bool in_rows = r < n;
+    double pn = 0.0, en = 0.0;
+    uint32_t b[16];
+#pragma unroll
+    for (int i = 0; i < 16; ++i) {
+        b[i] = 0u;
+        const int k = c0 + i;
+        if (i < CH && k < dim && in_rows) {
+            const double c = (double)P[r * ld + k] - (double)m[k];
+            double z = rint(c / step);
+            z = z > 127.0 ? 127.0 : z < -127.0 ? -127.0 : z;
+            const double e = c - step * z;
+            b[i] = (uint32_t)(-(int)z) & 0xFFu;
+            pn += c * c;
+            en += e * e;
+        }
+    }
+#pragma unroll
+    for (int d = 1; d < 8; d <<= 1) {
+        pn += __shfl_xor(pn, d);
+        en += __shfl_xor(en, d);
+    }
+    char *row = img + r * (size_t)CP * 16;
+#pragma unroll
+    for (int i = 0; i < 16; i += 4)
+        if (i + 4 <= CH) *reinterpret_cast<uint32_t *>(row + c0 + i) = b[i] | (b[i + 1] << 8) | (b[i + 2] << 16) | (b[i + 3] << 24);
+    const size_t rr = r % kBP;
+    if (sub == 1 && rr >= 16) {
+        typedef uint32_t u4_ __attribute__((ext_vector_type(4)));
+        *reinterpret_cast<u4_ *>(row + (size_t)(CP - 1) * 16) = u4_{0u, 0u, 0u, 0u};
+    }
+    if (sub == 0) {
+        const size_t tl = r / kBP;
+        int *slot = reinterpret_cast<int *>(img + ((tl * kBP + rr / 4) * (size_t)CP + (size_t)(CP - 1)) * 16) + (rr % 4);
+        const double np = floor(pn / kUp / (2.0 * step * step));
+        *slot = in_rows ? (int)(np < 1073741824.0 ? np : 1073741824.0) : (1 << 30);
+    }
+    double em = 0.0, pm = 0.0, es = 0.0, ps = 0.0;
+    if (sub == 0 && in_rows) {
+        em = en;
+        pm = pn;
+        es = sqrt(en);
+        ps = sqrt(pn);
+    }
+    for (int d = 32; d > 0; d >>= 1) {
+        em = fmax(em, __shfl_xor(em, d));
+        pm = fmax(pm, __shfl_xor(pm, d));
+        es += __shfl_xor(es, d);
+        ps += __shfl_xor(ps, d);
+    }
+    __shared__ double red[4][4];
+    const int wave = (int)(threadIdx.x >> 6);
+    if ((threadIdx.x & 63) == 0) {
+        red[wave][0] = em;
+        red[wave][1] = pm;
+        red[wave][2] = es;
+        red[wave][3] = ps;
+    }
+    __syncthreads();
+    if (threadIdx.x == 0) {
+        for (int w = 1; w < 4; ++w) {
+            em = fmax(em, red[w][0]);
+            pm = fmax(pm, red[w][1]);
+            es += red[w][2];
+            ps += red[w][3];
+        }
+        atomicMax(reinterpret_cast<unsigned long long *>(st), (unsigned long long)__double_as_longlong(em));
+        atomicMax(reinterpret_cast<unsigned long long *>(st + 1), (unsigned long long)__double_as_longlong(pm));
+        atomicAdd(st + 2, es);
+        atomicAdd(st + 3, ps);
+    }
+}
+
+template <typename T>
 __global__ void bf16_row_stats_kernel(const T *__restrict__ P, const float *__restrict__ mu, size_t n, int dim,
                                       size_t ld, double *__restrict__ out) {
     const size_t r = (size_t)blockIdx.x * blockDim.x + threadIdx.x;
@@ -463,7 +571,7 @@
                                           size_t nq_pad, int dim, size_t ld, int KS, uint16_t *__restrict__ B,
                                           double *__restrict__ qn, uint32_t *__restrict__ qbad, int ci, double bmax,
                                           double dmax, T *__restrict__ Qp, size_t ldq,
-                                          uint32_t *__restrict__ misc, Bf16SeedModel sm) {
+                                          uint32_t *__restrict__ misc, Bf16SeedModel sm, Bf16I8Query i8) {
     const size_t t = (size_t)blockIdx.x * blockDim.x + threadIdx.x;
     const size_t q = t >> 3;
     const int sub = (int)(t & 7);
@@ -605,14 +713,60 @@
 #pragma unroll
     for (int i = 0; i < 18; ++i)
         if (i < CH) dst[i] = v[i];
+    double qn_q = ok ? s / kUp : 0.0;
+    if (ci && ok) qn_q -= (sqrt(hn) * kUp * bmax + sqrt(en) * kUp * dmax) * kUp;
+    bool i8_ok = true;
+    if (i8.Q) {
+        const int K8 = 32 * i8_steps(dim);
+        double qm = 0.0, q8h = 0.0, q8e = 0.0, t1 = 0.0;
+        uint32_t b8[18];
+#pragma unroll
+        for (int i = 0; i < 18; ++i) {
+            b8[i] = 0u;
+            const int k = c0 + i;
+            if (i < CH && k < dim && q < nq && ok) {
+                const double c = (double)xf[i] - (double)i8.m[k];
+                const double lim = 127.0 * i8.s, b = c > lim ? lim : c < -lim ? -lim : c, t = c - b;
+                double z = rint(b / i8.s);
+                z = z > 127.0 ? 127.0 : z < -127.0 ? -127.0 : z;
+                const double e = b - i8.s * z;
+                b8[i] = (uint32_t)(int)z & 0xFFu;
+                qm += b * b + t * t;
+                t1 += fabs(t);
+                q8h += (i8.s * z) * (i8.s * z);
+                q8e += e * e;
+            }
+        }
+#pragma unroll
+        for (int d = 1; d < 8; d <<= 1) {
+            qm += __shfl_xor(qm, d);
+            q8h += __shfl_xor(q8h, d);
+            q8e += __shfl_xor(q8e, d);
+            t1 += __shfl_xor(t1, d);
+        }
+        const double slack = 2.0 * (sqrt(q8h) * kUp * i8.e_max + sqrt(q8e) * kUp * i8.p_max) * kUp;
+        double kd = qm / kUp - slack - qn_q;
+        kd -= 2.0 * i8.s * i8.s + fabs(kd) * (1.0 / 4194304.0);
+        i8_ok = kd > -1.0e37 && kd < 1.0e37;
+        signed char *row8 = static_cast<signed char *>(i8.Q) + q * (size_t)K8;
+        if (CH % 4 == 0) {
+#pragma unroll
+            for (int i = 0; i < 18; i += 4)
+                if (i + 4 <= CH)
+                    *reinterpret_cast<uint32_t *>(row8 + c0 + i) =
+                        i8_ok ? b8[i] | (b8[i + 1] << 8) | (b8[i + 2] << 16) | (b8[i + 3] << 24) : 0u;
+        } else {
+#pragma unroll
+            for (int i = 0; i < 18; ++i)
+                if (i < CH) row8[c0 + i] = (signed char)(i8_ok ? b8[i] : 0u);
+        }
+        for (int k = K + sub; k < K8; k += 8) row8[k] = 0;
+        if (sub == 0) i8.kappa[q] = i8_ok && ok ? f_down_signed(kd) : 0.0f;
+        if (sub == 0 && q < nq && ok && i8_ok && 4.0 * t1 * 127.0 * i8.s > slack) *i8.outside = i8.epoch;
+    }
     if (sub == 0) {
-        if (ci) {
-            const double eq = (sqrt(hn) * kUp * bmax + sqrt(en) * kUp * dmax) * kUp;
-            qn[q] = ok ? s / kUp - eq : 0.0;
-        } else {
-            qn[q] = ok ? s / kUp : 0.0;
-        }
-        qbad[q] = ok ? 0u : 1u;
+        qn[q] = qn_q;
+        qbad[q] = ok && i8_ok ? 0u : 1u;
         if (sm.seed_out) {
             float sd = __uint_as_float(0xFF800000u);
             if (q < nq && ok) {
@@ -802,10 +956,68 @@
     }
 }
 
-template <int CP>
-__device__ __forceinline__ f32x16 bf_cinit(const char *tb, int blk, int h) {
-    typedef float f32x4_ __attribute__((ext_vector_type(4)));
-    f32x16 c;
+typedef int i32x4 __attribute__((ext_vector_type(4)));
+typedef int i32x16 __attribute__((ext_vector_type(16)));
+struct BfOpBf16 {
+    typedef bf16x8 frag;
+    typedef f32x16 acc;
+    typedef float elem;
+    typedef float vec4 __attribute__((ext_vector_type(4)));
+    struct Args {};
+    struct Keys {
+        __device__ __forceinline__ void load(const Args &, size_t, int, bool) {}
+    };
+    static constexpr const char *name = "pair";
+    static constexpr bool thr_is_tau = true;
+    static __device__ __forceinline__ acc mfma(frag a, frag b, acc c) { return __builtin_amdgcn_mfma_f32_32x32x16_bf16(a, b, c, 0, 0, 0); }
+    static __device__ __forceinline__ elem min2(elem a, elem b) { return fminf(a, b); }
+    static __device__ __forceinline__ elem zero() { return 0.0f; }
+    static __device__ __forceinline__ elem big() { return 3.0e38f; }
+    static __device__ __forceinline__ elem none() { return __uint_as_float(0x7F800000u); }
+    static __device__ __forceinline__ const f32x16 &keys(const acc &a, const Keys &, int) { return a; }
+    static __device__ __forceinline__ elem thr(float tau, const Keys &, int) { return tau; }
+};
+struct BfOpI8 {
+    typedef i32x4 frag;
+    typedef i32x16 acc;
+    typedef int elem;
+    typedef int vec4 __attribute__((ext_vector_type(4)));
+    struct Args {
+        const float *kappa;
+        float c;
+        const uint32_t *outside;
+        uint32_t epoch;
+    };
+    struct Keys {
+        float c, kap[2];
+        __device__ __forceinline__ void load(const Args &a, size_t q0, int jq, bool active) {
+            c = a.c;
+            kap[0] = active ? a.kappa[q0 + jq] : 0.0f;
+            kap[1] = active ? a.kappa[q0 + 32 + jq] : 0.0f;
+        }
+    };
+    static constexpr const char *name = "i8pair";
+    static constexpr bool thr_is_tau = false;
+    static __device__ __forceinline__ acc mfma(frag a, frag b, acc c) { return __builtin_amdgcn_mfma_i32_32x32x32_i8(a, b, c, 0, 0, 0); }
+    static __device__ __forceinline__ elem min2(elem a, elem b) { return a < b ? a : b; }
+    static __device__ __forceinline__ elem zero() { return 0; }
+    static __device__ __forceinline__ elem big() { return 1 << 30; }
+    static __device__ __forceinline__ elem none() { return 1 << 30; }
+    static __device__ __forceinline__ f32x16 keys(const acc &a, const Keys &k, int blk) {
+        f32x16 v;
+#pragma unroll
+        for (int r = 0; r < 16; ++r) v[r] = __builtin_fmaf((float)a[r], k.c, k.kap[blk]);
+        return v;
+    }
+    static __device__ __forceinline__ elem thr(float tau, const Keys &k, int blk) {
+        const double x = ceil(((double)tau - (double)k.kap[blk]) / (double)k.c) + 1.0;
+        return (int)fmin(fmax(x, -1073741824.0), 1073741824.0);
+    }
+};
+template <int CP, typename OP = BfOpBf16>
+__device__ __forceinline__ typename OP::acc bf_cinit(const char *tb, int blk, int h) {
+    typedef typename OP::vec4 f32x4_;
+    typename OP::acc c;
 #pragma unroll
     for (int g = 0; g < 4; ++g) {
         const f32x4_ v = *reinterpret_cast<const f32x4_ *>(tb + ((blk * 8 + 2 * g + h) * CP + (CP - 1)) * 16);
@@ -821,52 +1033,62 @@
     static constexpr int at(int) { return -1; }
     __device__ __forceinline__ void operator()() const {}
 };
-template <int KS, bool CI, int CP, typename MID = BfNoMid>
-__device__ __forceinline__ void bf_chain_p(const char *arow, bf16x8 (&pre)[kLA], const bf16x8 (&b0)[KS],
-                                           const bf16x8 (&b1)[KS], f32x16 &c, f32x16 &w0, f32x16 &w1, f32x16 &r0,
-                                           f32x16 &r1, float &m0, float &m1, const char *narow, const char *ntb,
+template <int KS, bool CI, int CP, typename MID = BfNoMid, typename OP = BfOpBf16>
+struct BfChainP {
+static __device__ __forceinline__ void run(const char *arow, typename OP::frag (&pre)[kLA], const typename OP::frag (&b0)[KS],
+                                           const typename OP::frag (&b1)[KS], typename OP::acc &c, typename OP::acc &w0,
+                                           typename OP::acc &w1, typename OP::acc &r0, typename OP::acc &r1,
+                                           typename OP::elem &m0, typename OP::elem &m1, const char *narow, const char *ntb,
                                            int nblk, int h, MID mid = MID()) {
-    typedef float f32x4_ __attribute__((ext_vector_type(4)));
-    bf16x8 f[KS];
+    typedef typename OP::vec4 V4;
+    typedef typename OP::frag F;
+    typedef typename OP::acc A;
+    F f[KS];
 #pragma unroll
     for (int i = 0; i < kLA && i < KS; ++i) f[i] = pre[i];
-    f32x16 z, nc = c;
-#pragma unroll
-    for (int i = 0; i < 16; ++i) z[i] = 0.0f;
+    A z, nc = c;
+#pragma unroll
+    for (int i = 0; i < 16; ++i) z[i] = OP::zero();
 #pragma unroll
     for (int ks = 0; ks < KS; ++ks) {
         if (ks == MID::at(KS)) mid();
-        if (ks + kLA < KS) f[ks + kLA] = *reinterpret_cast<const bf16x8 *>(arow + 32 * (ks + kLA));
+        if (ks + kLA < KS) f[ks + kLA] = *reinterpret_cast<const F *>(arow + 32 * (ks + kLA));
 #pragma unroll
         for (int i = 0; i < kLA; ++i)
             if (ks == (KS - kLA + i > 0 ? KS - kLA + i : 0))
-                pre[i] = *reinterpret_cast<const bf16x8 *>(narow + 32 * (i < KS ? i : 0));
+                pre[i] = *reinterpret_cast<const F *>(narow + 32 * (i < KS ? i : 0));
         if (CI) {
 #pragma unroll
             for (int g = 0; g < 4; ++g)
                 if (ks == (KS - 4 + g > 0 ? KS - 4 + g : 0)) {
-                    const f32x4_ v =
-                        *reinterpret_cast<const f32x4_ *>(ntb + ((nblk * 8 + 2 * g + h) * CP + (CP - 1)) * 16);
+                    const V4 v = *reinterpret_cast<const V4 *>(ntb + ((nblk * 8 + 2 * g + h) * CP + (CP - 1)) * 16);
                     nc[4 * g + 0] = v[0];
                     nc[4 * g + 1] = v[1];
                     nc[4 * g + 2] = v[2];
                     nc[4 * g + 3] = v[3];
                 }
-            w0 = __builtin_amdgcn_mfma_f32_32x32x16_bf16(f[ks], b0[ks], ks ? w0 : c, 0, 0, 0);
-            w1 = __builtin_amdgcn_mfma_f32_32x32x16_bf16(f[ks], b1[ks], ks ? w1 : c, 0, 0, 0);
+            w0 = OP::mfma(f[ks], b0[ks], ks ? w0 : c);
+            w1 = OP::mfma(f[ks], b1[ks], ks ? w1 : c);
             if (ks == 0) asm volatile("" ::"v"(c));
         } else {
-            w0 = __builtin_amdgcn_mfma_f32_32x32x16_bf16(f[ks], b0[ks], ks ? w0 : z, 0, 0, 0);
-            w1 = __builtin_amdgcn_mfma_f32_32x32x16_bf16(f[ks], b1[ks], ks ? w1 : z, 0, 0, 0);
+            w0 = OP::mfma(f[ks], b0[ks], ks ? w0 : z);
+            w1 = OP::mfma(f[ks], b1[ks], ks ? w1 : z);
         }
 #pragma unroll
         for (int i = 16 * ks / KS; i < 16 * (ks + 1) / KS; ++i) {
-            m0 = i ? fminf(m0, r0[i]) : r0[0];
-            m1 = i ? fminf(m1, r1[i]) : r1[0];
+            m0 = i ? OP::min2(m0, r0[i]) : r0[0];
+            m1 = i ? OP::min2(m1, r1[i]) : r1[0];
         }
         __builtin_amdgcn_sched_barrier(0);
     }
     c = nc;
+}
+};
+template <int KS, bool CI, int CP>
+__device__ __forceinline__ void bf_chain_p(const char *arow, bf16x8 (&pre)[kLA], const bf16x8 (&b0)[KS], const bf16x8 (&b1)[KS],
+                                           f32x16 &c, f32x16 &w0, f32x16 &w1, f32x16 &r0, f32x16 &r1, float &m0, float &m1,
+                                           const char *narow, const char *ntb, int nblk, int h) {
+    BfChainP<KS, CI, CP>::run(arow, pre, b0, b1, c, w0, w1, r0, r1, m0, m1, narow, ntb, nblk, h);
 }
 
 constexpr uint32_t kShPeriod = 32;
@@ -1834,11 +2056,23 @@
     }
 };
 
-template <int KS, bool CI, int STAG>
+template <typename OP>
+__device__ __forceinline__ void bf_pair_slow(const typename OP::acc &a, float &tau, typename OP::elem &th,
+                                             const typename OP::Keys &kc, int blk, uint32_t &cnt, uint32_t row0, int h, int jq,
+                                             int lane, uint32_t kp, uint2 *ceq, uint2 *ce_blk, uint32_t &ns BF_DBG_ARG) {
+    const float before = tau;
+    bf_slow<1, false>(OP::keys(a, kc, blk), 0.0f, tau, cnt, row0, h, jq, lane, kp, ceq, ce_blk, ns BF_DBG_PASS);
+    if (OP::thr_is_tau || __any(tau != before)) th = OP::thr(tau, kc, blk);
+}
+template <int KS, bool CI, int STAG, typename OP>
 __device__ __forceinline__ void bf_pair_run(const char *__restrict__ img, char *tiles, uint32_t kp, uint32_t kfin, uint2 *__restrict__ cand,
                                             uint32_t *__restrict__ ccnt, uint32_t *__restrict__ ctau,
-                                            const bf16x8 (&b0)[KS], const bf16x8 (&b1)[KS], float tau0, float tau1,
-                                            uint32_t rt0, uint32_t rt1, size_t cell0, bool active, int wave, int lane) {
+                                            const typename OP::frag (&b0)[KS], const typename OP::frag (&b1)[KS], float tau0,
+                                            float tau1, const typename OP::Keys &kc, uint32_t rt0, uint32_t rt1, size_t cell0,
+                                            bool active, int wave, int lane) {
+    typedef typename OP::frag F;
+    typedef typename OP::acc A;
+    typedef typename OP::elem EL;
     constexpr int C = 2 * KS, CP = C + 1;
     constexpr uint32_t CAP = 64u;
     constexpr int TB = kBP * CP * 16;
@@ -1864,21 +2098,22 @@
     uint2 *ceq0 = ce_blk0 + (size_t)jq * CAP, *ceq1 = ce_blk1 + (size_t)jq * CAP;
     uint32_t ns = 0;
 
-    f32x16 a00, a01, a10, a11;
+    EL th0 = OP::thr(tau0, kc, 0), th1 = OP::thr(tau1, kc, 1);
+    A a00, a01, a10, a11;
 #pragma unroll
     for (int r = 0; r < 16; ++r) {
-        a00[r] = 3.0e38f;
-        a01[r] = 3.0e38f;
-        a10[r] = 3.0e38f;
-        a11[r] = 3.0e38f;
-    }
-    bf16x8 pre[kLA];
-    f32x16 cc = a00;
+        a00[r] = OP::big();
+        a01[r] = OP::big();
+        a10[r] = OP::big();
+        a11[r] = OP::big();
+    }
+    F pre[kLA];
+    A cc = a00;
     {
         const char *ar = tiles + (jq * CP + h) * 16;
 #pragma unroll
-        for (int i = 0; i < kLA; ++i) pre[i] = *reinterpret_cast<const bf16x8 *>(ar + 32 * (i < KS ? i : 0));
-        if (CI) cc = bf_cinit<CP>(tiles, 0, h);
+        for (int i = 0; i < kLA; ++i) pre[i] = *reinterpret_cast<const F *>(ar + 32 * (i < KS ? i : 0));
+        if (CI) cc = bf_cinit<CP, OP>(tiles, 0, h);
     }
     int cur = 0;
     for (uint32_t rt = rt0; rt < rt1; ++rt) {
@@ -1886,17 +2121,17 @@
         const char *tb = tiles + cur * TB;
         const char *arow0 = tb + (jq * CP + h) * 16;
         const char *arow1 = arow0 + 32 * CP * 16;
-        float m0, m1, p0, p1;
+        EL m0, m1, p0, p1;
         if (STAG == 2) BfPairMeet{ns}();
         if (STAG == 1)
-            bf_chain_p<KS, CI, CP>(arow0, pre, b0, b1, cc, a00, a01, a10, a11, m0, m1, arow1, tb, 1, h, BfPairMeet{ns});
+            BfChainP<KS, CI, CP, BfPairMeet, OP>::run(arow0, pre, b0, b1, cc, a00, a01, a10, a11, m0, m1, arow1, tb, 1, h, BfPairMeet{ns});
         else
-            bf_chain_p<KS, CI, CP>(arow0, pre, b0, b1, cc, a00, a01, a10, a11, m0, m1, arow1, tb, 1, h);
-        if (rt == rt0) { m0 = __uint_as_float(0x7F800000u); m1 = m0; }
-        if (__any(m0 < tau0 || m1 < tau1)) {
+            BfChainP<KS, CI, CP, BfNoMid, OP>::run(arow0, pre, b0, b1, cc, a00, a01, a10, a11, m0, m1, arow1, tb, 1, h);
+        if (rt == rt0) { m0 = OP::none(); m1 = m0; }
+        if (__any(m0 < th0 || m1 < th1)) {
             const uint32_t row0 = (rt - 1) * kBP + 32;
-            if (__any(m0 < tau0)) bf_slow<1, false>(a10, m0, tau0, cnt0, row0, h, jq, lane, kp, ceq0, ce_blk0, ns BF_DBG_PASS);
-            if (__any(m1 < tau1)) bf_slow<1, false>(a11, m1, tau1, cnt1, row0, h, jq, lane, kp, ceq1, ce_blk1, ns BF_DBG_PASS);
+            if (__any(m0 < th0)) bf_pair_slow<OP>(a10, tau0, th0, kc, 0, cnt0, row0, h, jq, lane, kp, ceq0, ce_blk0, ns BF_DBG_PASS);
+            if (__any(m1 < th1)) bf_pair_slow<OP>(a11, tau1, th1, kc, 1, cnt1, row0, h, jq, lane, kp, ceq1, ce_blk1, ns BF_DBG_PASS);
         }
         if (STAG == 0) {
             bf_wait_dma(ns);
@@ -1912,24 +2147,24 @@
         }
         const bool last = rt + 1 >= rt1;
         const char *ntb = last ? tb : tiles + nxt * TB;
-        bf_chain_p<KS, CI, CP>(arow1, pre, b0, b1, cc, a10, a11, a00, a01, p0, p1, ntb + (jq * CP + h) * 16, ntb, 0, h);
-        if (__any(p0 < tau0 || p1 < tau1)) {
+        BfChainP<KS, CI, CP, BfNoMid, OP>::run(arow1, pre, b0, b1, cc, a10, a11, a00, a01, p0, p1, ntb + (jq * CP + h) * 16, ntb, 0, h);
+        if (__any(p0 < th0 || p1 < th1)) {
             const uint32_t row0 = rt * kBP;
-            if (__any(p0 < tau0)) bf_slow<1, false>(a00, p0, tau0, cnt0, row0, h, jq, lane, kp, ceq0, ce_blk0, ns BF_DBG_PASS);
-            if (__any(p1 < tau1)) bf_slow<1, false>(a01, p1, tau1, cnt1, row0, h, jq, lane, kp, ceq1, ce_blk1, ns BF_DBG_PASS);
+            if (__any(p0 < th0)) bf_pair_slow<OP>(a00, tau0, th0, kc, 0, cnt0, row0, h, jq, lane, kp, ceq0, ce_blk0, ns BF_DBG_PASS);
+            if (__any(p1 < th1)) bf_pair_slow<OP>(a01, tau1, th1, kc, 1, cnt1, row0, h, jq, lane, kp, ceq1, ce_blk1, ns BF_DBG_PASS);
         }
         cur = nxt;
     }
     {
-        float m0 = a10[0], m1 = a11[0];
+        EL m0 = a10[0], m1 = a11[0];
 #pragma unroll
         for (int i = 1; i < 16; ++i) {
-            m0 = fminf(m0, a10[i]);
-            m1 = fminf(m1, a11[i]);
+            m0 = OP::min2(m0, a10[i]);
+            m1 = OP::min2(m1, a11[i]);
         }
         const uint32_t row0 = (rt1 - 1) * kBP + 32;
-        if (__any(m0 < tau0)) bf_slow<1, false>(a10, m0, tau0, cnt0, row0, h, jq, lane, kp, ceq0, ce_blk0, ns BF_DBG_PASS);
-        if (__any(m1 < tau1)) bf_slow<1, false>(a11, m1, tau1, cnt1, row0, h, jq, lane, kp, ceq1, ce_blk1, ns BF_DBG_PASS);
+        if (__any(m0 < th0)) bf_pair_slow<OP>(a10, tau0, th0, kc, 0, cnt0, row0, h, jq, lane, kp, ceq0, ce_blk0, ns BF_DBG_PASS);
+        if (__any(m1 < th1)) bf_pair_slow<OP>(a11, tau1, th1, kc, 1, cnt1, row0, h, jq, lane, kp, ceq1, ce_blk1, ns BF_DBG_PASS);
     }
     asm volatile("s_waitcnt vmcnt(0)" ::: "memory");
     auto final_compact = [&](uint2 *ce_blk, float &tau, uint32_t &cnt) {
@@ -1966,18 +2201,16 @@
     BF_DBG_FLUSH(lane);
 }
 
-template <int KS, bool CI>
-__global__ __launch_bounds__(512, 2) void bf16_filter_kernel_pair(const char *__restrict__ img, uint32_t n_tiles,
-                                                                  const u32x4 *__restrict__ Bq, uint32_t q_tiles,
-                                                                  uint32_t kp_keep, uint2 *__restrict__ cand,
-                                                                  uint32_t *__restrict__ ccnt,
-                                                                  uint32_t *__restrict__ ctau, size_t nq_pad,
-                                                                  const uint32_t *tau_init, BfShared sh) {
+template <int KS, bool CI, typename OP>
+__device__ __forceinline__ void bf_pair_kernel(unsigned char *smem_raw, const char *__restrict__ img, uint32_t n_tiles,
+                                               const u32x4 *__restrict__ Bq, uint32_t q_tiles, uint32_t kp_keep,
+                                               uint2 *__restrict__ cand, uint32_t *__restrict__ ccnt,
+                                               uint32_t *__restrict__ ctau, size_t nq_pad, const uint32_t *tau_init,
+                                               const BfShared &sh, const typename OP::Args &op_args) {
     const uint32_t kp = kp_keep & 0xFFFFu, keep_arg = kp_keep >> 16;
     const uint32_t kfin = keep_arg > kp ? keep_arg : kp;
     constexpr int CP = 2 * KS + 1;
     constexpr int TB = kBP * CP * 16;
-    extern __shared__ __attribute__((aligned(16))) unsigned char smem_raw[];
     char *tiles = reinterpret_cast<char *>(smem_raw);
     const int tid = threadIdx.x, lane = tid & 63;
     const int wave = __builtin_amdgcn_readfirstlane(tid >> 6);
@@ -1999,7 +2232,9 @@
     const size_t q0 = active ? (size_t)qt * kBQ + (size_t)(wave & 3) * 64 : 0;
     const size_t cell0 = (size_t)seg * nq_pad + q0;
 
-    bf16x8 b0[KS], b1[KS];
+    typename OP::frag b0[KS], b1[KS];
+    typename OP::Keys kc;
+    kc.load(op_args, q0, jq, active);
     float tau0 = __uint_as_float(0xFF800000u), tau1 = tau0;
     if (active) {
         const u32x4 *br0 = Bq + (q0 + jq) * (size_t)C + h;
@@ -2007,8 +2242,8 @@
 #pragma unroll
         for (int ks = 0; ks < KS; ++ks) {
             const u32x4 v0 = br0[2 * ks], v1 = br1[2 * ks];
-            b0[ks] = __builtin_bit_cast(bf16x8, v0);
-            b1[ks] = __builtin_bit_cast(bf16x8, v1);
+            b0[ks] = __builtin_bit_cast(typename OP::frag, v0);
+            b1[ks] = __builtin_bit_cast(typename OP::frag, v1);
         }
         if (sh.seed_lists) {
             const size_t ql = q0 + (size_t)lane;
@@ -2027,7 +2262,7 @@
         const u32x4 zero = {0u, 0u, 0u, 0u};
 #pragma unroll
         for (int ks = 0; ks < KS; ++ks) {
-            b0[ks] = __builtin_bit_cast(bf16x8, zero);
+            b0[ks] = __builtin_bit_cast(typename OP::frag, zero);
             b1[ks] = b0[ks];
         }
     }
@@ -2044,11 +2279,45 @@
     }
     __syncthreads();
     if (wave >= 4)
-        bf_pair_run<KS, CI, kPairStagger>(img, tiles, kp, kfin, cand, ccnt, ctau, b0, b1, tau0, tau1, rt0, rt1, cell0,
-                                          active, wave, lane);
+        bf_pair_run<KS, CI, kPairStagger, OP>(img, tiles, kp, kfin, cand, ccnt, ctau, b0, b1, tau0, tau1, kc, rt0, rt1,
+                                              cell0, active, wave, lane);
     else
-        bf_pair_run<KS, CI, 0>(img, tiles, kp, kfin, cand, ccnt, ctau, b0, b1, tau0, tau1, rt0, rt1, cell0, active, wave,
-                               lane);
+        bf_pair_run<KS, CI, 0, OP>(img, tiles, kp, kfin, cand, ccnt, ctau, b0, b1, tau0, tau1, kc, rt0, rt1, cell0, active,
+                                   wave, lane);
+}
+template <int KS, bool CI>
+__global__ __launch_bounds__(512, 2) void bf16_filter_kernel_pair(const char *__restrict__ img, uint32_t n_tiles,
+                                                                  const u32x4 *__restrict__ Bq, uint32_t q_tiles,
+                                                                  uint32_t kp_keep, uint2 *__restrict__ cand,
+                                                                  uint32_t *__restrict__ ccnt,
+                                                                  uint32_t *__restrict__ ctau, size_t nq_pad,
+                                                                  const uint32_t *tau_init, BfShared sh) {
+    extern __shared__ __attribute__((aligned(16))) unsigned char smem_raw[];
+    bf_pair_kernel<KS, CI, BfOpBf16>(smem_raw, img, n_tiles, Bq, q_tiles, kp_keep, cand, ccnt, ctau, nq_pad, tau_init, sh,
+                                     BfOpBf16::Args{});
+}
+template <int KS8>
+__global__ __launch_bounds__(512, 2) void i8_filter_kernel_pair(const char *__restrict__ img, uint32_t n_tiles,
+                                                                const u32x4 *__restrict__ Bq, uint32_t q_tiles,
+                                                                uint32_t kp_keep, uint2 *__restrict__ cand,
+                                                                uint32_t *__restrict__ ccnt, uint32_t *__restrict__ ctau,
+                                                                size_t nq_pad, const uint32_t *tau_init, BfShared sh,
+                                                                BfOpI8::Args op_args) {
+    extern __shared__ __attribute__((aligned(16))) unsigned char smem_raw[];
+    if (*op_args.outside == op_args.epoch) return;
+    bf_pair_kernel<KS8, true, BfOpI8>(smem_raw, img, n_tiles, Bq, q_tiles, kp_keep, cand, ccnt, ctau, nq_pad, tau_init, sh, op_args);
+}
+template <int KS>
+__global__ __launch_bounds__(512, 2) void bf16_pair_behind_i8_kernel(const char *__restrict__ img, uint32_t n_tiles,
+                                                                     const u32x4 *__restrict__ Bq, uint32_t q_tiles,
+                                                                     uint32_t kp_keep, uint2 *__restrict__ cand,
+                                                                     uint32_t *__restrict__ ccnt, uint32_t *__restrict__ ctau,
+                                                                     size_t nq_pad, const uint32_t *tau_init, BfShared sh,
+                                                                     const uint32_t *outside, uint32_t epoch) {
+    extern __shared__ __attribute__((aligned(16))) unsigned char smem_raw[];
+    if (*outside != epoch) return;
+    bf_pair_kernel<KS, true, BfOpBf16>(smem_raw, img, n_tiles, Bq, q_tiles, kp_keep, cand, ccnt, ctau, nq_pad, tau_init, sh,
+                                       BfOpBf16::Args{});
 }
 
 template <int M, bool RAD>
@@ -2511,21 +2780,50 @@
 template hipError_t launch_bf16_pack_corpus<float>(const float *, const float *, size_t, int, size_t, void *, uint32_t *, bool, hipStream_t);
 template hipError_t launch_bf16_pack_corpus<double>(const double *, const float *, size_t, int, size_t, void *, uint32_t *, bool, hipStream_t);
 
+int i8_ks_for(int dim) { return i8_steps(dim); }
+size_t i8_image_bytes(size_t n, int dim) { return (n + kBP - 1) / kBP * kBP * (size_t)(2 * i8_steps(dim) + 1) * 16; }
+size_t i8_query_bytes(size_t nq_pad, int dim) { return nq_pad * (size_t)(32 * i8_steps(dim)); }
+template <typename T>
+hipError_t launch_i8_absmax(const T *P, const float *m, size_t n, int dim, size_t ld, double *out, hipStream_t s) {
+    if (dim < 1 || dim > 128 || n < 1) return hipErrorInvalidValue;
+    const size_t blocks = (n * 8 + 255) / 256;
+    hipLaunchKernelGGL(i8_absmax_kernel<T>, dim3((unsigned)(blocks < 2048 ? blocks : 2048)), dim3(256), 0, s, P, m, n, dim, ld, out);
+    return hipGetLastError();
+}
+template <typename T>
+hipError_t launch_i8_pack_corpus(const T *P, const float *m, size_t n, int dim, size_t ld, double step, void *img, double *st,
+                                 hipStream_t s) {
+    if (dim < 1 || dim > 128 || n < 1 || !(step > 0.0)) return hipErrorInvalidValue;
+    const size_t rows = (n + kBP - 1) / kBP * kBP;
+    hipLaunchKernelGGL(i8_pack_corpus_kernel<T>, dim3((unsigned)(rows * 8 / 256)), dim3(256), 0, s, P, m, n, dim, ld,
+                       i8_steps(dim), step, static_cast<char *>(img), rows, st);
+    return hipGetLastError();
+}
+template hipError_t launch_i8_absmax<float>(const float *, const float *, size_t, int, size_t, double *, hipStream_t);
+template hipError_t launch_i8_absmax<double>(const double *, const float *, size_t, int, size_t, double *, hipStream_t);
+template hipError_t launch_i8_pack_corpus<float>(const float *, const float *, size_t, int, size_t, double, void *, double *, hipStream_t);
+template hipError_t launch_i8_pack_corpus<double>(const double *, const float *, size_t, int, size_t, double, void *, double *, hipStream_t);
+
 bool bf16_pack_fused_supported(int dim) { return !bf16_is_wide(dim); }
 template <typename T>
 hipError_t launch_bf16_pack_queries(const T *Q, const float *mu, size_t nq, size_t nq_pad, int dim, size_t ld,
                                     void *B, double *qn, uint32_t *qbad, bool ci, double bmax, double dmax,
-                                    hipStream_t s, T *Qp, size_t ldq, uint32_t *misc, const Bf16SeedModel *smp) {
+                                    hipStream_t s, T *Qp, size_t ldq, uint32_t *misc, const Bf16SeedModel *smp,
+                                    const Bf16I8Query *i8p) {
     if ((Qp || misc) && !bf16_pack_fused_supported(dim)) return hipErrorInvalidValue;
     Bf16SeedModel sm{};
     if (smp) sm = *smp;
+    Bf16I8Query i8{};
+    if (i8p) i8 = *i8p;
+    if (i8.Q && (!i8.m || !i8.kappa || !i8.outside || !(i8.s > 0.0) || !ci)) return hipErrorInvalidValue;
     if (sm.seed_out && (!sm.m1 || !sm.a || !sm.b)) return hipErrorInvalidValue;
     if (!bf16_is_wide(dim)) {
         hipLaunchKernelGGL(bf16_pack_queries8_kernel<T>, dim3((unsigned)(nq_pad * 8 / 256)), dim3(256), 0, s, Q, mu, nq,
                            nq_pad, dim, ld, bf16_ks_for(dim, ci), static_cast<uint16_t *>(B), qn, qbad, ci ? 1 : 0,
-                           bmax, dmax, Qp, ldq, misc, sm);
+                           bmax, dmax, Qp, ldq, misc, sm, i8);
         return hipGetLastError();
     }
+    if (i8.Q) return hipErrorInvalidValue;
     if (ci || nq_pad % 32 != 0) return hipErrorInvalidValue;
     hipLaunchKernelGGL((bf16_pack_wide8_kernel<T, true>), dim3((unsigned)(nq_pad * 8 / 256)), dim3(256), 0, s, Q, mu, nq, nq_pad,
                        dim, ld, static_cast<uint16_t *>(B), qn, qbad, (uint32_t *)nullptr, sm);
@@ -2564,10 +2862,10 @@
 
 template hipError_t launch_bf16_pack_queries<float>(const float *, const float *, size_t, size_t, int, size_t, void *, double *,
                                                     uint32_t *, bool, double, double, hipStream_t, float *, size_t, uint32_t *,
-                                                    const Bf16SeedModel *);
+                                                    const Bf16SeedModel *, const Bf16I8Query *);
 template hipError_t launch_bf16_pack_queries<double>(const double *, const float *, size_t, size_t, int, size_t, void *, double *,
                                                      uint32_t *, bool, double, double, hipStream_t, double *, size_t, uint32_t *,
-                                                     const Bf16SeedModel *);
+                                                     const Bf16SeedModel *, const Bf16I8Query *);
 
 static_assert(kBQ == (int)kBf16QueryTile && kBP == (int)kBf16RowTile && kWR == (int)kBf16WideTile, "bf16_launch.h");
 static void bf_debug_kernel(const char *which, unsigned grid, unsigned block) {
@@ -2595,6 +2893,45 @@
     if (thresholds != (l.tau != nullptr) || (l.pass == Bf16Pass::ScoutOnly) != (l.scout_out != nullptr)) return false;
     return l.pass != Bf16Pass::Radius || (cb.cap == 256 && !l.refresh);
 }
+static BfShared bf_shared_args(const Bf16Launch &l) {
+    BfShared a{};
+    a.nseg = (uint32_t)l.cb.nseg;
+    if (l.seed) {
+        a.seed_lists = l.seed->lists;
+        a.seed_rank = l.seed->rank;
+        a.seed_nq = l.seed->nq;
+        a.seed_words = l.seed->words;
+    }
+    return a;
+}
+template <int KS8>
+static hipError_t launch_i8_pair(const Bf16Launch &l, hipStream_t s) {
+    const CandBuf &cb = l.cb;
+    const Bf16Grid &g = l.grid;
+    const size_t sh = (size_t)3 * kBP * (2 * KS8 + 1) * 16 + 16;
+    const uint32_t kp = (uint32_t)l.kp;
+    const uint32_t kp_keep = kp | ((uint32_t)(cb.final_keep > (int)kp ? cb.final_keep : 0) << 16);
+    const unsigned grid = (unsigned)(((g.q_tiles + 1u) / 2u) * ((unsigned)g.n_wg / g.q_tiles));
+    bf_debug_kernel(BfOpI8::name, grid, 512);
+    return bf_go<i8_filter_kernel_pair<KS8>>(grid, 512, sh, s, static_cast<const char *>(l.i8->img), g.n_tiles,
+                                             static_cast<const u32x4 *>(l.i8->Q), g.q_tiles, kp_keep,
+                                             static_cast<uint2 *>(cb.keys), cb.cnt, static_cast<uint32_t *>(cb.tau), cb.nq_pad, l.tau,
+                                             bf_shared_args(l), BfOpI8::Args{l.i8->kappa, l.i8->c, l.i8->outside, l.i8->epoch});
+}
+template <int KS>
+static hipError_t launch_pair_behind_i8(const Bf16Launch &l, hipStream_t s) {
+    const CandBuf &cb = l.cb;
+    const Bf16Grid &g = l.grid;
+    const size_t sh = (size_t)3 * kBP * (2 * KS + 1) * 16 + 16;
+    const uint32_t kp = (uint32_t)l.kp;
+    const uint32_t kp_keep = kp | ((uint32_t)(cb.final_keep > (int)kp ? cb.final_keep : 0) << 16);
+    const unsigned grid = (unsigned)(((g.q_tiles + 1u) / 2u) * ((unsigned)g.n_wg / g.q_tiles));
+    bf_debug_kernel("pair_if_outside", grid, 512);
+    return bf_go<bf16_pair_behind_i8_kernel<KS>>(grid, 512, sh, s, static_cast<const char *>(l.img), g.n_tiles,
+                                                 static_cast<const u32x4 *>(l.B), g.q_tiles, kp_keep, static_cast<uint2 *>(cb.keys),
+                                                 cb.cnt, static_cast<uint32_t *>(cb.tau), cb.nq_pad, l.tau, bf_shared_args(l),
+                                                 l.i8->outside, l.i8->epoch);
+}
 template <int KS, int M, bool RAD, bool CI>
 static hipError_t launch_bf16_t(const Bf16Launch &l, hipStream_t s) {
     const CandBuf &cb = l.cb;
@@ -2604,14 +2941,7 @@
     const uint32_t kp_keep = kp | ((uint32_t)(M <= 2 && !RAD && cb.final_keep > (int)kp ? cb.final_keep : 0) << 16);
     const uint32_t spp = (uint32_t)bf16_touching((size_t)g.q_tiles * split, g.n_wg);
     const unsigned n_wg = (unsigned)g.n_wg, n_all = n_wg + (unsigned)(l.refresh ? l.refresh->n_refresh : 0);
-    BfShared a{};
-    a.nseg = (uint32_t)cb.nseg;
-    if (l.seed) {
-        a.seed_lists = l.seed->lists;
-        a.seed_rank = l.seed->rank;
-        a.seed_nq = l.seed->nq;
-        a.seed_words = l.seed->words;
-    }
+    BfShared a = bf_shared_args(l);
     if (l.refresh) {
         a.pcnt = l.refresh->pcnt;
         a.done = l.refresh->done;
@@ -2627,7 +2957,7 @@
         if constexpr (M == 1)
             if (l.kernel == Bf16Kernel::Pair) {
                 const unsigned grid = (unsigned)(((g.q_tiles + 1u) / 2u) * (n_wg / g.q_tiles));
-                bf_debug_kernel("pair", grid, 512);
+                bf_debug_kernel(BfOpBf16::name, grid, 512);
                 return bf_go<bf16_filter_kernel_pair<KS, CI>>(grid, 512, sh, s, img, g.n_tiles, B, g.q_tiles, kp_keep, keys,
                                                               cb.cnt, tau, cb.nq_pad, l.tau, a);
             }
@@ -2684,6 +3014,33 @@
     }
     if (l.seed && (!l.seed->lists || l.seed->rank < 1 || l.seed->rank > (uint32_t)kScoutList || !bf16_seed_in_kernel(cb.nseg)))
         return hipErrorInvalidValue;
+    if ((l.kernel == Bf16Kernel::I8Pair) != l.i8.has_value()) return hipErrorInvalidValue;
+    if (l.i8) {
+        if (!l.ci || !l.i8->img || !l.i8->Q || !l.i8->kappa || !l.i8->outside || !(l.i8->c > 0.0f)) return hipErrorInvalidValue;
+        hipError_t e;
+#ifdef PN_DEV_KS8_ONLY
+        if (i8_steps(l.dim) != 4 || bf16_ks_for(l.dim, true) != 8) return hipErrorInvalidValue;
+        e = launch_i8_pair<4>(l, s);
+        return e != hipSuccess ? e : launch_pair_behind_i8<8>(l, s);
+#else
+        switch (i8_steps(l.dim)) {
+            case 2: e = launch_i8_pair<2>(l, s); break;
+            case 3: e = launch_i8_pair<3>(l, s); break;
+            default: e = launch_i8_pair<4>(l, s); break;
+        }
+        if (e != hipSuccess) return e;
+        switch (bf16_ks_for(l.dim, true)) {
+            case 2: return launch_pair_behind_i8<2>(l, s);
+            case 3: return launch_pair_behind_i8<3>(l, s);
+            case 4: return launch_pair_behind_i8<4>(l, s);
+            case 5: return launch_pair_behind_i8<5>(l, s);
+            case 6: return launch_pair_behind_i8<6>(l, s);
+            case 7: return launch_pair_behind_i8<7>(l, s);
+            case 8: return launch_pair_behind_i8<8>(l, s);
+            default: return hipErrorInvalidValue;
+        }
+#endif
+    }
 #define PN_BF_CASE(K, C) \
     case K: return launch_bf16_m<K, C>(l, s);
 #ifdef PN_DEV_KS8_ONLY
diff --git a/petal-neighbors_amd/csrc/bf16_launch.h b/petal-neighbors_amd/csrc/bf16_launch.h
--- a/petal-neighbors_amd/csrc/bf16_launch.h
+++ b/petal-neighbors_amd/csrc/bf16_launch.h
@@ -6,7 +6,7 @@
 namespace pn {
 
 enum class Bf16Pass { ScoutOnly, SelfScout, Seeded, Radius };
-enum class Bf16Kernel { Four, Eight, Pair, Wide };
+enum class Bf16Kernel { Four, Eight, Pair, Wide, I8Pair };
 
 constexpr uint32_t kBf16QueryTile = 256;
 constexpr uint32_t kBf16RowTile = 64;
@@ -62,4 +62,12 @@
     return want8 ? Bf16Kernel::Eight : Bf16Kernel::Four;
 }
 
+
+inline bool i8_main_kernel(const Bf16Grid &g, int cap, Bf16Pass pass, bool refreshers, size_t image_bytes, int wg_slots,
+                           int forced, bool image, bool gate, int i8_opt) {
+    if (!image || i8_opt == 2 || forced != 0 || !bf16_kernel_applies(Bf16Kernel::I8Pair, g, cap, pass, refreshers)) return false;
+    if (i8_opt == 1) return true;
+    return gate && bf16_main_kernel(g, cap, pass, refreshers, image_bytes, wg_slots, 0) == Bf16Kernel::Pair;
 }
+
+}
diff --git a/petal-neighbors_amd/csrc/index.hip b/petal-neighbors_amd/csrc/index.hip
--- a/petal-neighbors_amd/csrc/index.hip
+++ b/petal-neighbors_amd/csrc/index.hip
@@ -119,6 +119,7 @@
 struct WorkspaceBufs {
     DevBuf w_q, w_qnorm, w_qnrm, w_keys, w_idx, w_cnt, w_tau, w_flags, w_sel, w_misc, w2_keys, w2_idx, w2_cnt, w2_tau, w_lo;
     DevBuf w_bq, w_qn, w_qbad, w_gq, w_gqn, w_gsel, w_seed, w_lists;
+    DevBuf w_bq8, w_kappa, w_i8out;
     DevBuf w_hq, w_hidx, w_hdist;
     DevBuf w_hrad;
     DevBuf w_fparts;
@@ -155,6 +156,7 @@
         return PN_OK;
     }
     uint32_t sh_epoch = 0;
+    uint32_t i8_epoch = 0;
     size_t sh_nseg = 0, sh_nq_pad = 0;
     hipStream_t stream = nullptr;
     hipEvent_t ev_r[2] = {nullptr, nullptr};
@@ -220,8 +222,16 @@
     double sm_c0 = 0.0, sm_v0 = 0.0;
     double sm_zgrid[kSeedModelGrid] = {};
     double sm_sigma = 0.0;
+    double sm_sd_row = 0.0;
     bool sm_ok = false;
     int seed_model = 1;
+    void *d_img8 = nullptr;
+    float *d_m8 = nullptr;
+    double i8_step = 0.0, i8_emax = 0.0, i8_pmax = 0.0;
+    double i8_inflation = 0.0;
+    bool i8_gate = false;
+    double bf16_bmean = 0.0, bf16_dmean = 0.0;
+    int i8_filter = 0;
     uint64_t piece[kPieceFamilies] = {};
     uint64_t mst_batch = 0;
     int kmeans_filter = 0;
@@ -381,6 +391,8 @@
 
 template <typename RT>
 static int seed_model_build(pn_index *ix, const RT *rows, hipStream_t s);
+template <typename T>
+static int i8_build(pn_index *ix, hipStream_t s, bool gated);
 template <typename T>
 static int finish_index(pn_index *ix, const T *d_src, size_t row_stride, hipStream_t s) {
     {
@@ -461,6 +473,8 @@
                           h_st[0] < 1e30 && h_st[1] < 1e30;
             ix->bf16_bmax = h_st[0];
             ix->bf16_dmax = h_st[1];
+            ix->bf16_bmean = bmean;
+            ix->bf16_dmean = dmean;
         }
         HIPCHK(hipMalloc(&ix->d_img, bf16_image_bytes(ix->n, (int)ix->dim, ix->bf16_ci)));
         HIPCHK(pack());
@@ -491,6 +505,7 @@
         if (nrm.p) PNCHK(seed_model_build<double>(ix, (const double *)nrm.p, s));
     } else {
         PNCHK(seed_model_build<T>(ix, (const T *)ix->d_pts, s));
+        if (ix->sm_ok) PNCHK(i8_build<T>(ix, s, true));
     }
     return PN_OK;
 }
@@ -658,6 +673,8 @@
     if (ix->d_img) (void)hipFree(ix->d_img);
     if (ix->d_mu) (void)hipFree(ix->d_mu);
     if (ix->d_smodel) (void)hipFree(ix->d_smodel);
+    if (ix->d_img8) (void)hipFree(ix->d_img8);
+    if (ix->d_m8) (void)hipFree(ix->d_m8);
     if (ix->d_norm) (void)hipFree(ix->d_norm);
     if (ix->d_cnorm) (void)hipFree(ix->d_cnorm);
     if (ix->d_stats) (void)hipFree(ix->d_stats);
@@ -910,6 +927,16 @@
             if (value != 0 && value != 1) return fail(PN_ERR_INVALID, "bad seed-model switch (0 or 1)");
             ix->seed_model = (int)value;
             return PN_OK;
+        case PN_OPT_I8_FILTER: {
+            if (value < 0 || value > 2) return fail(PN_ERR_INVALID, "bad int8 filter choice (0, 1 or 2)");
+            if (value == 1 && !ix->d_img8) {
+                DeviceGuard g(ix->device);
+                if (!g.ok) return fail(PN_ERR_DEVICE, "hipSetDevice(%d) failed", ix->device);
+                PNCHK(ix->elem_bytes == 8 ? i8_build<double>(ix, ix->stream, false) : i8_build<float>(ix, ix->stream, false));
+            }
+            ix->i8_filter = (int)value;
+            return PN_OK;
+        }
         case PN_OPT_DBSCAN_PIECE: return set_piece(ix, kPieceDbscan, value, "bad DBSCAN piece size");
         case PN_OPT_MST_BATCH:
             if (value < 0) return fail(PN_ERR_INVALID, "bad MST batch size");
@@ -1275,6 +1302,11 @@
     const double lm = ls / (double)used, lv = lss / (double)used - lm * lm;
     ix->sm_c0 = c0;
     ix->sm_v0 = v0;
+    {
+        double sd = 0.0;
+        for (size_t q = 0; q < NQ; ++q) sd += qsd[q];
+        ix->sm_sd_row = sd / (double)used;
+    }
     ix->sm_sigma = std::sqrt(lv > 0.0 ? lv : 0.0);
     bool mono = true;
     for (int j = 1; j < kSeedModelGrid; ++j) mono = mono && ix->sm_zgrid[j] < ix->sm_zgrid[j - 1];
@@ -1290,6 +1322,84 @@
     HIPCHK(hipMemcpyAsync(ix->d_smodel, h_model.data(), h_model.size() * sizeof(float), hipMemcpyHostToDevice, s));
     HIPCHK(hipStreamSynchronize(s));
     ix->sm_ok = true;
+    return PN_OK;
+}
+
+#ifndef PN_DIAG_I8_COARSEN
+#define PN_DIAG_I8_COARSEN 1.0
+#endif
+constexpr double kI8MaxInflation = 1.0;
+template <typename T>
+static int i8_build(pn_index *ix, hipStream_t s, bool gated) {
+    const int dim = (int)ix->dim;
+    if (ix->d_img8 || !ix->bf16_ok || !ix->bf16_ci || ix->metric != 0 || dim > 128 || !ix->d_pts) return PN_OK;
+    if (gated && !ix->sm_ok) return PN_OK;
+    DevTmp scr;
+    const size_t sums_bytes = (ix->dim + 1) * sizeof(double), scr_bytes = sums_bytes + 8 * sizeof(double);
+    HIPCHK(scr.alloc(scr_bytes));
+    HIPCHK(hipMemsetAsync(scr.p, 0, scr_bytes, s));
+    double *d_sums = (double *)scr.p, *d_st = (double *)((char *)scr.p + sums_bytes);
+    const T *rows = (const T *)ix->d_pts;
+    std::vector<double> h((ix->dim + 1) + 8);
+    HIPCHK(launch_bf16_column_sums<T>(rows, ix->n, dim, ix->ld, d_sums, s));
+    HIPCHK(hipMemcpyAsync(h.data(), d_sums, sums_bytes, hipMemcpyDeviceToHost, s));
+    HIPCHK(hipStreamSynchronize(s));
+    std::vector<float> h_m(ix->ld, 0.0f);
+    for (int k = 0; k < dim; ++k) {
+        h_m[k] = (float)(h[k] / (double)ix->n);
+        if (!std::isfinite(h_m[k])) return PN_OK;
+    }
+    float *d_m = nullptr;
+    HIPCHK(hipMalloc((void **)&d_m, ix->ld * sizeof(float)));
+    struct Drop {
+        float *m;
+        void *img = nullptr;
+        ~Drop() {
+            if (m) (void)hipFree(m);
+            if (img) (void)hipFree(img);
+        }
+    } drop{d_m};
+    HIPCHK(hipMemcpyAsync(d_m, h_m.data(), ix->ld * sizeof(float), hipMemcpyHostToDevice, s));
+    HIPCHK(launch_i8_absmax<T>(rows, d_m, ix->n, dim, ix->ld, d_st, s));
+    HIPCHK(hipMemcpyAsync(h.data(), d_st, sizeof(double), hipMemcpyDeviceToHost, s));
+    HIPCHK(hipStreamSynchronize(s));
+    const double amax = h[0];
+    if (!(amax > 0.0) || !(amax < 1e18) || !(amax > 1e-18)) return PN_OK;
+    float step_f = (float)(amax / 127.0 * (1.0 + 1.0 / 1048576.0) * (double)PN_DIAG_I8_COARSEN);
+    if ((double)step_f * 127.0 < amax) step_f = std::nextafter(step_f, INFINITY);
+    const double step = (double)step_f;
+    HIPCHK(hipMalloc(&drop.img, i8_image_bytes(ix->n, dim)));
+    HIPCHK(launch_i8_pack_corpus<T>(rows, d_m, ix->n, dim, ix->ld, step, drop.img, d_st + 4, s));
+    HIPCHK(hipMemcpyAsync(h.data(), d_st + 4, 4 * sizeof(double), hipMemcpyDeviceToHost, s));
+    HIPCHK(hipStreamSynchronize(s));
+    const double up = 1.0 + 1.0 / 1099511627776.0;
+    const double e_max = std::sqrt(h[0]) * up, p_max = std::sqrt(h[1]) * up;
+    const double e_mean = h[2] / (double)ix->n, p_mean = h[3] / (double)ix->n;
+    if (!std::isfinite(e_max) || !std::isfinite(p_max) || !(p_max > 0.0)) return PN_OK;
+    double inflation = 0.0;
+    if (ix->sm_ok && ix->sm_sd_row > 0.0) {
+        const double g = 1.0 / 8192.0;
+        const double slack8 = 2.0 * (p_mean * e_max + e_mean * p_max) + 2.0 * step * step;
+        const double aq = 0.5 * ix->bf16_dmean, cq = 0.5 * (ix->bf16_bmean - 2.0 * g * aq);
+        const double slack16 = aq * ix->bf16_bmax + (cq > 0.0 ? cq : 0.0) * ix->bf16_dmax;
+        inflation = std::exp(ix->sm_zgrid[2] * (slack8 - slack16) / ix->sm_sd_row);
+    }
+    const bool pass = inflation > 0.0 && inflation <= kI8MaxInflation;
+    if (plan_knobs().debug)
+        std::fprintf(stderr, "[pn int8 image] n %zu dim %d: step %.6g, max |e_p| %.6g (mean %.6g), max |p - m| %.6g (mean %.6g), "
+                             "predicted candidate inflation %.3f (limit %.2f): %s\n",
+                     ix->n, dim, step, e_max, e_mean, p_max, p_mean, inflation, kI8MaxInflation,
+                     pass ? "kept" : gated ? "dropped" : "kept for PN_OPT_I8_FILTER = 1 only");
+    if (gated && !pass) return PN_OK;
+    ix->d_img8 = drop.img;
+    ix->d_m8 = d_m;
+    drop.img = nullptr;
+    drop.m = nullptr;
+    ix->i8_step = step;
+    ix->i8_emax = e_max;
+    ix->i8_pmax = p_max;
+    ix->i8_inflation = inflation;
+    ix->i8_gate = pass;
     return PN_OK;
 }
 
@@ -1547,6 +1657,9 @@
     p.main_pass = p.shared_scout || (p.model_seed && ix->d_smodel) ? Bf16Pass::Seeded : Bf16Pass::SelfScout;
     p.main_kernel = bf16_main_kernel(p.grid, p.cap, p.main_pass, p.n_refresh > 0,
                                      bf16_image_bytes(ix->n, (int)ix->dim, ix->bf16_ci), 2 * ix->n_cu, ix->bf16_waves);
+    if (i8_main_kernel(p.grid, p.cap, p.main_pass, p.n_refresh > 0, bf16_image_bytes(ix->n, (int)ix->dim, ix->bf16_ci),
+                       2 * ix->n_cu, ix->bf16_waves, ix->d_img8 != nullptr, ix->i8_gate, ix->i8_filter))
+        p.main_kernel = Bf16Kernel::I8Pair;
     if (plan_knobs().debug)
         fprintf(stderr, "bf16_plan: n %zu q_tiles %zu k %zu R %.0f: n_wg %d per_tile %zu split %d nseg %d kp %d cap %d aligned %d "
                         "shared_scout %d scout_tiles %d seed_rank %d scout_max %d n_refresh %d sh_rank %d model_seed %d z %.3f\n",
@@ -1659,6 +1772,26 @@
         smd.seed_out = (uint32_t *)ws.w_seed.p;
         if (rec) rec->model_seed = true;
     }
+    const bool i8 = plan.main_kernel == Bf16Kernel::I8Pair;
+    Bf16I8Query q8{};
+    if (i8) {
+        if (!ix->d_img8 || cosine) return fail(PN_ERR_INVALID, "int8 filter planned on an index without its image");
+        PNCHK(ws.w_bq8.ensure(i8_query_bytes(nq_pad, (int)ix->dim)));
+        PNCHK(ws.w_kappa.ensure(nq_pad * sizeof(float)));
+        const void *out_before = ws.w_i8out.p;
+        PNCHK(ws.w_i8out.ensure(sizeof(uint32_t)));
+        if (ws.w_i8out.p != out_before) {
+            HIPCHK(hipMemsetAsync(ws.w_i8out.p, 0, sizeof(uint32_t), s));
+            ws.i8_epoch = 0;
+        }
+        if (ws.i8_epoch == 0xFFFFFFFFu) {
+            HIPCHK(hipMemsetAsync(ws.w_i8out.p, 0, sizeof(uint32_t), s));
+            ws.i8_epoch = 0;
+        }
+        ws.i8_epoch += 1u;
+        q8 = Bf16I8Query{ix->d_m8, ix->i8_step, ix->i8_emax, ix->i8_pmax, ws.w_bq8.p, (float *)ws.w_kappa.p,
+                         (uint32_t *)ws.w_i8out.p, ws.i8_epoch};
+    }
     if (cosine) {
         PNCHK(ws.w_qnrm.ensure(nq_pad * ix->ld * sizeof(double)));
         HIPCHK(launch_cos_normalize_rows<T>(Qp, nq, nq_pad, (int)ix->dim, ix->ld, (double *)ws.w_qnrm.p, ix->ld, nullptr,
@@ -1670,11 +1803,12 @@
     } else if (d_q_raw)
         HIPCHK(launch_bf16_pack_queries(d_q_raw, ix->d_mu, nq, nq_pad, (int)ix->dim, q_stride, ws.w_bq.p,
                                         (double *)ws.w_qn.p, (uint32_t *)ws.w_qbad.p, ix->bf16_ci, ix->bf16_bmax,
-                                        ix->bf16_dmax, s, const_cast<T *>(Qp), ix->ld, d_misc, model ? &smd : nullptr));
+                                        ix->bf16_dmax, s, const_cast<T *>(Qp), ix->ld, d_misc, model ? &smd : nullptr,
+                                        i8 ? &q8 : nullptr));
     else
         HIPCHK(launch_bf16_pack_queries(Qp, ix->d_mu, nq, nq_pad, (int)ix->dim, ix->ld, ws.w_bq.p, (double *)ws.w_qn.p,
                                         (uint32_t *)ws.w_qbad.p, ix->bf16_ci, ix->bf16_bmax, ix->bf16_dmax, s,
-                                        (T *)nullptr, 0, nullptr, model ? &smd : nullptr));
+                                        (T *)nullptr, 0, nullptr, model ? &smd : nullptr, i8 ? &q8 : nullptr));
     CandBuf cb{ws.w_keys.p, (uint32_t *)ws.w_keys.p + 1, (uint32_t *)ws.w_cnt.p, ws.w_tau.p, nq_pad, nseg, cap, 2};
     cb.final_keep = bf16_cell_max((int)kp, cap, nseg, bf16_is_wide((int)ix->dim));
     if (!plan.grid.aligned) {
@@ -1688,6 +1822,11 @@
         rec->two_launches = plan.shared_scout && !model;
     }
     Bf16Launch main{ix->d_img, ix->n, (int)ix->dim, ix->bf16_ci, ws.w_bq.p, (int)kp, cb, plan.grid, plan.main_pass, plan.main_kernel};
+    if (i8) {
+        const double step = ix->i8_step;
+        main.i8 = Bf16I8Operands{ix->d_img8, ws.w_bq8.p, (const float *)ws.w_kappa.p, (float)(2.0 * step * step),
+                                 (const uint32_t *)ws.w_i8out.p, ws.i8_epoch};
+    }
     auto launch = [&](const Bf16Launch &l) { return plan.wide ? launch_bf16_wide_filter(l, s) : launch_bf16_filter(l, s); };
     if (plan.shared_scout) {
         const size_t words = cells * 2 * (size_t)bf16_scout_list();
@@ -1699,6 +1838,7 @@
             if (!plan.wide && bf16_seed_in_kernel(nseg) && plan.seed_rank <= bf16_scout_list())
                 main.seed = Bf16SeedLists{(const float *)ws.w_lists.p, (uint32_t)plan.seed_rank, (uint32_t)nq, (uint32_t *)ws.w_seed.p};
             Bf16Launch scout = main;
+            scout.i8.reset();
             scout.pass = Bf16Pass::ScoutOnly;
             scout.kernel = plan.wide ? Bf16Kernel::Wide : Bf16Kernel::Four;
             scout.scout_tiles = plan.scout_tiles;
diff --git a/petal-neighbors_amd/csrc/pn_internal.h b/petal-neighbors_amd/csrc/pn_internal.h
--- a/petal-neighbors_amd/csrc/pn_internal.h
+++ b/petal-neighbors_amd/csrc/pn_internal.h
@@ -400,11 +400,27 @@
     double c0 = 0.0, v0 = 0.0, z = 0.0;
     uint32_t *seed_out = nullptr;
 };
+struct Bf16I8Query {
+    const float *m = nullptr;
+    double s = 0.0, e_max = 0.0, p_max = 0.0;
+    void *Q = nullptr;
+    float *kappa = nullptr;
+    uint32_t *outside = nullptr;
+    uint32_t epoch = 0;
+};
+int i8_ks_for(int dim);
+size_t i8_image_bytes(size_t n, int dim);
+size_t i8_query_bytes(size_t nq_pad, int dim);
+template <typename T>
+hipError_t launch_i8_absmax(const T *P, const float *m, size_t n, int dim, size_t ld, double *out, hipStream_t s);
+template <typename T>
+hipError_t launch_i8_pack_corpus(const T *P, const float *m, size_t n, int dim, size_t ld, double step, void *img, double *st,
+                                 hipStream_t s);
 template <typename T>
 hipError_t launch_bf16_pack_queries(const T *Q, const float *mu, size_t nq, size_t nq_pad, int dim, size_t ld,
                                     void *B, double *qn, uint32_t *qbad, bool ci, double bmax, double dmax,
                                     hipStream_t s, T *Qp = nullptr, size_t ldq = 0, uint32_t *misc = nullptr,
-                                    const Bf16SeedModel *sm = nullptr);
+                                    const Bf16SeedModel *sm = nullptr, const Bf16I8Query *i8 = nullptr);
 template <typename T>
 hipError_t launch_bf16_column_moments(const T *P, const float *mu, size_t n, int dim, size_t ld, double *out, hipStream_t s);
 struct Bf16SeedLists {
@@ -416,6 +432,13 @@
     uint32_t *pcnt, *done;
     uint32_t epoch, rank;
     int n_refresh;
+};
+struct Bf16I8Operands {
+    const void *img, *Q;
+    const float *kappa;
+    float c;
+    const uint32_t *outside;
+    uint32_t epoch;
 };
 struct Bf16Launch {
     const void *img;
@@ -433,6 +456,7 @@
     float *scout_out = nullptr;
     std::optional<Bf16SeedLists> seed;
     std::optional<Bf16Refresh> refresh;
+    std::optional<Bf16I8Operands> i8;
 };
 bool bf16_seed_in_kernel(int nseg);
 bool bf16_shared_supported(int cap);
```
